# danielzgtg/TTS.cpp

Hardware: AMD Instinct MI355X
Metric: audio-sec/wall-sec (RTF^-1), Parler-TTS-mini v1 Q4_K AR decode + DAC decode (higher is better)
Workload: dtype q4_K weights x q8_K activations (int dot, f32 combine); DAC f16 im2col x f32 weights, f64 accumulate

## Files before the change

### include/tts_hip.h

```cpp
#ifndef TTS_HIP_H
#define TTS_HIP_H

#include <stddef.h>
#include <stdint.h>

#ifdef __cplusplus
extern "C" {
#endif

#define TTS_MAX_DIMS 4
#define TTS_MAX_SRC 4
#define TTS_MAX_OP_PARAMS 16
#define TTS_MAX_NAME 64

enum tts_type {
    TTS_TYPE_F32 = 0,
    TTS_TYPE_F16 = 1,
    TTS_TYPE_Q4_0 = 2,
    TTS_TYPE_Q4_1 = 3,
    TTS_TYPE_Q5_0 = 6,
    TTS_TYPE_Q5_1 = 7,
    TTS_TYPE_Q8_0 = 8,
    TTS_TYPE_Q8_1 = 9,
    TTS_TYPE_Q4_K = 12,
// ... 122 lines not shown
const char * tts_hip_backend_name(tts_hip_backend_t backend);

void * tts_hip_buffer_alloc(tts_hip_backend_t backend, size_t size);
void tts_hip_buffer_free(tts_hip_backend_t backend, void * ptr);
size_t tts_hip_buffer_alignment(void);

int tts_hip_tensor_set(tts_hip_backend_t backend, void * dst_dev, const void * src_host, size_t size);
int tts_hip_tensor_get(tts_hip_backend_t backend, void * dst_host, const void * src_dev, size_t size);
int tts_hip_tensor_copy(tts_hip_backend_t backend, void * dst_dev, const void * src_dev, size_t size);
int tts_hip_copy_stream(tts_hip_backend_t backend, void * dst_dev, const void * src_dev, size_t size);
int tts_hip_plan_stats(tts_tensor * const * nodes, int n_nodes, int mask, int32_t * counts);
int tts_hip_tensor_set_async(tts_hip_backend_t backend, void * dst_dev, const void * src_host, size_t size);
int tts_hip_memset(tts_hip_backend_t backend, void * dst_dev, int value, size_t size);
int tts_hip_synchronize(tts_hip_backend_t backend);

int tts_hip_weight_set(tts_hip_backend_t backend, tts_tensor * t, const void * src_host);
int tts_hip_weight_get(tts_hip_backend_t backend, const tts_tensor * t, void * dst_host);
int tts_hip_quantize(tts_hip_backend_t backend, int type, const float * x_dev, void * dst_dev, int64_t rows, int64_t K);
void tts_repack_q4_K(const void * src, void * dst, int64_t nblocks, int inverse);
void tts_repack_q4_K_tiled(const void * src, void * dst, int64_t nrows, int64_t nb, int inverse);

int tts_hip_supports_op(const tts_tensor * node);
int tts_hip_graph_compute(tts_hip_backend_t backend, tts_tensor * const * nodes, int n_nodes);
int tts_hip_graph_prepare(tts_hip_backend_t backend, tts_tensor * const * nodes, int n_nodes, int slot);
int tts_hip_graph_launch(tts_hip_backend_t backend, int slot);

enum tts_hip_option {
    TTS_HIP_OPT_FUSION = 0,
    TTS_HIP_OPT_PROFILE_GEMV = 1,
    TTS_HIP_OPT_GRAPHS = 2,
    TTS_HIP_OPT_CONV_F32ACC = 3,
    TTS_HIP_OPT_CONVT_LDS = 4,
    TTS_HIP_OPT_ATTN_SPLIT = 5,
    TTS_HIP_OPT_KV_PREFETCH = 6,
    TTS_HIP_OPT_KV_PREFETCH_BLOCKS = 7,
    TTS_HIP_OPT_Q4K_TILE_BYTES = 8,
    TTS_HIP_OPT_GEMV_DEBUG = 10,
    TTS_HIP_OPT_CONV_SPLIT = 12,
    TTS_HIP_OPT_GEMV_UNIQUE = 11,
    TTS_HIP_OPT_GEMV_KS = 13,
    TTS_HIP_OPT_ATTN_FUSED = 14,
    TTS_HIP_OPT_GEMM_Q8 = 18,
    TTS_HIP_OPT_BGEMM_F32 = 19,
    TTS_HIP_OPT_CU_PARTITION = 20,
    TTS_HIP_OPT_Q4K_DUAL_BYTES = 16,
    TTS_HIP_OPT_GEMV_RSPLIT = 17,
    TTS_HIP_OPT_ATTN_PV16 = 15,
    TTS_HIP_OPT_GEMV_PREQUANT = 21,
    TTS_HIP_OPT_GEMV_KRELAY = 22,
    TTS_HIP_OPT_ATTN_KS = 23,
    TTS_HIP_OPT_ATTN_PV8 = 24,
    TTS_HIP_OPT_GEMV_KRELAY_LOOP = 26,
    TTS_HIP_OPT_GEMV_Q80_PRO = 27,
    TTS_HIP_OPT_GEMV_Q80_SLAB = 28,
    TTS_HIP_OPT_GEMV_Q80_RW = 29,
    TTS_HIP_OPT_GEMM_Q8_STAGED = 30,
    TTS_HIP_OPT_GEMV_KR_INKERNEL = 31,
    TTS_HIP_OPT_GEMV_F32_WIDE = 32,
    TTS_HIP_OPT_ATTN_PV_MP = 33,
    TTS_HIP_OPT_GEMM_KR_INKERNEL = 35,
    TTS_HIP_OPT_GEMM_KR_CT2 = 36,
    TTS_HIP_OPT_GEMM_KR_NW = 34,
    TTS_HIP_OPT_GEMV_NW_MIN = 25,
    TTS_HIP_OPT_GEMM_KR_XCD = 38,
    TTS_HIP_OPT_GEMM_KR_CP = 39,
    TTS_HIP_OPT_GEMM_KR_WALK = 40,
    TTS_HIP_OPT_GEMM_PF = 41,
    TTS_HIP_OPT_GEMM_PF_NW = 42,
    TTS_HIP_OPT_ATTN_ONE = 43,
    TTS_HIP_OPT_GEMV_KR_TAIL = 44,
    TTS_HIP_OPT_GEMV_Q50_SLAB = 45,
    TTS_HIP_OPT_GEMV_Q50_RW = 46,
    TTS_HIP_OPT_GEMM_Q5 = 47,
    TTS_HIP_OPT_GEMM_Q5_STAGED = 48,
    TTS_HIP_OPT_GEMV_Q40_SLAB = 49,
    TTS_HIP_OPT_GEMV_Q40_RW = 50,
    TTS_HIP_OPT_GEMM_Q4_0 = 51,
    TTS_HIP_OPT_GEMM_Q4_0_STAGED = 52,
    TTS_HIP_OPT_CONV_VFMA = 53,
    TTS_HIP_OPT_CONV_TILE96 = 54,
    TTS_HIP_OPT_CONV_PACK = 55,
    TTS_HIP_OPT_CONVT_PACK = 56,
    TTS_HIP_OPT_CONV_XREG = 57,
    TTS_HIP_OPT_COALESCE = 37,
};
enum tts_fuse_bits {
    TTS_FUSE_LN = 1, TTS_FUSE_GROUP = 2, TTS_FUSE_KV = 4, TTS_FUSE_EPI = 8, TTS_FUSE_HEADS = 16, TTS_FUSE_ATTN = 32,
    TTS_FUSE_LSTM = 64,
    TTS_FUSE_SNAKE = 128,
    TTS_FUSE_EMBED = 256,
    TTS_FUSE_CONV = 512,
    TTS_FUSE_ADAIN = 1024,
    TTS_FUSE_XATTN = 2048,
    TTS_FUSE_MCPY = 4096,
    TTS_FUSE_CONTREAD = 8192
};
int tts_hip_set_option(tts_hip_backend_t backend, int option, int value);
int tts_hip_attn_decode(tts_hip_backend_t backend, const tts_tensor * q, const tts_tensor * k, const tts_tensor * v,
                        const float * mask, int64_t mbs, float scale, float * out, float * out2, const int64_t * koff,
                        const int64_t * voff, const int64_t * moff, const int32_t * pseq);
int tts_hip_coalesce_stats(int device, int64_t * out, int n);
void tts_hip_coalesce_set_wait(int us);
int tts_hip_coalesce_enable(int on);
#define TTS_HIP_HOOK_FAULT_WEIGHT_SET 1
int tts_hip_test_hook(int hook, int value);
int tts_hip_install_crash_handler(void);
int tts_hip_gemv_stats(tts_hip_backend_t backend, int type, double * ms, int64_t * launches, double * bytes, int reset);
int tts_hip_greedy_step(tts_hip_backend_t backend, const float * logits, int32_t B, int32_t NH, int32_t V, int32_t step,
                        int32_t bos, int32_t eos, int32_t * eos_seen, int32_t * hist, int32_t * next);
typedef struct tts_sampling {
    float temperature;
    float top_p;
    float repetition_penalty;
    int32_t top_k;
    int32_t do_sample;
    int32_t pad_;
    uint64_t seed;
} tts_sampling;
void tts_sampling_default(tts_sampling * cfg);
uint32_t tts_sampler_call_seed(uint64_t seed, int32_t stream, int64_t call);
int tts_sampler_sample(const tts_sampling * cfg, const float * logits, int32_t NH, int32_t V, uint32_t call_seed, int32_t * last,
                       int32_t * count, int32_t * out);
int tts_hip_sample_step(tts_hip_backend_t backend, const float * logits, int32_t B, int32_t NH, int32_t V, const tts_sampling * cfg,
                        int64_t call, int32_t * rep_state, int32_t step, int32_t bos, int32_t eos, int32_t * eos_seen, int32_t * hist,
                        int32_t * next);
int tts_sampling_device_ok(const tts_sampling * cfg, int32_t V);
int tts_hip_counters(tts_hip_backend_t backend, int64_t * out, int n);

int tts_hip_gemv(tts_hip_backend_t backend, int type, const void * w, const float * x, float * y,
                 int64_t K, int64_t N, int64_t M);
int tts_hip_gemv_ex(tts_hip_backend_t backend, int type, const void * w, const float * x, float * y,
                    int64_t K, int64_t N, int64_t M, int32_t wflags);
int tts_hip_gemv_res(tts_hip_backend_t backend, int type, const void * w, const float * x, float * y, const float * res,
                     int64_t K, int64_t N, int64_t M, int32_t wflags);

typedef struct tts_backend_iface {
    void * ctx;
    const char * name;
    void * (*alloc)(void * ctx, size_t size);
    void (*free)(void * ctx, void * ptr);
    int (*set)(void * ctx, void * dst, const void * src, size_t size);
    int (*set_tensor)(void * ctx, tts_tensor * t, const void * src);
    int (*get)(void * ctx, void * dst, const void * src, size_t size);
    int (*memset)(void * ctx, void * dst, int value, size_t size);
    int (*compute)(void * ctx, tts_tensor * const * nodes, int n_nodes);
    int (*synchronize)(void * ctx);
    int (*prepare)(void * ctx, tts_tensor * const * nodes, int n_nodes, int slot);
    int (*launch)(void * ctx, int slot);
    int (*set_async)(void * ctx, void * dst, const void * src, size_t size);
    int (*copy)(void * ctx, void * dst, const void * src, size_t size);
    int (*greedy_step)(void * ctx, const float * logits, int B, int NH, int V, int step, int bos, int eos, int32_t * eos_seen,
                       int32_t * hist, int32_t * next);
    int (*sample_step)(void * ctx, const float * logits, int B, int NH, int V, const tts_sampling * cfg, int64_t call, int32_t * rep_state,
                       int step, int bos, int eos, int32_t * eos_seen, int32_t * hist, int32_t * next);
} tts_backend_iface;

int tts_hip_backend_iface(tts_hip_backend_t backend, tts_backend_iface * out);

#ifdef __cplusplus
}
#endif

#endif
```

### tts.cpp_amd/csrc/backend.hip

```cpp
#include <cmath>
#include <atomic>
#include <cstring>
#include <map>
#include <mutex>
#include <thread>

#include "hip_internal.h"
#include <hip/hip_ext.h>

#include <dlfcn.h>
#include <execinfo.h>
#include <fcntl.h>
#include <signal.h>
#include <unistd.h>

using namespace tts;


static void build_gelu_table(uint16_t * t) {
    const float GELU_COEF_A = 0.044715f;
    const float SQRT_2_OVER_PI = 0.79788456080286535587989211986876f;
    for (int i = 0; i < 65536; ++i) {
        const float x = fp16_to_fp32_host((uint16_t)i);
        const float g = 0.5f * x * (1.0f + tanhf(SQRT_2_OVER_PI * x * (1.0f + GELU_COEF_A * x * x)));
// ... 326 lines not shown
        tts::conv_pack_freed(nullptr, ptr, r.size);
        tts::coalesce_written(ptr, r.size);
    }
    hipFree(ptr);
}

int tts_hip_tensor_set(tts_hip_backend_t be, void * dst, const void * src, size_t size) {
    if (!be) return TTS_STATUS_BAD_ARG;
    hipSetDevice(be->device);
    be->rb_clear();
    drop_tiled_copies(dst, size);
    tts::coalesce_written(dst, size);
    if (size > 0 && size <= be->pin_size / 4) {
        const int st = tts_hip_tensor_set_async(be, dst, src, size);
        if (st != 0) return st;
    } else if (hipMemcpyAsync(dst, src, size, hipMemcpyHostToDevice, be->stream) != hipSuccess) {
        return TTS_STATUS_FAILED;
    } else {
        tts::conv_pack_written(be, dst, size);
    }
    if (hipStreamSynchronize(be->stream) != hipSuccess) return TTS_STATUS_FAILED;
    return 0;
}

int tts_hip_tensor_set_async(tts_hip_backend_t be, void * dst, const void * src, size_t size) {
    if (!be) return TTS_STATUS_BAD_ARG;
    if (size == 0) return 0;
    hipSetDevice(be->device);
    be->rb_clear();
    if (size > be->pin_size / 2) return tts_hip_tensor_set(be, dst, src, size);
    tts::coalesce_written(dst, size);
    std::lock_guard<std::mutex> pl(be->pin_mu);
    while (!be->pin_pending.empty() && hipEventQuery(be->pin_pending.front().ev) == hipSuccess) {
        be->pin_events.push_back(be->pin_pending.front().ev);
        be->pin_pending.pop_front();
    }
    size_t off = (be->pin_head + 255) & ~(size_t)255;
    if (off + size > be->pin_size) off = 0;
    int last = -1;
    for (int i = 0; i < (int)be->pin_pending.size(); ++i) {
        const auto & r = be->pin_pending[i];
        if (r.off < off + size && off < r.off + r.size) last = i;
    }
    if (last >= 0) {
        if (hipEventSynchronize(be->pin_pending[last].ev) != hipSuccess) return TTS_STATUS_FAILED;
        for (int i = 0; i <= last; ++i) {
            be->pin_events.push_back(be->pin_pending.front().ev);
            be->pin_pending.pop_front();
        }
    }
    memcpy(be->pin + off, src, size);
    if (hipMemcpyAsync(dst, be->pin + off, size, hipMemcpyHostToDevice, be->stream) != hipSuccess) return TTS_STATUS_FAILED;
    tts::conv_pack_written(be, dst, size);
    hipEvent_t ev;
    if (be->pin_events.empty()) {
        if (hipEventCreateWithFlags(&ev, hipEventDisableTiming) != hipSuccess) return TTS_STATUS_FAILED;
    } else {
        ev = be->pin_events.back();
        be->pin_events.pop_back();
    }
    if (hipEventRecord(ev, be->stream) != hipSuccess) return TTS_STATUS_FAILED;
    be->pin_pending.push_back({off, size, ev});
    be->pin_head = off + size;
    return 0;
}

int tts_hip_greedy_step(tts_hip_backend_t be, const float * logits, int32_t B, int32_t NH, int32_t V, int32_t step, int32_t bos,
                        int32_t eos, int32_t * eos_seen, int32_t * hist, int32_t * next) {
    if (!be || !logits || B <= 0 || NH <= 0 || V <= 0) return TTS_STATUS_BAD_ARG;
    hipSetDevice(be->device);
    be->rb_clear();
    launch_greedy_step(be, logits, B, NH, V, step, bos, eos, eos_seen, hist, next);
    return 0;
}

int tts_hip_sample_step(tts_hip_backend_t be, const float * logits, int32_t B, int32_t NH, int32_t V, const tts_sampling * cfg, int64_t call,
                        int32_t * rep_state, int32_t step, int32_t bos, int32_t eos, int32_t * eos_seen, int32_t * hist, int32_t * next) {
    if (!be || !logits || !cfg || B <= 0 || NH <= 0 || V <= 0) return TTS_STATUS_BAD_ARG;
    hipSetDevice(be->device);
    be->rb_clear();
    return launch_sample_step(be, logits, B, NH, V, cfg, call, rep_state, step, bos, eos, eos_seen, hist, next);
}

int tts_hip_tensor_get(tts_hip_backend_t be, void * dst, const void * src, size_t size) {
    if (!be) return TTS_STATUS_BAD_ARG;
    hipSetDevice(be->device);
    if (be->rb_any.load(std::memory_order_acquire)) {
        std::lock_guard<std::mutex> l(be->rb_mu);
        for (const auto & r : be->rb) {
            const char * s = (const char *)src;
            if (s >= r.dev && s + size <= r.dev + r.bytes) {
                if (hipStreamSynchronize(be->stream) != hipSuccess) return TTS_STATUS_FAILED;
                memcpy(dst, be->rb_host + r.off + (s - r.dev), size);
                return 0;
            }
        }
    }
    if (hipMemcpyAsync(dst, src, size, hipMemcpyDeviceToHost, be->stream) != hipSuccess) return TTS_STATUS_FAILED;
    if (hipStreamSynchronize(be->stream) != hipSuccess) return TTS_STATUS_FAILED;
    return 0;
}

int tts_hip_copy_stream(tts_hip_backend_t be, void * dst, const void * src, size_t size) {
    if (!be || !dst || !src || size % 16 || ((uintptr_t)dst | (uintptr_t)src) % 16) return TTS_STATUS_BAD_ARG;
    if (size == 0) return 0;
    hipSetDevice(be->device);
    be->rb_clear();
    tts::launch_copy_stream(be, dst, src, (int64_t)(size / 16));
    tts::conv_pack_written(be, dst, size);
    return hipGetLastError() == hipSuccess ? 0 : TTS_STATUS_FAILED;
}

int tts_hip_tensor_copy(tts_hip_backend_t be, void * dst, const void * src, size_t size) {
    if (!be) return TTS_STATUS_BAD_ARG;
    hipSetDevice(be->device);
    be->rb_clear();
    tts::coalesce_written(dst, size);
    tts::launch_copy_bytes(be, dst, src, size);
    tts::conv_pack_written(be, dst, size);
    return hipGetLastError() == hipSuccess ? 0 : TTS_STATUS_FAILED;
}

int tts_hip_memset(tts_hip_backend_t be, void * dst, int value, size_t size) {
    if (!be) return TTS_STATUS_BAD_ARG;
    hipSetDevice(be->device);
    be->rb_clear();
    tts::coalesce_written(dst, size);
    if (hipMemsetAsync(dst, value, size, be->stream) != hipSuccess) return TTS_STATUS_FAILED;
    tts::conv_pack_written(be, dst, size);
    return 0;
}

int tts_hip_synchronize(tts_hip_backend_t be) {
    if (!be) return TTS_STATUS_BAD_ARG;
    hipSetDevice(be->device);
    return hipStreamSynchronize(be->stream) == hipSuccess ? 0 : TTS_STATUS_FAILED;
}

void tts_repack_q4_K(const void * src, void * dst, int64_t nblocks, int inverse) {
    const uint8_t * s = (const uint8_t *)src;
    uint8_t * d = (uint8_t *)dst;
    for (int64_t b = 0; b < nblocks; ++b) {
        const uint8_t * sb = s + b * 144;
        uint8_t * db = d + b * 144;
        memcpy(db, sb, 16);
        for (int i = 0; i < 128; ++i) {
            const int l = i >> 4, c = (i >> 2) & 3, k = i & 3;
            const int nat = 32 * c + 8 * k + l;
            if (!inverse) db[16 + i] = sb[16 + nat];
            else db[16 + nat] = sb[16 + i];
        }
    }
}

static void repack_tiled_rows(const uint8_t * s, uint8_t * d, int64_t r0, int64_t r1, int64_t nb, int inverse) {
    const int64_t rb = nb * 144;
    for (int64_t row = r0; row < r1; ++row) {
        const int64_t t = row >> 2, i = row & 3;
        for (int64_t b = 0; b < nb; ++b) {
            const int64_t nat = row * rb + b * 144;
            const int64_t til = (t * nb + b) * 576;
            const uint8_t * a = inverse ? s + til : s + nat;
            uint8_t * o = inverse ? d + nat : d + til;
            if (!inverse) memcpy(o + i * 16, a, 16);
            else memcpy(o, a + i * 16, 16);
            for (int c = 0; c < 4; ++c)
// ... 330 lines not shown
        }
        default:
            return 0;
    }
}

}

extern "C" int tts_hip_set_option(tts_hip_backend_t be, int option, int value) {
    if (!be) return TTS_STATUS_BAD_ARG;
    switch (option) {
        case TTS_HIP_OPT_FUSION: be->fusion = value; return 0;
        case TTS_HIP_OPT_CONVT_LDS: be->convt_lds = value != 0; return 0;
        case TTS_HIP_OPT_CONV_SPLIT: be->conv_split = value < 0 ? 1 : value; return 0;
        case TTS_HIP_OPT_CONV_VFMA: be->conv_vfma = value < 0 || value > 2 ? 1 : value; return 0;
        case TTS_HIP_OPT_CONV_TILE96: be->conv_tile96 = value != 0; return 0;
        case TTS_HIP_OPT_CONV_PACK: be->conv_pack = value != 0; return 0;
        case TTS_HIP_OPT_CONVT_PACK: be->convt_pack = value != 0; return 0;
        case TTS_HIP_OPT_CONV_XREG: be->conv_xreg = value != 0; return 0;
        case TTS_HIP_OPT_PROFILE_GEMV: be->profile_gemv = value != 0; return 0;
        case TTS_HIP_OPT_GRAPHS: be->use_graphs = value != 0; return 0;
        case TTS_HIP_OPT_CONV_F32ACC:
            be->conv_f32acc = value == 1;
            be->conv_acc_mode = value == 2 ? 2 : 0;
            return 0;
        case TTS_HIP_OPT_ATTN_SPLIT: be->attn_split_minp = value; return 0;
        case TTS_HIP_OPT_ATTN_FUSED: be->attn_fused_minp = value; return 0;
        case TTS_HIP_OPT_ATTN_PV16: be->attn_pv_uv16 = value != 0; return 0;
        case TTS_HIP_OPT_KV_PREFETCH: be->kv_prefetch_minp = value; return 0;
        case TTS_HIP_OPT_Q4K_TILE_BYTES: be->q4k_tile_bytes = value; return 0;
        case TTS_HIP_OPT_Q4K_DUAL_BYTES: be->q4k_dual_bytes = value; return 0;
        case TTS_HIP_OPT_GEMV_RSPLIT: be->gemv_mf_rsplit = value != 0; return 0;
        case TTS_HIP_OPT_GEMV_PREQUANT: be->gemv_mf_prequant = value != 0; return 0;
        case TTS_HIP_OPT_GEMV_KRELAY: be->gemv_kr = value != 0; return 0;
        case TTS_HIP_OPT_GEMV_KRELAY_LOOP: be->gemv_kr_loop = value != 0; return 0;
        case TTS_HIP_OPT_GEMV_Q80_PRO: be->gemv_q80_pro = value != 0; return 0;
        case TTS_HIP_OPT_GEMV_Q80_SLAB: be->gemv_q80_slab = value != 0; return 0;
        case TTS_HIP_OPT_GEMV_KR_INKERNEL:
            if (value < 0) return TTS_STATUS_BAD_ARG;
            be->gemv_kr_ink = value;
            return 0;
        case TTS_HIP_OPT_GEMM_Q8_STAGED:
            if (value < 0 || value > 2) return TTS_STATUS_BAD_ARG;
            be->gemm_q8_staged = value;
            return 0;
        case TTS_HIP_OPT_GEMV_Q80_RW:
            if (value < 0 || value > 32 || (value & (value - 1))) return TTS_STATUS_BAD_ARG;
            be->gemv_q80_rw = value;
            return 0;
        case TTS_HIP_OPT_GEMV_Q50_SLAB: be->gemv_q50_slab = value != 0; return 0;
        case TTS_HIP_OPT_GEMV_Q50_RW:
            if (value < 0 || value > 32 || (value & (value - 1))) return TTS_STATUS_BAD_ARG;
            be->gemv_q50_rw = value;
            return 0;
        case TTS_HIP_OPT_GEMM_Q5: be->gemm_q5 = value != 0; return 0;
        case TTS_HIP_OPT_GEMM_Q5_STAGED:
            if (value < 0 || value > 2) return TTS_STATUS_BAD_ARG;
            be->gemm_q5_staged = value;
            return 0;
        case TTS_HIP_OPT_GEMV_Q40_SLAB: be->gemv_q40_slab = value != 0; return 0;
        case TTS_HIP_OPT_GEMV_Q40_RW:
            if (value < 0 || value > 32 || (value & (value - 1))) return TTS_STATUS_BAD_ARG;
            be->gemv_q40_rw = value;
            return 0;
        case TTS_HIP_OPT_GEMM_Q4_0: be->gemm_q4_0 = value != 0; return 0;
        case TTS_HIP_OPT_GEMM_Q4_0_STAGED:
            if (value < 0 || value > 2) return TTS_STATUS_BAD_ARG;
            be->gemm_q4_0_staged = value;
            return 0;
        case TTS_HIP_OPT_ATTN_KS: be->attn_ks = value; return 0;
        case TTS_HIP_OPT_GEMV_NW_MIN: be->gemv_nw_min = value; return 0;
        case TTS_HIP_OPT_ATTN_PV8: be->attn_pv8 = value != 0; return 0;
        case TTS_HIP_OPT_GEMM_KR_CT2: be->gemm_kr_ct2 = value != 0; return 0;
        case TTS_HIP_OPT_GEMM_KR_INKERNEL: be->gemm_kr_ink = value < 0 ? 0 : value; return 0;
        case TTS_HIP_OPT_ATTN_PV_MP: be->attn_pv_mp = value == 2 ? 2 : value != 0; return 0;
        case TTS_HIP_OPT_ATTN_ONE:
            if (value < 0 || value > 2) return TTS_STATUS_BAD_ARG;
            be->attn_one = value;
            return 0;
        case TTS_HIP_OPT_GEMV_KR_TAIL:
            if (value < 0 || value > 4) return TTS_STATUS_BAD_ARG;
            be->gemv_kr_tail = value;
            return 0;
        case TTS_HIP_OPT_GEMM_KR_NW: be->gemm_kr_nw = value == 8 ? 8 : 4; return 0;
        case TTS_HIP_OPT_GEMM_Q8: be->gemm_q8 = value != 0; return 0;
        case TTS_HIP_OPT_CU_PARTITION: {
            const int count = value & 0xFF, index = (value >> 8) & 0xFF;
            const bool inter = (value >> 16) & 1;
            hipSetDevice(be->device);
            TTS_HIP_CHECK(hipStreamSynchronize(be->stream));
            hipStream_t ns = nullptr;
            if (count <= 1) {
                TTS_HIP_CHECK(hipStreamCreateWithFlags(&ns, hipStreamNonBlocking));
                be->cus = be->cu_total;
            } else {
                if (index >= count) return TTS_STATUS_BAD_ARG;
                std::vector<uint32_t> mask((be->cu_total + 31) / 32, 0u);
                const int per = be->cu_total / count;
                int n = 0;
                for (int c = 0; c < be->cu_total; ++c) {
                    const bool on = inter ? (c % count == index) : (c / per == index && c < per * count);
                    if (on) mask[c / 32] |= 1u << (c % 32), ++n;
                }
                if (hipExtStreamCreateWithCUMask(&ns, (uint32_t)mask.size(), mask.data()) != hipSuccess) return TTS_STATUS_FAILED;
                be->cus = n;
            }
            TTS_HIP_CHECK(hipStreamDestroy(be->stream));
            be->stream = ns;
            for (auto & ex : be->gsig_exec)
                if (ex) hipGraphExecDestroy(ex), ex = nullptr;
            for (auto & g : be->gsig) g = 0;
            return 0;
        }
        case TTS_HIP_OPT_BGEMM_F32: be->bgemm_f32 = value != 0; return 0;
        case TTS_HIP_OPT_GEMV_F32_WIDE: be->gemv_f32_wide = value != 0; return 0;
        case TTS_HIP_OPT_GEMV_DEBUG: be->gemv_dbg = value; return 0;
        case TTS_HIP_OPT_GEMV_UNIQUE: be->gemv_unique = value != 0; return 0;
        case TTS_HIP_OPT_GEMV_KS: be->gemv_ks_tiles = value > 0 ? value : 0; return 0;
        case TTS_HIP_OPT_COALESCE: be->co_member = value != 0; return 0;
        case TTS_HIP_OPT_GEMM_KR_XCD: be->gemm_kr_xcd = value != 0; return 0;
        case TTS_HIP_OPT_GEMM_KR_CP: be->gemm_kr_cp = value != 0; return 0;
        case TTS_HIP_OPT_GEMM_KR_WALK: be->gemm_kr_walk = value < 0 ? 0 : value; return 0;
        case TTS_HIP_OPT_GEMM_PF: be->gemm_pf = value < 0 ? 0 : value; return 0;
        case TTS_HIP_OPT_GEMM_PF_NW: be->gemm_pf_nw = value == 8 ? 8 : 4; return 0;
        case TTS_HIP_OPT_KV_PREFETCH_BLOCKS: be->kv_prefetch_blocks = value > 0 ? value : 1; return 0;
        default: return TTS_STATUS_BAD_ARG;
    }
}

extern "C" int tts_hip_counters(tts_hip_backend_t be, int64_t * out, int n) {
    if (!be || !out) return TTS_STATUS_BAD_ARG;
    const int64_t v[10] = {be->graph_updates, be->graph_instantiations, be->lstm_chains, be->lstm_steps, be->plan_wait_ns,
                           be->cap_plan_ns, be->cap_launch_ns, be->cap_update_ns, (int64_t)g_packs_n.load(), (int64_t)g_packs_bytes.load()};
    int k = 0;
    for (; k < n && k < 10; ++k) out[k] = v[k];
    return k;
}

extern "C" int tts_hip_gemv_stats(tts_hip_backend_t be, int type, double * ms, int64_t * launches, double * bytes, int reset) {
    if (!be) return TTS_STATUS_BAD_ARG;
    hipSetDevice(be->device);
    TTS_HIP_CHECK(hipStreamSynchronize(be->stream));
    for (size_t i = 0; i < be->ev_pending.size(); ++i) {
        float t = 0;
        TTS_HIP_CHECK(hipEventElapsedTime(&t, be->ev_pending[i].first, be->ev_pending[i].second));
        const int ty = be->ev_type[i];
        be->gemv_ms[ty] += t;
        be->gemv_launches[ty] += 1;
        be->gemv_bytes[ty] += be->ev_bytes[i];
        be->ev_free.push_back(be->ev_pending[i].first);
        be->ev_free.push_back(be->ev_pending[i].second);
    }
    be->ev_pending.clear();
    be->ev_bytes.clear();
    be->ev_type.clear();
    double a = 0, c = 0;
    int64_t b = 0;
    for (int ty = 0; ty < TTS_TYPE_COUNT; ++ty) {
        if (type >= 0 && ty != type) continue;
        a += be->gemv_ms[ty];
        b += be->gemv_launches[ty];
        c += be->gemv_bytes[ty];
    }
    if (ms) *ms = a;
    if (launches) *launches = b;
    if (bytes) *bytes = c;
    if (reset) {
        for (int ty = 0; ty < TTS_TYPE_COUNT; ++ty) {
            be->gemv_ms[ty] = 0;
            be->gemv_launches[ty] = 0;
            be->gemv_bytes[ty] = 0;
        }
    }
    return 0;
}

static void * hb_alloc(void * c, size_t n) { return tts_hip_buffer_alloc((tts_hip_backend_t)c, n); }
static void hb_free(void * c, void * p) { tts_hip_buffer_free((tts_hip_backend_t)c, p); }
static int hb_set(void * c, void * d, const void * s, size_t n) { return tts_hip_tensor_set((tts_hip_backend_t)c, d, s, n); }
static int hb_set_tensor(void * c, tts_tensor * t, const void * s) { return tts_hip_weight_set((tts_hip_backend_t)c, t, s); }
static int hb_get(void * c, void * d, const void * s, size_t n) { return tts_hip_tensor_get((tts_hip_backend_t)c, d, s, n); }
static int hb_memset(void * c, void * d, int v, size_t n) { return tts_hip_memset((tts_hip_backend_t)c, d, v, n); }
static int hb_compute(void * c, tts_tensor * const * nodes, int n) { return tts_hip_graph_compute((tts_hip_backend_t)c, nodes, n); }
static int hb_sync(void * c) { return tts_hip_synchronize((tts_hip_backend_t)c); }
static int hb_prepare(void * c, tts_tensor * const * nodes, int n, int slot) {
    return tts_hip_graph_prepare((tts_hip_backend_t)c, nodes, n, slot);
}
static int hb_launch(void * c, int slot) { return tts_hip_graph_launch((tts_hip_backend_t)c, slot); }
static int hb_set_async(void * c, void * d, const void * s, size_t n) { return tts_hip_tensor_set_async((tts_hip_backend_t)c, d, s, n); }
static int hb_copy(void * c, void * d, const void * s, size_t n) { return tts_hip_tensor_copy((tts_hip_backend_t)c, d, s, n); }
static int hb_greedy(void * c, const float * l, int B, int NH, int V, int step, int bos, int eos, int32_t * seen, int32_t * hist, int32_t * next) {
    return tts_hip_greedy_step((tts_hip_backend_t)c, l, B, NH, V, step, bos, eos, seen, hist, next);
}
static int hb_sample(void * c, const float * l, int B, int NH, int V, const tts_sampling * cfg, int64_t call, int32_t * rep, int step, int bos,
                     int eos, int32_t * seen, int32_t * hist, int32_t * next) {
    return tts_hip_sample_step((tts_hip_backend_t)c, l, B, NH, V, cfg, call, rep, step, bos, eos, seen, hist, next);
}

extern "C" int tts_hip_backend_iface(tts_hip_backend_t be, tts_backend_iface * out) {
    if (!be || !out) return TTS_STATUS_BAD_ARG;
    out->ctx = be;
    out->name = be->name;
    out->alloc = hb_alloc;
    out->free = hb_free;
    out->set = hb_set;
    out->set_tensor = hb_set_tensor;
    out->get = hb_get;
    out->memset = hb_memset;
    out->compute = hb_compute;
    out->synchronize = hb_sync;
    out->prepare = hb_prepare;
    out->launch = hb_launch;
    out->set_async = hb_set_async;
    out->copy = hb_copy;
    out->greedy_step = hb_greedy;
    out->sample_step = hb_sample;
    return 0;
}
```

### tts.cpp_amd/csrc/hip_internal.h

```cpp
#pragma once

#include <hip/hip_fp16.h>
#include <hip/hip_runtime.h>

#include <cstdio>
#include <cstdlib>
#include <atomic>
#include <deque>
#include <mutex>
#include <unordered_map>
#include <tuple>
#include <vector>

#include "common.h"

#define TTS_HIP_CHECK(expr)                                                                          \
    do {                                                                                             \
        hipError_t err_ = (expr);                                                                    \
        if (err_ != hipSuccess) {                                                                    \
            fprintf(stderr, "%s:%d: HIP error %s: %s\n", __FILE__, __LINE__, #expr, hipGetErrorString(err_)); \
            abort();                                                                                 \
        }                                                                                            \
    } while (0)

// ... 273 lines not shown
    const int64_t *koff = nullptr, *voff = nullptr;
    const int64_t * moff = nullptr;
    const int * pseq = nullptr;
    int pmax = 0;
    const int64_t * ioff[EMBED_MAX_TERMS] = {};
};
struct BatchCtx {
    int N = 0;
    uint64_t key = 0;
    std::vector<BatchCls> cls;
    std::vector<tts_tensor * const *> mnodes;
    std::vector<tts_hip_backend *> mbe;
    int n_nodes = 0;
    bool checked = false;
    int canon = 0;
    bool ragged = false;
    bool differs = false;
    std::vector<ItemTab> tabs;
    void * comap = nullptr;
    const BatchCls * find(const void * p) const {
        const char * c = (const char *)p;
        size_t lo = 0, hi = cls.size();
        while (lo < hi) {
            const size_t m = (lo + hi) / 2;
            if (cls[m].b0 <= c) lo = m + 1;
            else hi = m;
        }
        if (lo == 0) return nullptr;
        const BatchCls & b = cls[lo - 1];
        return c < b.b0 + b.size ? &b : nullptr;
    }
    template <typename T>
    T * win(T * p) const {
        const BatchCls * b = p ? find(p) : nullptr;
        return b ? (T *)(b->win + ((const char *)p - b->b0)) : p;
    }
    int64_t stride(const void * p) const {
        const BatchCls * b = p ? find(p) : nullptr;
        return b ? b->stride : 0;
    }
    template <typename T>
    T * reloc(T * p, int k) const {
        const BatchCls * b = p ? find(p) : nullptr;
        return b ? (T *)(b->win + k * b->stride + ((const char *)p - b->b0)) : p;
    }
};

}

struct tts_hip_backend {
    int device = 0;
    hipStream_t stream = nullptr;
    char name[64] = {0};
    char * scratch = nullptr;
    size_t scratch_size = 0;
    float * shadow = nullptr;
    size_t shadow_size = 0;
    void * hoist = nullptr;
    size_t hoist_size = 0;
    float * attn_buf = nullptr;
    size_t attn_floats = 0;
    int attn_split_minp = 128;
    int attn_ks = 2;
    int attn_pv_mp = 1;
    int attn_one = 1;
    int attn_pv8 = 0;
    int attn_pv_uv16 = 0;
    int attn_fused_minp = 0;
    unsigned long long * argmax_keys = nullptr;
    unsigned * argmax_counts = nullptr;
    int64_t q4k_tile_bytes = 4 << 20;
    int gemv_dbg = 0;
    int gemv_unique = 1;
    int gemm_q8 = 1;
    int64_t cus = 256;
    int cu_total = 256;
    int bgemm_f32 = 1;
    int gemv_f32_wide = 1;
    int gemm_kr_nw = 4;
    int64_t gemv_ks_tiles = 256;
    int gemv_mf_prequant = 1;
    int gemv_kr = 1;
    int gemv_kr_loop = 1;
    int gemv_kr_tail = 1;
    int gemv_q80_pro = 1;
    int gemv_q80_slab = 1;
    int gemv_q80_rw = 0;
    int gemm_q8_staged = 2;
    int gemv_q50_slab = 1;
    int gemv_q50_rw = 0;
    int gemm_q5 = 1;
    int gemm_q5_staged = 2;
    int gemv_q40_slab = 1;
    int gemv_q40_rw = 0;
    int gemm_q4_0 = 1;
    int gemm_q4_0_staged = 2;
    int64_t gemv_kr_ink = 0;
    int gemm_kr_walk = 0;
    int gemm_pf = 64;
    int gemm_pf_nw = 4;
    int gemm_kr_cp = 0;
    int gemm_kr_xcd = 0;
    int gemm_kr_ct2 = 0;
    int64_t gemm_kr_ink = 0;
    int gemv_nw_min = 0;
    int gemv_mf_rsplit = 1;
    int64_t q4k_dual_bytes = 1 << 20;
    void * sample_cand = nullptr;
    size_t sample_cand_size = 0;
    int kv_prefetch_minp = 0;
    int kv_prefetch_blocks = 128;
    hipStream_t pf_stream = nullptr;
    hipEvent_t pf_fork = nullptr, pf_join = nullptr;
    uint8_t * pin = nullptr;
    size_t pin_size = 0, pin_head = 0;
    struct PinRec {
        size_t off, size;
        hipEvent_t ev;
    };
    std::deque<PinRec> pin_pending;
    std::vector<hipEvent_t> pin_events;
    std::mutex pin_mu;
    hipEvent_t plan_ev[2] = {nullptr, nullptr};
    bool plan_ev_pending[2] = {false, false};
    float * lstm_buf = nullptr;
    float * conv_stage = nullptr;
    size_t conv_stage_floats = 0;
    float * vec_scratch = nullptr;
    size_t lstm_floats = 0;
    tts::ActQuant aq;
    int64_t graph_epoch = 0;
    uint16_t * gelu_table = nullptr;
    bool convt_lds = true;
    double * conv_part = nullptr;
    size_t conv_part_doubles = 0;
    int conv_vfma = 1;
    int conv_tile96 = 1;
    int conv_pack = 1;
    int convt_pack = 1;
    int conv_xreg = 1;
    bool capturing = false;
    int conv_split = 1;
    int fusion = 0x3FFF;
    bool profile_gemv = false;
    double gemv_ms[TTS_TYPE_COUNT] = {0};
    int64_t gemv_launches[TTS_TYPE_COUNT] = {0};
    double gemv_bytes[TTS_TYPE_COUNT] = {0};
    std::vector<std::pair<hipEvent_t, hipEvent_t>> ev_pending;
    std::vector<double> ev_bytes;
    std::vector<int> ev_type;
    std::vector<hipEvent_t> ev_free;
    char * repack_tmp = nullptr;
    size_t repack_tmp_size = 0;
    std::vector<char *> repack_retired;
    float * attn_stage = nullptr;
    size_t attn_stage_size = 0;
    bool use_graphs = false;
    static constexpr int N_GSIG = 4;
    uint64_t gsig[N_GSIG] = {};
    hipGraphExec_t gsig_exec[N_GSIG] = {};
    int gsig_next = 0;
    bool conv_f32acc = false;
    int conv_acc_mode = 0;
    hipStream_t cap_stream = nullptr;
    int64_t graph_updates = 0, graph_instantiations = 0;
    int64_t lstm_chains = 0, lstm_steps = 0;
    int64_t plan_wait_ns = 0;
    int64_t cap_plan_ns = 0, cap_launch_ns = 0, cap_update_ns = 0;
    hipGraphExec_t pexec[2] = {nullptr, nullptr};
    tts_tensor * const * plan_nodes[2] = {nullptr, nullptr};
    int plan_n[2] = {0, 0};
    bool plan_eager[2] = {true, true};
    bool plan_prepared[2] = {false, false};
    tts::BatchCtx * bat = nullptr;
    hipEvent_t co_ev = nullptr;
    int64_t * co_tab = nullptr;
    size_t co_tab_bytes = 0;
    int64_t co_prep_ns = 0;
    bool co_member = true;
    struct RbEnt {
        const char * dev;
        size_t bytes, off;
    };
    char * rb_host = nullptr;
    size_t rb_cap = 0;
    std::vector<RbEnt> rb;
    std::mutex rb_mu;
    std::atomic<bool> rb_any{false};
    void rb_clear() {
        if (!rb_any.load(std::memory_order_acquire)) return;
        std::lock_guard<std::mutex> l(rb_mu);
        rb.clear();
        rb_any.store(false, std::memory_order_release);
    }
};

namespace tts {

const uint8_t * tiled_copy_find(const void * weight);

void profile_pair(tts_hip_backend * be, hipEvent_t & e0, hipEvent_t & e1);
void profile_push(tts_hip_backend * be, hipEvent_t e0, hipEvent_t e1, double bytes, int type);

void launch_quantize_act(tts_hip_backend * be, int wtype, const float * x, int64_t xcs, int64_t K, int64_t M, ActQuant & aq);
void launch_gemv_job(tts_hip_backend * be, const GemvJob & job);
bool gemv_q6k_ok(const GemvJob & j);
bool launch_bgemm_f32(tts_hip_backend * be, const tts_tensor * node);
bool gemm_f32_ok(const GemvJob & j);
void launch_gemm_f32(tts_hip_backend * be, const GemvJob & j);
void launch_copy_cols(tts_hip_backend * be, float * dst, const float * src, int64_t K, int64_t scs, int64_t M);
void launch_profile_spin(tts_hip_backend * be, double us);
void launch_im2col(tts_hip_backend * be, const tts_tensor * node);
constexpr int kLstmQMaxK = 512;
struct LstmStepArgs {
    const float * pre[4];
    const void * w[4];
    int64_t w_rs[4];
    const float * bias[4];
    const float * hprev;
    const float * cprev;
    float * h;
    float * c;
    int Hd, K, wtype;
};
void launch_lstm_step(tts_hip_backend * be, const LstmStepArgs & a, const LstmStepArgs * b = nullptr);
void launch_repeat_interleave1(tts_hip_backend * be, const tts_tensor * dst, const tts_tensor * a, int r);
void launch_copy_bytes(tts_hip_backend * be, void * dst, const void * src, size_t bytes);
void launch_cpy_multi(tts_hip_backend * be, const tts_tensor * src, const tts_tensor * const * dsts, int nd);
void launch_rope_multi(tts_hip_backend * be, const tts_tensor * rope, const tts_tensor * src, const tts_tensor * const * dsts, int nd);
void launch_greedy_step(tts_hip_backend * be, const float * logits, int B, int NH, int V, int step, int bos, int eos, int32_t * eos_seen,
                        int32_t * hist, int32_t * next);
int launch_sample_step(tts_hip_backend * be, const float * logits, int B, int NH, int V, const tts_sampling * c, int64_t call,
                       int32_t * rep_state, int step, int bos, int eos, int32_t * eos_seen, int32_t * hist, int32_t * next);
struct BatchCtx;
void launch_embed_sum(tts_hip_backend * be, const tts_tensor * out, const tts_tensor * const * gr, int n, const BatchCtx * bat = nullptr,
                      const ItemTab * tab = nullptr);
void launch_snake(tts_hip_backend * be, const tts_tensor * dst, const tts_tensor * x, const tts_tensor * alpha, const tts_tensor * recip,
                  const tts_tensor * one = nullptr, const tts_tensor * mask = nullptr);
void launch_lstm_finish(tts_hip_backend * be, const tts_tensor * final_out, const float * hist, int64_t Hd, int64_t T);
bool audio_op_supported(const tts_tensor * n);
int launch_audio_op(tts_hip_backend * be, const tts_tensor * n);
void launch_conv_transpose_1d(tts_hip_backend * be, const tts_tensor * node, int w_stable = 0);
constexpr int CONV1D_MAX_R = 128;
struct Conv1dArgs {
    TD x;
    const void * w = nullptr;
    int w16 = 0;
    int64_t wk = 0, wic = 0, woc = 0;
    float * y = nullptr;
    int64_t ycs = 0;
    const float * bias = nullptr;
    int64_t bcs = 0;
    const float * res = nullptr;
    int64_t rcs = 0;
    int64_t L = 0, IC = 0, OL = 0, OC = 0;
    int K = 1, s = 1, p = 0, d = 1;
    int icc = 0, xw = 0, rs = 0;
    float * copy_dst = nullptr;
    uint32_t x_bytes = 0, w_bytes = 0;
    double * part = nullptr;
    int ic_per_split = 0;
    int w_stable = 0;
    const float * wimg = nullptr;
};
constexpr int CONV1D_XN = 16, CONV1D_WN = 16;
inline int conv1d_icc(int64_t IC, int K, int xw) {
    int best = 0;
    double best_eff = -1.0;
    const int top = (int)(IC < 64 ? IC : 64);
    for (int c = 1; c <= top; ++c) {
        const int r = c * K, rp = (r + 31) & ~31;
        if (rp > 64 || c * xw > 256 * CONV1D_XN) break;
        const double eff = (double)r / rp + 1e-4 * c;
        if (eff > best_eff) best_eff = eff, best = c;
    }
    return best;
}
bool conv1d_fused_ok(int64_t IC, int K, int s, int d, size_t * lds);
__host__ __device__ inline int64_t conv1d_pack_index(int nchunk, int oct, int rp, int ct, int chunk, int row, int r) {
    const int lane = (r & 3) * 16 + (row & 15);
    return (int64_t)(ct * nchunk + chunk) * oct * rp + ((((row >> 4) * (rp >> 4) + (r >> 4)) * 64 + lane) * 4 + ((r >> 2) & 3));
}
__host__ __device__ inline int convt_pack_index(int tap, int half, int icl, int c16) { return (((tap * 2 + half) * 16 + icl) * 16) + c16; }
struct ConvPackKey {
    const tts_hip_backend * be;
    const void * w;
    int kind = 0;
    int w16, K, oct, icc, rp;
    int64_t IC, OC, wk, wic, woc;
    bool operator<(const ConvPackKey & o) const {
        return std::tie(be, w, kind, w16, K, oct, icc, rp, IC, OC, wk, wic, woc) <
               std::tie(o.be, o.w, o.kind, o.w16, o.K, o.oct, o.icc, o.rp, o.IC, o.OC, o.wk, o.wic, o.woc);
    }
    int nchunk() const { return (int)((IC + icc - 1) / icc); }
    int ntile() const { return (int)((OC + oct - 1) / oct); }
    size_t floats() const { return (size_t)ntile() * nchunk() * oct * rp; }
};
void launch_conv1d_pack(hipStream_t stream, const ConvPackKey & k, float * img);
const float * conv_pack_get(tts_hip_backend * be, const ConvPackKey & k);
void conv_pack_written(tts_hip_backend * be, const void * p, size_t n);
void conv_pack_freed(const tts_hip_backend * be, const void * p, size_t n);
bool conv1d_pack_key(const tts_hip_backend * be, const Conv1dArgs & a, ConvPackKey * k);
bool convt_pack_key(const tts_hip_backend * be, const tts_tensor * node, int w_stable, ConvPackKey * k);
struct AdainArgs {
    const float * x = nullptr;
    int64_t xcs = 0;
    float * y = nullptr;
    int64_t ycs = 0;
    const float *gamma = nullptr, *beta = nullptr, *alpha = nullptr, *recip = nullptr;
    const float * one = nullptr;
    int stage = 0;
    const float *gw = nullptr, *gb = nullptr, *bw = nullptr, *bb = nullptr, *style = nullptr;
    int64_t S = 0;
    int64_t gcs = 1, bcs = 1, acs = 1, rcs = 1;
    int64_t T = 0, C = 0;
    float eps = 0.f;
// ... 25 lines not shown
```

### tts.cpp_amd/csrc/k_fused.hip

```cpp
#include "hip_internal.h"

namespace tts {

template <bool RMS>
__global__ __launch_bounds__(256) void k_layernorm(TD dst, TD x, const float * __restrict__ w, const float * __restrict__ bias,
                                                   float eps) {
    __shared__ double shd[2][4];
    const int64_t r = blockIdx.x;
    const int64_t i1 = r % x.ne[1], i2 = (r / x.ne[1]) % x.ne[2], i3 = r / (x.ne[1] * x.ne[2]);
    const float * xr = (const float *)(x.data + i1 * x.nb[1] + i2 * x.nb[2] + i3 * x.nb[3]);
    float * yr = (float *)(dst.data + i1 * dst.nb[1] + i2 * dst.nb[2] + i3 * dst.nb[3]);
    const int n = (int)x.ne[0];
    const int tid = threadIdx.x, lane = tid & 63, wave = tid >> 6;
    auto bsum = [&](double v, int slot) {
        v = wave_sum_f64(v);
        if (lane == 0) shd[slot][wave] = v;
        __syncthreads();
        return ((shd[slot][0] + shd[slot][1]) + shd[slot][2]) + shd[slot][3];
    };
    float mean = 0.f;
    if (!RMS) {
        double s = 0.0;
        for (int i = tid; i < n; i += 256) s += (double)xr[i];
        mean = (float)(bsum(s, 0) / (double)n);
// ... 259 lines not shown
        const float d = __fsub_rn(v[u], mean);
        if (t < T) s2 += (double)__fmul_rn(d, d);
    }
    s2 = block_sum1024(s2, sh);
    const float variance = (float)(s2 / (double)T);
    const float scale = cr_divf(1.0f, cr_sqrtf(__fadd_rn(variance, a.eps)));
    float g, b;
    if (a.gw) {
        __shared__ float gbv[2];
        const int w = threadIdx.x >> 6, l = threadIdx.x & 63;
        if (w < 2) {
            const float * wr = (w == 0 ? a.gw : a.bw) + c * a.S;
            double acc = 0.0;
            for (int64_t k = l * 4; k < a.S; k += 256) {
                const float4 wv = *(const float4 *)(wr + k);
                const float4 xv = *(const float4 *)(a.style + k);
                acc += (double)__fmul_rn(wv.x, xv.x);
                acc += (double)__fmul_rn(wv.y, xv.y);
                acc += (double)__fmul_rn(wv.z, xv.z);
                acc += (double)__fmul_rn(wv.w, xv.w);
            }
            for (int off = 32; off >= 1; off >>= 1) acc += __shfl_xor(acc, off);
            if (l == 0) gbv[w] = __fadd_rn((float)acc, (w == 0 ? a.gb : a.bb)[c]);
        }
        __syncthreads();
        g = gbv[0], b = gbv[1];
    } else {
        g = a.gamma[c * a.gcs], b = a.beta[c * a.bcs];
    }
    const float al = SNAKE ? a.alpha[c * a.acs] : 0.f;
    const float rc = SNAKE ? (a.recip ? a.recip[c * a.rcs] : cr_divf(a.one[0], al)) : 0.f;
#pragma unroll
    for (int u = 0; u < NPT; ++u) {
        const int64_t t = threadIdx.x + 1024 * u;
        if (t >= T) continue;
        const float n = __fmul_rn(__fsub_rn(v[u], mean), scale);
        float o = __fadd_rn(__fadd_rn(n, __fmul_rn(n, g)), b);
        if (SNAKE) {
            const float sn = cr_sinf(__fmul_rn(o, al));
            o = __fadd_rn(o, __fmul_rn(__fmul_rn(sn, sn), rc));
        }
        y[t] = o;
    }
}

bool adain_supported(int64_t T) { return T >= 1 && T <= 1024 * 64; }

__global__ void k_stage_vecs(float * __restrict__ dst, AdainArgs a) {
    const int64_t c = (int64_t)blockIdx.x * blockDim.x + threadIdx.x;
    if (c >= a.C) return;
    if (!a.gw) {
        dst[c] = a.gamma[c * a.gcs];
        dst[a.C + c] = a.beta[c * a.bcs];
    }
    if (a.alpha) dst[2 * a.C + c] = a.alpha[c * a.acs];
    if (a.alpha && a.recip) dst[3 * a.C + c] = a.recip[c * a.rcs];
    if (c == 0 && a.one) dst[4 * a.C] = a.one[0];
}

void launch_adain_snake(tts_hip_backend * be, const AdainArgs & args) {
    AdainArgs a = args;
    if (a.stage) {
        float * v = be->vec_scratch;
        hipLaunchKernelGGL(k_stage_vecs, dim3((unsigned)((a.C + 255) / 256)), dim3(256), 0, be->stream, v, args);
        if (!a.gw) a.gamma = v, a.gcs = 1, a.beta = v + a.C, a.bcs = 1;
        if (a.alpha) a.alpha = v + 2 * a.C, a.acs = 1;
        if (a.alpha && a.recip) a.recip = v + 3 * a.C, a.rcs = 1;
        if (a.one) a.one = v + 4 * a.C;
    }
    const bool sn = a.alpha != nullptr;
    const int npt = a.T <= 8192 ? 8 : a.T <= 16384 ? 16 : a.T <= 32768 ? 32 : 64;
    const dim3 grid((unsigned)a.C), block(1024);
#define TTS_ADAIN(N)                                                                                       \
    if (npt == N) {                                                                                        \
        if (sn) hipLaunchKernelGGL((k_adain_snake<N, true>), grid, block, 0, be->stream, a);               \
        else hipLaunchKernelGGL((k_adain_snake<N, false>), grid, block, 0, be->stream, a);                 \
    }
    TTS_ADAIN(8) TTS_ADAIN(16) TTS_ADAIN(32) TTS_ADAIN(64)
#undef TTS_ADAIN
    TTS_HIP_CHECK(hipGetLastError());
}

__global__ __launch_bounds__(256) void k_greedy_step(const float * __restrict__ logits, int B, int NH, int V, int step, int bos, int eos,
                                                     int32_t * eos_seen, int32_t * hist, int32_t * next) {
    const int row = blockIdx.x * 4 + (threadIdx.x >> 6);
    const int lane = threadIdx.x & 63;
    if (row >= B * NH) return;
    const float * l = logits + (int64_t)row * V;
    float best = -INFINITY;
    int bi = 0x7FFFFFFF;
    for (int i = lane; i < V; i += 64) {
        const float v = l[i];
        if (v > best) {
            best = v;
            bi = i;
        }
    }
    for (int off = 32; off >= 1; off >>= 1) {
        const float ov = __shfl_xor(best, off);
        const int oi = __shfl_xor(bi, off);
        if (ov > best || (ov == best && oi < bi)) {
            best = ov;
            bi = oi;
        }
    }
    if (lane != 0) return;
    const int tok = bi == 0x7FFFFFFF ? 0 : bi;
    const int b = row / NH, h = row % NH;
    hist[row] = tok;
    const int seen = eos_seen[row] | (tok == eos);
    eos_seen[row] = seen;
    next[h * B + b] = step + 1 > h ? (seen ? eos : tok) : bos;
}

__device__ __forceinline__ unsigned long long argmax_key(float v, int i) {
    unsigned u = __float_as_uint(v);
    u = (u & 0x80000000u) ? ~u : (u | 0x80000000u);
    return ((unsigned long long)u << 32) | (unsigned)(0xFFFFFFFFu - (unsigned)i);
}

__global__ __launch_bounds__(256) void k_greedy_step_wide(const float * __restrict__ logits, int B, int NH, int V, int step, int bos,
                                                          int eos, int32_t * eos_seen, int32_t * hist, int32_t * next,
                                                          unsigned long long * keys, unsigned * counts) {
    __shared__ unsigned long long s_k[4];
    const int row = blockIdx.y, nseg = gridDim.x;
    const int64_t seg = ((int64_t)V + nseg - 1) / nseg;
    const int64_t i0 = (int64_t)blockIdx.x * seg, i1 = min((int64_t)V, i0 + seg);
    const float * l = logits + (int64_t)row * V;
    unsigned long long best = 0;
    for (int64_t i = i0 + threadIdx.x; i < i1; i += 256) {
        const unsigned long long k = argmax_key(l[i], (int)i);
        best = k > best ? k : best;
    }
    for (int off = 32; off >= 1; off >>= 1) {
        const unsigned long long o = __shfl_xor(best, off);
        best = o > best ? o : best;
    }
    if ((threadIdx.x & 63) == 0) s_k[threadIdx.x >> 6] = best;
    __syncthreads();
    if (threadIdx.x != 0) return;
    for (int w = 1; w < 4; ++w) best = s_k[w] > best ? s_k[w] : best;
    atomicMax(keys + row, best);
    __threadfence();
    if (atomicAdd(counts + row, 1u) != (unsigned)nseg - 1) return;
    const unsigned long long k = atomicExch(keys + row, 0ull);
    atomicExch(counts + row, 0u);
    const int tok = k ? (int)(0xFFFFFFFFu - (unsigned)(k & 0xFFFFFFFFull)) : 0;
    const int b = row / NH, h = row % NH;
    hist[row] = tok;
    const int seen = eos_seen[row] | (tok == eos);
    eos_seen[row] = seen;
    next[h * B + b] = step + 1 > h ? (seen ? eos : tok) : bos;
}

void launch_greedy_step(tts_hip_backend * be, const float * logits, int B, int NH, int V, int step, int bos, int eos, int32_t * eos_seen,
                        int32_t * hist, int32_t * next) {
    if (V >= 16384 && B * NH <= kArgmaxRows) {
        const unsigned nseg = (unsigned)((V + 4095) / 4096 < 64 ? (V + 4095) / 4096 : 64);
        hipLaunchKernelGGL(k_greedy_step_wide, dim3(nseg, (unsigned)(B * NH)), dim3(256), 0, be->stream, logits, B, NH, V, step, bos, eos,
                           eos_seen, hist, next, be->argmax_keys, be->argmax_counts);
        TTS_HIP_CHECK(hipGetLastError());
        return;
    }
    hipLaunchKernelGGL(k_greedy_step, dim3((unsigned)((B * NH + 3) / 4)), dim3(256), 0, be->stream, logits, B, NH, V, step, bos, eos, eos_seen,
                       hist, next);
    TTS_HIP_CHECK(hipGetLastError());
}

}
```

### tts.cpp_amd/csrc/k_ops.hip

```cpp
#include "hip_internal.h"

namespace tts {

__global__ void k_cpy(TD dst, TD src, int64_t n) {
    for (int64_t k = (int64_t)blockIdx.x * blockDim.x + threadIdx.x; k < n; k += (int64_t)gridDim.x * blockDim.x) {
        int64_t a0, a1, a2, a3, b0, b1, b2, b3;
        unravel(k, src.ne, a0, a1, a2, a3);
        unravel(k, dst.ne, b0, b1, b2, b3);
        if (src.type == TTS_TYPE_I32 && dst.type == TTS_TYPE_I32) {
            *(int32_t *)td_ptr(dst, b0, b1, b2, b3) = *(const int32_t *)td_ptr(src, a0, a1, a2, a3);
        } else {
            td_store(dst, b0, b1, b2, b3, td_load(src, a0, a1, a2, a3));
        }
    }
}

__global__ void k_copy_bytes(char * __restrict__ dst, const char * __restrict__ src, int64_t n) {
    const int64_t n16 = (((uintptr_t)dst | (uintptr_t)src) & 15) == 0 ? n >> 4 : 0;
    const int64_t stride = (int64_t)gridDim.x * blockDim.x;
    const int64_t t = (int64_t)blockIdx.x * blockDim.x + threadIdx.x;
    for (int64_t k = t; k < n16; k += stride) ((uint4 *)dst)[k] = ((const uint4 *)src)[k];
    for (int64_t k = (n16 << 4) + t; k < n; k += stride) dst[k] = src[k];
}

// ... 207 lines not shown
    }
}

__global__ __launch_bounds__(256) void k_soft_max(TD dst, TD a, TD m, int mask_f16, float scale) {
    __shared__ double shd[8];
    __shared__ float shf[8];
    const int64_t r = blockIdx.x;
    const int64_t nc = a.ne[0];
    const float * sp = (const float *)(a.data + r * a.nb[1]);
    float * dp = (float *)(dst.data + r * dst.nb[1]);
    const int64_t i01 = r % a.ne[1], i02 = (r / a.ne[1]) % a.ne[2], i03 = r / (a.ne[1] * a.ne[2]);
    const char * mask = m.data ? m.data + (i01 % m.ne[1]) * m.nb[1] + (i02 % m.ne[2]) * m.nb[2] + (i03 % m.ne[3]) * m.nb[3] : nullptr;
    float mx = -INFINITY;
    for (int64_t i = threadIdx.x; i < nc; i += blockDim.x) {
        float w = __fmul_rn(sp[i], scale);
        if (mask) {
            const float mv = mask_f16 ? __half2float(((const __half *)mask)[i]) : ((const float *)mask)[i];
            w = __fadd_rn(w, __fmul_rn(1.0f, mv));
        }
        dp[i] = w;
        mx = fmaxf(mx, w);
    }
    mx = block_max(mx, shf);
    double s = 0.0;
    for (int64_t i = threadIdx.x; i < nc; i += blockDim.x) {
        const float v = cr_expf(__fsub_rn(dp[i], mx));
        dp[i] = v;
        s += (double)v;
    }
    s = block_sum<double>(s, shd);
    const float inv = (float)(1.0 / s);
    for (int64_t i = threadIdx.x; i < nc; i += blockDim.x) dp[i] = __fmul_rn(dp[i], inv);
}

__device__ __forceinline__ float table_elem(const TD & s0, const char * src, int64_t k) {
    if (s0.type == TTS_TYPE_F32) return ((const float *)src)[k];
    if (s0.type == TTS_TYPE_F16) return __half2float(((const __half *)src)[k]);
    if (s0.type == TTS_TYPE_Q8_0) {
        const block_q8_0 * b = (const block_q8_0 *)src + k / QK8_0;
        return __fmul_rn((float)b->qs[k % QK8_0], __half2float(__ushort_as_half(b->d)));
    }
    if (s0.type == TTS_TYPE_Q5_0) {
        const block_q5_0 * b = (const block_q5_0 *)src + k / QK5_0;
        const int e = (int)(k % QK5_0), jq = e & 15;
        const int nib = e < 16 ? (b->qs[jq] & 0x0F) : (b->qs[jq] >> 4);
        const int hb = (b->qh[e >> 3] >> (e & 7)) & 1;
        return __fmul_rn((float)((nib | (hb << 4)) - 16), __half2float(__ushort_as_half(b->d)));
    }
    if (s0.type == TTS_TYPE_Q4_0) {
        const block_q4_0 * b = (const block_q4_0 *)src + k / QK4_0;
        const int e = (int)(k % QK4_0), jq = e & 15;
        const int nib = e < 16 ? (b->qs[jq] & 0x0F) : (b->qs[jq] >> 4);
        return __fmul_rn((float)(nib - 8), __half2float(__ushort_as_half(b->d)));
    }
    if (s0.type == TTS_TYPE_Q6_K) {
        const uint8_t * b = (const uint8_t *)src + (k / QK_K) * (int64_t)sizeof(block_q6_K);
        const int e = (int)(k % QK_K), h = e >> 7, gq = (e >> 5) & 3, l = e & 31;
        const int qb = b[64 * h + 32 * (gq & 1) + l];
        const int v = ((gq & 2 ? qb >> 4 : qb & 15) | (((b[128 + 32 * h + l] >> (2 * gq)) & 3) << 4)) - 32;
        const float d = __half2float(__ushort_as_half((uint16_t)(b[208] | (b[209] << 8))));
        return __fmul_rn(__fmul_rn(d, (float)(int8_t)b[192 + (e >> 4)]), (float)v);
    }
    const block_q4_K * b = (const block_q4_K *)src + k / QK_K;
    const int e = (int)(k % QK_K);
    const int j64 = e / 64, w = e % 64, hi = w >= 32, l = w % 32;
    const int qbyte = (s0.pad & TTS_FLAG_REPACKED) ? ((l & 7) * 16 + j64 * 4 + (l >> 3)) : (32 * j64 + l);
    const int sb = 2 * j64 + hi;
    const uint8_t * q = b->scales;
    int sc, mn;
    if (sb < 4) {
        sc = q[sb] & 63;
        mn = q[sb + 4] & 63;
    } else {
        sc = (q[sb + 4] & 0xF) | ((q[sb - 4] >> 6) << 4);
        mn = (q[sb + 4] >> 4) | ((q[sb] >> 6) << 4);
    }
    const float d = __half2float(__ushort_as_half(b->d));
    const float dm = __half2float(__ushort_as_half(b->dmin));
    const uint8_t qb = b->qs[qbyte];
    const int qv = hi ? (qb >> 4) : (qb & 0xF);
    return __fsub_rn(__fmul_rn(__fmul_rn(d, (float)sc), (float)qv), __fmul_rn(dm, (float)mn));
}

__device__ __forceinline__ float table_elem_q4K_tiled(const char * base, int64_t row, int64_t nb, int64_t k) {
    const uint8_t * g = (const uint8_t *)base + ((row >> 2) * nb + k / QK_K) * 576;
    const int i = (int)(row & 3);
    const uint8_t * hdr = g + i * 16;
    const int e = (int)(k % QK_K);
    const int c = e / 64, w = e % 64, hi = w >= 32, l = w % 32 % 8, kk = w % 32 / 8;
    const int sb = 2 * c + hi;
    const uint8_t * q = hdr + 4;
    int sc, mn;
    if (sb < 4) {
        sc = q[sb] & 63;
        mn = q[sb + 4] & 63;
    } else {
        sc = (q[sb + 4] & 0xF) | ((q[sb - 4] >> 6) << 4);
        mn = (q[sb + 4] >> 4) | ((q[sb] >> 6) << 4);
    }
    const float d = __half2float(__ushort_as_half(*(const uint16_t *)hdr));
    const float dm = __half2float(__ushort_as_half(*(const uint16_t *)(hdr + 2)));
    const uint8_t qb = g[64 + ((c * 2 + (l >> 2)) * 4 + i) * 16 + (l & 3) * 4 + kk];
    const int qv = hi ? (qb >> 4) : (qb & 0xF);
    return __fsub_rn(__fmul_rn(__fmul_rn(d, (float)sc), (float)qv), __fmul_rn(dm, (float)mn));
}

__global__ void k_get_rows(TD dst, TD s0, TD s1) {
    const int64_t i = blockIdx.x;
    const int64_t i10 = i % s1.ne[0], i11 = (i / s1.ne[0]) % s1.ne[1], i12 = i / (s1.ne[0] * s1.ne[1]);
    const int64_t i01 = *(const int32_t *)(s1.data + i10 * s1.nb[0] + i11 * s1.nb[1] + i12 * s1.nb[2]);
    const char * src = s0.data + i01 * s0.nb[1] + i11 * s0.nb[2] + i12 * s0.nb[3];
    float * out = (float *)(dst.data + i10 * dst.nb[1] + i11 * dst.nb[2] + i12 * dst.nb[3]);
    const int64_t nc = s0.ne[0];
    if (s0.type == TTS_TYPE_Q4_K && (s0.pad & TTS_FLAG_TILED)) {
        for (int64_t k = threadIdx.x; k < nc; k += blockDim.x) out[k] = table_elem_q4K_tiled(s0.data, i01, nc / QK_K, k);
        return;
    }
    for (int64_t k = threadIdx.x; k < nc; k += blockDim.x) out[k] = table_elem(s0, src, k);
}

struct EmbedTerm {
    TD table;
    const int32_t * idx;
    int64_t idx_stride;
    int64_t rows;
    const int64_t * moff;
};
struct EmbedArgs {
    EmbedTerm t[EMBED_MAX_TERMS];
    int n;
    float * out;
    int64_t H, M;
    int64_t ocs;
};

__global__ void k_embed_sum(EmbedArgs a) {
    const int64_t m = blockIdx.y;
    const int64_t h = (int64_t)blockIdx.x * blockDim.x + threadIdx.x;
    if (h >= a.H) return;
    float acc = 0.f;
    for (int t = 0; t < a.n; ++t) {
        const EmbedTerm & T = a.t[t];
        const int64_t r = T.moff ? T.idx[T.moff[m]] : T.idx[(T.rows == 1 ? 0 : m) * T.idx_stride];
        const float v = (T.table.type == TTS_TYPE_Q4_K && (T.table.pad & TTS_FLAG_TILED))
                            ? table_elem_q4K_tiled(T.table.data, r, T.table.ne[0] / QK_K, h)
                            : table_elem(T.table, T.table.data + r * T.table.nb[1], h);
        acc = t == 0 ? v : __fadd_rn(acc, v);
    }
    a.out[m * a.ocs + h] = acc;
}

void launch_embed_sum(tts_hip_backend * be, const tts_tensor * out, const tts_tensor * const * gr, int n, const BatchCtx * bat,
                      const ItemTab * tab) {
    EmbedArgs a{};
    a.n = n;
    a.out = (float *)out->data;
    a.H = out->ne[0];
    a.M = out->ne[1] * out->ne[2] * out->ne[3];
    a.ocs = a.H;
    for (int i = 0; i < n; ++i) {
        a.t[i].table = make_td(gr[i]->src[0]);
        a.t[i].idx = (const int32_t *)gr[i]->src[1]->data;
        a.t[i].idx_stride = (int64_t)(gr[i]->src[1]->nb[0] / 4);
        a.t[i].rows = gr[i]->ne[1] * gr[i]->ne[2] * gr[i]->ne[3];
    }
    if (bat) {
        a.M = bat->N;
        a.ocs = bat->stride(a.out) / 4;
        a.out = bat->win(a.out);
        for (int i = 0; i < n; ++i) {
            if (tab && tab->ioff[i]) {
                a.t[i].moff = tab->ioff[i];
                a.t[i].rows = bat->N;
                continue;
            }
            const int64_t s = bat->stride(a.t[i].idx);
            a.t[i].idx_stride = s / 4;
            a.t[i].rows = s ? bat->N : 1;
            a.t[i].idx = bat->win(a.t[i].idx);
        }
    }
    hipLaunchKernelGGL(k_embed_sum, dim3((unsigned)((a.H + 255) / 256), (unsigned)a.M), dim3(256), 0, be->stream, a);
    TTS_HIP_CHECK(hipGetLastError());
}

__global__ void k_concat(TD dst, TD a, TD b, int dim, int64_t n) {
    const bool i32 = dst.type == TTS_TYPE_I32 && a.type == TTS_TYPE_I32 && b.type == TTS_TYPE_I32;
    for (int64_t k = (int64_t)blockIdx.x * blockDim.x + threadIdx.x; k < n; k += (int64_t)gridDim.x * blockDim.x) {
        int64_t i[4];
        unravel(k, dst.ne, i[0], i[1], i[2], i[3]);
        const bool first = i[0] < a.ne[0] && i[1] < a.ne[1] && i[2] < a.ne[2] && i[3] < a.ne[3];
        const char * sp;
        if (first) sp = td_ptr(a, i[0], i[1], i[2], i[3]);
        else {
            i[dim] -= a.ne[dim];
            sp = td_ptr(b, i[0], i[1], i[2], i[3]);
            i[dim] += a.ne[dim];
        }
        if (i32) *(int32_t *)td_ptr(dst, i[0], i[1], i[2], i[3]) = *(const int32_t *)sp;
        else td_store(dst, i[0], i[1], i[2], i[3], first ? td_load_at(a, sp) : td_load_at(b, sp));
    }
}

__global__ void k_repeat(TD dst, TD a, int64_t n) {
    const bool i32 = dst.type == TTS_TYPE_I32 && a.type == TTS_TYPE_I32;
    for (int64_t k = (int64_t)blockIdx.x * blockDim.x + threadIdx.x; k < n; k += (int64_t)gridDim.x * blockDim.x) {
        int64_t i0, i1, i2, i3;
        unravel(k, dst.ne, i0, i1, i2, i3);
        const char * sp = td_ptr(a, i0 % a.ne[0], i1 % a.ne[1], i2 % a.ne[2], i3 % a.ne[3]);
        if (i32) *(int32_t *)td_ptr(dst, i0, i1, i2, i3) = *(const int32_t *)sp;
        else td_store(dst, i0, i1, i2, i3, td_load_at(a, sp));
    }
}

__global__ __launch_bounds__(256) void k_sum_rows(TD dst, TD a) {
    __shared__ double shd[8];
    const int64_t r = blockIdx.x;
    const int64_t i1 = r % a.ne[1], i2 = (r / a.ne[1]) % a.ne[2], i3 = r / (a.ne[1] * a.ne[2]);
    double s = 0.0;
    for (int64_t i = threadIdx.x; i < a.ne[0]; i += blockDim.x) s += (double)td_load(a, i, i1, i2, i3);
    s = block_sum<double>(s, shd);
    if (threadIdx.x == 0) td_store(dst, 0, i1, i2, i3, (float)s);
}

__global__ void k_rope(CpyMulti m, TD a, const int32_t * pos, const float * ff, int n_dims, int neox, float theta_scale,
                       float freq_scale, float attn_factor) {
    auto td_store_all = [&](int64_t j0, int64_t i1, int64_t i2, int64_t i3, float v) {
        for (int d = 0; d < m.nd; ++d) td_store(m.dst[d], j0, i1, i2, i3, v);
    };
    const int64_t i1 = blockIdx.x, i2 = blockIdx.y, i3 = blockIdx.z;
    const int64_t p = pos[i2];
    for (int64_t i0 = 2 * threadIdx.x; i0 < a.ne[0]; i0 += 2 * blockDim.x) {
        if (i0 < n_dims) {
            float theta = (float)p;
            for (int64_t k = 0; k < i0 / 2; ++k) theta = __fmul_rn(theta, theta_scale);
            const float f = ff ? ff[i0 / 2] : 1.0f;
            const float th = __fmul_rn(freq_scale, cr_divf(theta, f));
            const float c = __fmul_rn(cr_cosf(th), attn_factor), s = __fmul_rn(cr_sinf(th), attn_factor);
            int64_t j0, j1;
            if (neox) {
                j0 = i0 / 2;
                j1 = i0 / 2 + n_dims / 2;
            } else {
                j0 = i0;
                j1 = i0 + 1;
            }
            const float x0 = td_load(a, j0, i1, i2, i3), x1 = td_load(a, j1, i1, i2, i3);
            td_store_all(j0, i1, i2, i3, __fsub_rn(__fmul_rn(x0, c), __fmul_rn(x1, s)));
            td_store_all(j1, i1, i2, i3, __fadd_rn(__fmul_rn(x0, s), __fmul_rn(x1, c)));
        } else {
            const float x0 = td_load(a, i0, i1, i2, i3);
            const float x1 = i0 + 1 < a.ne[0] ? td_load(a, i0 + 1, i1, i2, i3) : 0.f;
            td_store_all(i0, i1, i2, i3, x0);
            if (i0 + 1 < a.ne[0]) td_store_all(i0 + 1, i1, i2, i3, x1);
        }
    }
}

__global__ __launch_bounds__(256) void k_mul_mat_f32(TD dst, TD s0, TD s1, int64_t nout) {
    const int lane = threadIdx.x & 63;
    const int64_t o = (int64_t)blockIdx.x * 4 + (threadIdx.x >> 6);
    if (o >= nout) return;
    const int64_t i01 = o % dst.ne[0];
    int64_t rest = o / dst.ne[0];
    const int64_t i11 = rest % dst.ne[1];
// ... 259 lines not shown
```

### tts.cpp_amd/csrc/k_sample.hip

```cpp
#include "hip_internal.h"

namespace tts {

namespace {

constexpr int SMAX = 4096;
constexpr int KC = 64;

struct SampleArgs {
    const float * logits;
    int B, NH, V;
    float temperature, top_p, rep;
    int top_k, do_sample;
    uint64_t seed;
    int64_t call;
    int32_t * rep_state;
    int step, bos, eos;
    int32_t *eos_seen, *hist, *next;
    unsigned long long * cand;
    int nseg;
};

__device__ __forceinline__ uint32_t ord_f32(float f) {
    const uint32_t u = __float_as_uint(__fadd_rn(f, 0.0f));
    return (u & 0x80000000u) ? ~u : (u | 0x80000000u);
}
__device__ __forceinline__ unsigned long long sort_key(float v, int i) {
    return ((unsigned long long)(~ord_f32(v)) << 32) | (unsigned)i;
}

__device__ void bitonic(unsigned long long * k, int n) {
    for (int size = 2; size <= n; size <<= 1) {
        for (int stride = size >> 1; stride > 0; stride >>= 1) {
            __syncthreads();
            for (int t = threadIdx.x; t < n / 2; t += blockDim.x) {
                const int lo = 2 * t - (t & (stride - 1));
                const int hi = lo + stride;
                const bool up = (lo & size) == 0;
                const unsigned long long a = k[lo], b = k[hi];
                if ((a > b) == up) {
                    k[lo] = b;
                    k[hi] = a;
                }
            }
        }
    }
    __syncthreads();
}

__device__ __forceinline__ uint32_t minstd_at(uint32_t s, int n) {
    uint64_t x = s;
    for (int i = 0; i < n; ++i) x = (x * 48271ull) % 2147483647ull;
    return (uint32_t)x;
}
__device__ __forceinline__ float canonical_f32(uint32_t g) {
    const float r = __fmul_rn((float)(g - 1u), 4.656612873077392578125e-10f);
    return r >= 1.0f ? __uint_as_float(0x3F7FFFFFu) : r;
}

__device__ __forceinline__ uint32_t call_seed_dev(uint64_t seed, int stream, int64_t call) {
    uint64_t z = seed ^ ((uint64_t)(uint32_t)stream << 40) ^ ((uint64_t)call * 0x9E3779B97F4A7C15ull);
    z += 0x9E3779B97F4A7C15ull;
    z = (z ^ (z >> 30)) * 0xBF58476D1CE4E5B9ull;
    z = (z ^ (z >> 27)) * 0x94D049BB133111EBull;
    z ^= z >> 31;
    return (uint32_t)(1 + z % 2147483646ull);
}

struct RowState {
    int last, count;
    double pw;
    bool rep, temp;
};

__device__ __forceinline__ float penal(const RowState & r, int i, float v) {
    return (r.rep && r.last == i) ? (float)((double)v / r.pw) : v;
}
__device__ __forceinline__ float temper(const SampleArgs & a, const RowState & r, float v) {
    return r.temp ? __fdiv_rn(v, a.temperature) : v;
}

__device__ void finish_row(const SampleArgs & a, RowState & r, int row, int tok) {
    const int b = row / a.NH, h = row % a.NH;
    if (r.rep && a.do_sample) {
        if (r.last != tok) r.count = 0;
        r.last = tok;
        r.count += 1;
        a.rep_state[2 * row] = r.last;
        a.rep_state[2 * row + 1] = r.count;
    }
    a.hist[row] = tok;
    const int seen = a.eos_seen[row] | (tok == a.eos);
    a.eos_seen[row] = seen;
    a.next[h * a.B + b] = a.step + 1 > h ? (seen ? a.eos : tok) : a.bos;
}

__device__ int draw_pick(const SampleArgs & a, int row, const float * p, const int * pick, int n, float mhp, bool topp) {
    const int b = row / a.NH, h = row % a.NH;
    float u = canonical_f32(minstd_at(call_seed_dev(a.seed, b, a.call), h + 1));
    if (topp) u = __fmul_rn(u, mhp);
    float cum = 0.0f;
    for (int j = 0; j < n; ++j) {
        cum = __fadd_rn(cum, p[j]);
        if (u <= cum || j >= n - 1) return pick ? pick[j] : j;
    }
    return 0;
}

__device__ void load_state(const SampleArgs & a, int row, RowState & r) {
    r.rep = a.rep != 1.0f;
    r.temp = a.temperature != 1.0f;
    r.last = r.rep ? a.rep_state[2 * row] : -1;
    r.count = r.rep ? a.rep_state[2 * row + 1] : 0;
    r.pw = r.rep ? pow((double)a.rep, (double)(uint32_t)r.count) : 1.0;
}

}

__global__ __launch_bounds__(256) void k_sample_rows(SampleArgs a) {
    __shared__ unsigned long long keys[SMAX];
    __shared__ float pv[SMAX];
    __shared__ int pk[SMAX];
    __shared__ int s_n;
    __shared__ float s_max, s_cum, s_mhp;
    const int row = blockIdx.x;
    const int V = a.V;
    const float * l = a.logits + (int64_t)row * V;
    RowState r;
    load_state(a, row, r);
    int n2 = 1;
    while (n2 < V) n2 <<= 1;
    for (int i = threadIdx.x; i < n2; i += 256) keys[i] = i < V ? sort_key(penal(r, i, l[i]), i) : ~0ull;
    __syncthreads();
    unsigned long long best = ~0ull;
    for (int i = threadIdx.x; i < V; i += 256) best = keys[i] < best ? keys[i] : best;
    for (int off = 32; off >= 1; off >>= 1) {
        const unsigned long long o = __shfl_xor(best, off);
        best = o < best ? o : best;
    }
    __shared__ unsigned long long s_best[4];
    if ((threadIdx.x & 63) == 0) s_best[threadIdx.x >> 6] = best;
    __syncthreads();
    for (int w = 0; w < 4; ++w) best = s_best[w] < best ? s_best[w] : best;
    const int maxi = (int)(best & 0xFFFFFFFFu);
    if (!a.do_sample) {
        if (threadIdx.x == 0) finish_row(a, r, row, maxi);
        return;
    }
    const bool topp = a.top_p < 1.0f;
    const bool usek = a.top_k > 0 && a.top_k < V;
    const float max_val = temper(a, r, penal(r, maxi, l[maxi]));
    if (topp) {
        for (int i = threadIdx.x; i < V; i += 256) pv[i] = cr_expf(__fsub_rn(temper(a, r, penal(r, i, l[i])), max_val));
        __syncthreads();
        if (threadIdx.x == 0) {
            float c = 0.0f;
            for (int i = 0; i < V; ++i) c = __fadd_rn(c, pv[i]);
            s_cum = c;
        }
        __syncthreads();
        const float cum = s_cum;
        for (int i = threadIdx.x; i < V; i += 256) pv[i] = __fdiv_rn(pv[i], cum);
        __syncthreads();
        for (int i = threadIdx.x; i < n2; i += 256) keys[i] = i < V ? sort_key(pv[i], i) : ~0ull;
        bitonic(keys, n2);
        const int n = usek ? a.top_k : V;
        for (int j = threadIdx.x; j < n; j += 256) pk[j] = (int)(keys[j] & 0xFFFFFFFFu);
        __syncthreads();
        if (threadIdx.x == 0) {
            float ps = 0.0f;
            int trim = -1;
            for (int j = 0; j < n; ++j) {
                ps = __fadd_rn(ps, pv[pk[j]]);
                if (ps >= a.top_p) {
                    trim = j + 1;
                    break;
                }
            }
            s_mhp = ps < a.top_p ? ps : a.top_p;
            s_n = trim > 0 ? trim : n;
        }
        __syncthreads();
        float * pp = (float *)keys;
        const int n_ = s_n;
        for (int j = threadIdx.x; j < n_; j += 256) pp[j] = pv[pk[j]];
        __syncthreads();
        if (threadIdx.x == 0) finish_row(a, r, row, draw_pick(a, row, pp, pk, n_, s_mhp, true));
        return;
    }
    if (usek) {
        bitonic(keys, n2);
        const int k = a.top_k;
        for (int j = threadIdx.x; j < k; j += 256) {
            const int i = (int)(keys[j] & 0xFFFFFFFFu);
            pk[j] = i;
            pv[j] = cr_expf(__fsub_rn(temper(a, r, penal(r, i, l[i])), max_val));
        }
        __syncthreads();
        if (threadIdx.x == 0) {
            float c = 0.0f;
            for (int j = 0; j < k; ++j) c = __fadd_rn(c, pv[j]);
            s_cum = c;
        }
        __syncthreads();
        for (int j = threadIdx.x; j < k; j += 256) pv[j] = __fdiv_rn(pv[j], s_cum);
        __syncthreads();
        if (threadIdx.x == 0) finish_row(a, r, row, draw_pick(a, row, pv, pk, k, 1.0f, false));
        return;
    }
    for (int i = threadIdx.x; i < V; i += 256) pv[i] = cr_expf(__fsub_rn(temper(a, r, penal(r, i, l[i])), max_val));
    __syncthreads();
    if (threadIdx.x == 0) {
        float c = 0.0f;
        for (int i = 0; i < V; ++i) c = __fadd_rn(c, pv[i]);
        s_cum = c;
    }
    __syncthreads();
    for (int i = threadIdx.x; i < V; i += 256) pv[i] = __fdiv_rn(pv[i], s_cum);
    __syncthreads();
    if (threadIdx.x == 0) finish_row(a, r, row, draw_pick(a, row, pv, nullptr, V, 1.0f, false));
}

__global__ __launch_bounds__(256) void k_topk_segments(SampleArgs a) {
    __shared__ unsigned long long keys[SMAX];
    const int row = blockIdx.y, seg = blockIdx.x;
    const float * l = a.logits + (int64_t)row * a.V;
    RowState r;
    load_state(a, row, r);
    const int i0 = seg * SMAX;
    for (int t = threadIdx.x; t < SMAX; t += 256) {
        const int i = i0 + t;
        keys[t] = i < a.V ? sort_key(penal(r, i, l[i]), i) : ~0ull;
    }
    bitonic(keys, SMAX);
    for (int t = threadIdx.x; t < KC; t += 256) a.cand[((int64_t)row * a.nseg + seg) * KC + t] = keys[t];
}

__global__ __launch_bounds__(256) void k_sample_wide(SampleArgs a) {
    __shared__ unsigned long long keys[SMAX];
    __shared__ float pv[KC];
    __shared__ int pk[KC];
    __shared__ float s_cum;
    const int row = blockIdx.x;
    const float * l = a.logits + (int64_t)row * a.V;
    RowState r;
    load_state(a, row, r);
    const int nc = a.nseg * KC;
    int n2 = 1;
    while (n2 < nc) n2 <<= 1;
    for (int t = threadIdx.x; t < n2; t += 256) keys[t] = t < nc ? a.cand[(int64_t)row * nc + t] : ~0ull;
    bitonic(keys, n2);
    const int maxi = (int)(keys[0] & 0xFFFFFFFFu);
    if (!a.do_sample) {
        if (threadIdx.x == 0) finish_row(a, r, row, maxi);
        return;
    }
    const float max_val = temper(a, r, penal(r, maxi, l[maxi]));
    const int k = a.top_k;
    for (int j = threadIdx.x; j < k; j += 256) {
        const int i = (int)(keys[j] & 0xFFFFFFFFu);
        pk[j] = i;
        pv[j] = cr_expf(__fsub_rn(temper(a, r, penal(r, i, l[i])), max_val));
    }
    __syncthreads();
    if (threadIdx.x == 0) {
        float c = 0.0f;
        for (int j = 0; j < k; ++j) c = __fadd_rn(c, pv[j]);
        s_cum = c;
    }
    __syncthreads();
    for (int j = threadIdx.x; j < k; j += 256) pv[j] = __fdiv_rn(pv[j], s_cum);
    __syncthreads();
    if (threadIdx.x == 0) finish_row(a, r, row, draw_pick(a, row, pv, pk, k, 1.0f, false));
}

int launch_sample_step(tts_hip_backend * be, const float * logits, int B, int NH, int V, const tts_sampling * c, int64_t call,
                       int32_t * rep_state, int step, int bos, int eos, int32_t * eos_seen, int32_t * hist, int32_t * next) {
    SampleArgs a;
    a.logits = logits;
    a.B = B, a.NH = NH, a.V = V;
    a.temperature = c->temperature, a.top_p = c->top_p, a.rep = c->repetition_penalty;
    a.top_k = c->top_k, a.do_sample = c->do_sample;
    a.seed = c->seed, a.call = call;
    a.rep_state = rep_state;
    a.step = step, a.bos = bos, a.eos = eos;
    a.eos_seen = eos_seen, a.hist = hist, a.next = next;
    a.cand = nullptr, a.nseg = 0;
    if (a.rep != 1.0f && !rep_state) return TTS_STATUS_BAD_ARG;
    const int rows = B * NH;
    if (V <= SMAX) {
        hipLaunchKernelGGL(k_sample_rows, dim3((unsigned)rows), dim3(256), 0, be->stream, a);
        TTS_HIP_CHECK(hipGetLastError());
        return 0;
    }
    const int nseg = (V + SMAX - 1) / SMAX;
    const bool ok = nseg * KC <= SMAX && (!c->do_sample || (c->top_k > 0 && c->top_k <= KC && c->top_p >= 1.0f));
    if (!ok) return TTS_STATUS_UNSUPPORTED;
    const size_t need = (size_t)rows * nseg * KC * sizeof(unsigned long long);
    if (need > be->sample_cand_size) {
        if (be->sample_cand) {
            TTS_HIP_CHECK(hipStreamSynchronize(be->stream));
            TTS_HIP_CHECK(hipFree(be->sample_cand));
        }
        TTS_HIP_CHECK(hipMalloc(&be->sample_cand, need));
        be->sample_cand_size = need;
    }
    a.cand = (unsigned long long *)be->sample_cand;
    a.nseg = nseg;
    hipLaunchKernelGGL(k_topk_segments, dim3((unsigned)nseg, (unsigned)rows), dim3(256), 0, be->stream, a);
    hipLaunchKernelGGL(k_sample_wide, dim3((unsigned)rows), dim3(256), 0, be->stream, a);
    TTS_HIP_CHECK(hipGetLastError());
    return 0;
}

}
```

### tts.cpp_amd/csrc/parler.cpp

```cpp
#include <chrono>
#include <cmath>
#include <cstdio>
#include <cstring>
#include <string>
#include <vector>

#include "../../include/tts_gguf.h"
#include "../../include/tts_runners.h"
#include "graph.h"
#include "weights.h"

using namespace tts;

struct parler_layer {
    tts_tensor *q, *k, *v, *o, *sa_norm, *sa_norm_b;
    tts_tensor *aq, *ak, *av, *ao, *a_norm, *a_norm_b;
    tts_tensor *cross_k, *cross_v;
    tts_tensor *fc1, *fc2, *f_norm, *f_norm_b;
};

struct tts_parler {
    tts_parler_config cfg;
    tts_backend_iface be;
    weight_store w;
    void * kvbuf = nullptr;
    size_t kvbytes = 0;
    std::vector<tts_tensor *> embds, heads;
    std::vector<parler_layer> layers;
    tts_tensor *pos_embd = nullptr, *prompt_embd = nullptr, *text_encoding = nullptr, *norm = nullptr, *norm_b = nullptr;
    std::vector<tts_tensor *> k_l, v_l;
    char * arena = nullptr;
    size_t arena_size = 0;
    tg::context gctx;
    tts_tensor * res = nullptr;
    tts_tensor *in_tokens = nullptr, *in_positions = nullptr, *in_mask = nullptr, *in_mask_cross = nullptr;
    int32_t position = 0;
    int32_t current_step = 0;
    bool ragged = false;
    std::vector<int32_t> seq_len;
    int32_t hole_end = 0;
    int32_t last_nodes = 0;
    double host_us[5] = {0, 0, 0, 0, 0};
    bool prepared = false;
    bool device_sampling = true;
    int prep_slot = 0, prep_n = 0;
    bool prep_audio = true;
    void * launched_out = nullptr;
    int launched_n = 0;
    int64_t host_steps = 0;
    std::vector<std::vector<int32_t>> output_tokens;
    std::vector<std::vector<char>> eos_seen;
    bool sampling = false;
    tts_sampling samp{};
    int64_t sample_calls = 0;
    std::vector<int32_t> rep_last, rep_count;
};

extern "C" void tts_parler_default_config(tts_parler_config * c) {
    c->n_layers = 24;
    c->hidden_size = 1024;
    c->n_attn_heads = 16;
    c->ffn_size = 4096;
    c->n_output_heads = 9;
    c->output_vocab = 1088;
    c->audio_vocab = 1024;
    c->max_ctx = 4096;
    c->n_encode = 3;
    c->prompt_vocab = 32128;
    c->max_positions = 4102;
    c->weight_type = TTS_TYPE_Q4_K;
    c->head_type = TTS_TYPE_F32;
    c->use_cross_attn = 1;
    c->batch = 1;
    c->eos_token = 1024;
    c->bos_token = 1025;
    c->seed = 0x5EED;
    c->arena_bytes = 0;
    c->debug_no_reuse = 0;
    c->pad_ = 0;
}

static tts_tensor * wnew(tts_parler * p, int type, int64_t ne0, int64_t ne1, int kind, const std::string & name) {
    type = p->w.file_type(name, type);
    const weight_fill fill = type != TTS_TYPE_F32 || kind == 0 ? weight_fill::matrix(kind == 3 ? 0.25f : 0.02f)
                             : kind == 1                       ? weight_fill::uniform(0.1f, 1.0f)
                             : kind == 2                       ? weight_fill::uniform(0.02f, 0.0f)
                                                               : weight_fill::uniform(0.5f, 0.0f);
    return p->w.add(type, ne0, ne1, 1, name, fill, p->cfg.seed ^ p->w.index());
}

static tts_tensor * layer_norm(tg::context & c, tts_tensor * x, tts_tensor * w, tts_tensor * b) {
    x = tg::norm(c, x, 0.00001f);
    x = tg::mul(c, x, w);
    return tg::add(c, x, b);
}

static bool run_graph(tts_parler * p, tg::context & c) {
    if (!tg::alloc_graph(c, p->arena, p->arena_size, !p->cfg.debug_no_reuse)) {
        fprintf(stderr, "parler: compute arena too small (%zu needed)\n", c.arena_used);
        return false;
    }
    return true;
}

static bool prep_cross_key_values(tts_parler * p) {
    const auto & cf = p->cfg;
    const int hd = cf.hidden_size / cf.n_attn_heads;
    tg::context & c = p->gctx;
    c.reset();
    for (int l = 0; l < cf.n_layers; ++l) {
        parler_layer & L = p->layers[l];
        tts_tensor * Kc = tg::mul_mat(c, L.ak, p->text_encoding);
        tts_tensor * Vc = tg::mul_mat(c, L.av, p->text_encoding);
        Kc = tg::reshape_3d(c, Kc, hd, cf.n_attn_heads, cf.n_encode);
        Vc = tg::transpose(c, Vc);
// ... 23 lines not shown
    for (int i = 0; i < cf.n_output_heads; ++i)
        p->heads.push_back(wnew(p, cf.head_type, H, cf.output_vocab, 0, "lm_heads." + std::to_string(i) + ".weight.head"));
    p->pos_embd = wnew(p, TTS_TYPE_F32, H, cf.max_positions, 3, "positional_embed");
    p->prompt_embd = wnew(p, TTS_TYPE_F32, H, cf.prompt_vocab, 3, "embed_prompts");
    p->text_encoding = wnew(p, TTS_TYPE_F32, H, cf.n_encode, 3, "text_encoding");
    p->norm = wnew(p, TTS_TYPE_F32, H, 1, 1, "layer_norm.weight");
    p->norm_b = wnew(p, TTS_TYPE_F32, H, 1, 2, "layer_norm.bias");
    p->layers.resize(cf.n_layers);
    for (int l = 0; l < cf.n_layers; ++l) {
        parler_layer & L = p->layers[l];
        const std::string pre = "layers." + std::to_string(l);
        L.q = wnew(p, cf.weight_type, H, H, 0, pre + ".self_attn.q_proj.weight");
        L.k = wnew(p, cf.weight_type, H, H, 0, pre + ".self_attn.k_proj.weight");
        L.v = wnew(p, cf.weight_type, H, H, 0, pre + ".self_attn.v_proj.weight");
        L.o = wnew(p, cf.weight_type, H, H, 0, pre + ".self_attn.out_proj.weight");
        L.sa_norm = wnew(p, TTS_TYPE_F32, H, 1, 1, pre + ".self_attn_layer_norm.weight");
        L.sa_norm_b = wnew(p, TTS_TYPE_F32, H, 1, 2, pre + ".self_attn_layer_norm.bias");
        L.aq = wnew(p, cf.weight_type, H, H, 0, pre + ".encoder_attn.q_proj.weight");
        L.ak = wnew(p, TTS_TYPE_F32, H, H, 0, pre + ".encoder_attn.k_proj.weight");
        L.av = wnew(p, TTS_TYPE_F32, H, H, 0, pre + ".encoder_attn.v_proj.weight");
        L.ao = wnew(p, cf.weight_type, H, H, 0, pre + ".encoder_attn.out_proj.weight");
        L.a_norm = wnew(p, TTS_TYPE_F32, H, 1, 1, pre + ".encoder_attn_layer_norm.weight");
        L.a_norm_b = wnew(p, TTS_TYPE_F32, H, 1, 2, pre + ".encoder_attn_layer_norm.bias");
        L.fc1 = wnew(p, cf.weight_type, H, cf.ffn_size, 0, pre + ".fc1.weight");
        L.fc2 = wnew(p, cf.weight_type, cf.ffn_size, H, 0, pre + ".fc2.weight");
        L.f_norm = wnew(p, TTS_TYPE_F32, H, 1, 1, pre + ".final_layer_norm.weight");
        L.f_norm_b = wnew(p, TTS_TYPE_F32, H, 1, 2, pre + ".final_layer_norm.bias");
    }
}

static tts_parler * parler_create(const tts_backend_iface * be, const tts_parler_config * cfg, const tts_gguf * g) {
    auto * p = new tts_parler();
    p->cfg = *cfg;
    p->be = *be;
    p->w.attach(g);
    const auto & cf = p->cfg;
    const int64_t H = cf.hidden_size;
    const int hd = cf.hidden_size / cf.n_attn_heads;
    const int B = cf.batch < 1 ? 1 : cf.batch;
    p->cfg.batch = B;
    declare_weights(p);
    if (!p->w.upload(p->be)) {
        fprintf(stderr, "parler: weight allocation/upload failed\n");
        tts_parler_free(p);
        return nullptr;
    }
    const size_t ck = (size_t)hd * cf.n_encode * cf.n_attn_heads * 4;
    const size_t cv = ck * (size_t)B;
    const size_t kvl = (size_t)H * cf.max_ctx * 4 * (size_t)B;
    p->kvbytes = (size_t)cf.n_layers * (((ck + 255) & ~(size_t)255) + ((cv + 255) & ~(size_t)255) + 2 * kvl);
    p->kvbuf = p->be.alloc(p->be.ctx, p->kvbytes);
    if (!p->kvbuf) {
        tts_parler_free(p);
        return nullptr;
    }
    p->be.memset(p->be.ctx, p->kvbuf, 0, p->kvbytes);
    char * kp = (char *)p->kvbuf;
    for (int l = 0; l < cf.n_layers; ++l) {
        parler_layer & L = p->layers[l];
        L.cross_k = tg::new_tensor_3d(p->w.wctx, TTS_TYPE_F32, hd, cf.n_encode, cf.n_attn_heads);
        L.cross_k->data = kp;
        kp += (ck + 255) & ~(size_t)255;
        if (B > 1) L.cross_v = tg::new_tensor_4d(p->w.wctx, TTS_TYPE_F32, cf.n_encode, hd, cf.n_attn_heads, B);
        else L.cross_v = tg::new_tensor_3d(p->w.wctx, TTS_TYPE_F32, cf.n_encode, hd, cf.n_attn_heads);
        L.cross_v->data = kp;
        kp += (cv + 255) & ~(size_t)255;
        tts_tensor * k = tg::new_tensor_1d(p->w.wctx, TTS_TYPE_F32, H * cf.max_ctx * B);
        k->data = kp;
        kp += kvl;
        tts_tensor * v = tg::new_tensor_1d(p->w.wctx, TTS_TYPE_F32, H * cf.max_ctx * B);
        v->data = kp;
        kp += kvl;
        tg::set_name(k, "cache_k_l" + std::to_string(l));
        tg::set_name(v, "cache_v_l" + std::to_string(l));
        p->k_l.push_back(k);
        p->v_l.push_back(v);
    }
    p->arena_size = cf.arena_bytes ? cf.arena_bytes : (256ull << 20);
    p->arena = (char *)p->be.alloc(p->be.ctx, p->arena_size);
    if (!p->arena) {
        tts_parler_free(p);
        return nullptr;
    }
    if (cf.use_cross_attn && !prep_cross_key_values(p)) {
        fprintf(stderr, "parler: cross K/V precompute failed\n");
        tts_parler_free(p);
        return nullptr;
    }
    tts_parler_reset(p);
    return p;
}

extern "C" tts_parler * tts_parler_create(const tts_backend_iface * be, const tts_parler_config * cfg) { return parler_create(be, cfg, nullptr); }

extern "C" void tts_parler_free(tts_parler * p) {
    if (!p) return;
    if (p->arena) p->be.free(p->be.ctx, p->arena);
    if (p->kvbuf) p->be.free(p->be.ctx, p->kvbuf);
    p->w.release(p->be);
    delete p;
}

extern "C" void tts_parler_reset(tts_parler * p) {
    p->position = 0;
    p->ragged = false;
    p->seq_len.clear();
    p->hole_end = 0;
    p->current_step = 0;
    p->prepared = false;
    p->output_tokens.assign(p->cfg.batch, {});
    p->eos_seen.assign(p->cfg.batch, std::vector<char>(p->cfg.n_output_heads, 0));
    p->sample_calls = 0;
    p->rep_last.assign((size_t)p->cfg.batch * p->cfg.n_output_heads, -1);
    p->rep_count.assign((size_t)p->cfg.batch * p->cfg.n_output_heads, 0);
}

extern "C" int tts_parler_set_conditional_prompt(tts_parler * p, const float * encoding, int32_t n) {
    if (!p || !encoding || !p->cfg.use_cross_attn || n != p->cfg.n_encode) return TTS_STATUS_BAD_ARG;
    if (p->be.synchronize(p->be.ctx) != 0) return TTS_STATUS_FAILED;
    if (p->be.set_tensor(p->be.ctx, p->text_encoding, encoding) != 0) return TTS_STATUS_FAILED;
    if (!prep_cross_key_values(p)) return TTS_STATUS_FAILED;
    tts_parler_reset(p);
    return TTS_STATUS_SUCCESS;
}

extern "C" void tts_parler_set_sampling(tts_parler * p, const tts_sampling * cfg) {
    p->sampling = cfg != nullptr;
    if (cfg) p->samp = *cfg;
}

static tts_tensor * build_graph(tts_parler * p, bool audio, int n) {
    const auto & cf = p->cfg;
    const int B = cf.batch;
    const int64_t H = cf.hidden_size;
    const int hd = cf.hidden_size / cf.n_attn_heads;
    const int nh = cf.n_attn_heads;
    const int64_t full = p->position + n;
    const size_t S = (size_t)H * cf.max_ctx * 4;
    tg::context & c = p->gctx;
    c.reset();

    const bool rg = p->ragged && B > 1;
    p->in_positions = tg::new_tensor_1d(c, TTS_TYPE_I32, rg ? (int64_t)n * B : n);
    tg::set_input(p->in_positions);
    tts_tensor * inp = nullptr;
    if (audio) {
        if (B == 1) {
            tts_tensor * tok = tg::reshape_2d(c, tg::new_tensor_1d(c, TTS_TYPE_I32, (int64_t)n * cf.n_output_heads), n, cf.n_output_heads);
            p->in_tokens = tok->view_src;
            tg::set_input(p->in_tokens);
            for (int i = 0; i < cf.n_output_heads; ++i) {
                tts_tensor * e = tg::get_rows(c, p->embds[i], tg::view_2d(c, tok, 1, n, tok->nb[1], i * sizeof(int32_t)));
                inp = i == 0 ? e : tg::add(c, e, inp);
            }
        } else {
            p->in_tokens = tg::new_tensor_1d(c, TTS_TYPE_I32, (int64_t)B * cf.n_output_heads);
            tg::set_input(p->in_tokens);
            for (int i = 0; i < cf.n_output_heads; ++i) {
                tts_tensor * idx = tg::view_1d(c, p->in_tokens, B, (size_t)i * B * sizeof(int32_t));
                tts_tensor * e = tg::get_rows(c, p->embds[i], idx);
                inp = i == 0 ? e : tg::add(c, e, inp);
            }
        }
    } else {
        if (B == 1) {
            p->in_tokens = tg::new_tensor_1d(c, TTS_TYPE_I32, n);
            tg::set_input(p->in_tokens);
            inp = tg::get_rows(c, p->prompt_embd, p->in_tokens);
        } else {
            p->in_tokens = tg::new_tensor_1d(c, TTS_TYPE_I32, (int64_t)n * B);
            tg::set_input(p->in_tokens);
            inp = tg::reshape_3d(c, tg::get_rows(c, p->prompt_embd, p->in_tokens), H, n, B);
        }
    }
    tts_tensor * pe = tg::get_rows(c, p->pos_embd, p->in_positions);
    if (rg && !audio) pe = tg::reshape_3d(c, pe, H, n, B);
    tts_tensor * inpL = tg::add(c, inp, pe);
    if (B > 1 && audio) inpL = tg::reshape_3d(c, inpL, H, 1, B);

    p->in_mask = rg ? tg::new_tensor_4d(c, TTS_TYPE_F32, full, n, 1, B) : tg::new_tensor_2d(c, TTS_TYPE_F32, full, full);
    tg::set_input(p->in_mask);
    p->in_mask_cross = tg::new_tensor_2d(c, TTS_TYPE_F32, cf.n_encode, n);
    tg::set_input(p->in_mask_cross);

    const float kq_scale = 1.0f / sqrtf((float)hd);
    tts_tensor * cur = nullptr;
    for (int l = 0; l < cf.n_layers; ++l) {
        parler_layer & L = p->layers[l];
        tts_tensor * residual = inpL;
        cur = layer_norm(c, inpL, L.sa_norm, L.sa_norm_b);
        tts_tensor * attn_out;
        {
            tts_tensor * Qcur = tg::mul_mat(c, L.q, cur);
            tts_tensor * Kcur = tg::mul_mat(c, L.k, cur);
            tts_tensor * Vcur = tg::mul_mat(c, L.v, cur);
            if (B == 1) {
                tts_tensor * kv = tg::view_1d(c, p->k_l[l], (int64_t)n * H, tts_row_size(TTS_TYPE_F32, H) * p->position);
                tg::build_forward_expand(c, tg::cpy(c, Kcur, kv));
                tts_tensor * vv = tg::view_2d(c, p->v_l[l], n, H, (size_t)cf.max_ctx * 4, (size_t)p->position * 4);
                tts_tensor * vt = tg::cont(c, tg::transpose(c, Vcur));
                tg::build_forward_expand(c, tg::cpy(c, vt, vv));
            } else {
                tts_tensor * kv = tg::view_2d(c, p->k_l[l], (int64_t)n * H, B, S, tts_row_size(TTS_TYPE_F32, H) * p->position);
                tg::build_forward_expand(c, tg::cpy(c, Kcur, kv));
                tts_tensor * vv = tg::view_3d(c, p->v_l[l], n, H, B, (size_t)cf.max_ctx * 4, S, (size_t)p->position * 4);
                tts_tensor * V3 = tg::reshape_3d(c, Vcur, H, n, B);
                tts_tensor * vt = tg::cont(c, tg::transpose(c, V3));
                tg::build_forward_expand(c, tg::cpy(c, vt, vv));
            }
            tts_tensor *k, *v, *q;
            if (B == 1) {
                k = tg::view_3d(c, p->k_l[l], hd, full, nh, tts_row_size(TTS_TYPE_F32, H), tts_row_size(TTS_TYPE_F32, hd), 0);
                v = tg::view_3d(c, p->v_l[l], full, hd, nh, 4 * (size_t)cf.max_ctx, 4 * (size_t)cf.max_ctx * hd, 0);
                Qcur = tg::reshape_3d(c, Qcur, hd, nh, n);
            } else {
                k = tg::view_4d(c, p->k_l[l], hd, full, nh, B, tts_row_size(TTS_TYPE_F32, H), tts_row_size(TTS_TYPE_F32, hd), S, 0);
                v = tg::view_4d(c, p->v_l[l], full, hd, nh, B, 4 * (size_t)cf.max_ctx, 4 * (size_t)cf.max_ctx * hd, S, 0);
                Qcur = tg::reshape_4d(c, Qcur, hd, nh, n, B);
            }
            q = tg::cont(c, tg::permute(c, Qcur, 0, 2, 1, 3));
            tts_tensor * kq = tg::mul_mat(c, tg::cont(c, k), q);
            kq = tg::soft_max_ext(c, kq, p->in_mask, kq_scale, 0.0f);
            tts_tensor * kqv = tg::mul_mat(c, kq, v);
            tts_tensor * merged = tg::permute(c, kqv, 2, 0, 1, 3);
            attn_out = B == 1 ? tg::cont_2d(c, merged, H, n) : tg::cont_3d(c, merged, H, n, B);
            attn_out = tg::mul_mat(c, L.o, attn_out);
        }
        cur = tg::add(c, attn_out, residual);
        if (cf.use_cross_attn) {
            tts_tensor * residuala = cur;
            cur = layer_norm(c, cur, L.a_norm, L.a_norm_b);
            tts_tensor * Qcur = tg::mul_mat(c, L.aq, cur);
            Qcur = B == 1 ? tg::reshape_3d(c, Qcur, hd, nh, n) : tg::reshape_4d(c, Qcur, hd, nh, n, B);
            tts_tensor * q = tg::cont(c, tg::permute(c, Qcur, 0, 2, 1, 3));
            tts_tensor * kq = tg::mul_mat(c, L.cross_k, q);
            kq = tg::soft_max_ext(c, kq, p->in_mask_cross, kq_scale, 0.0f);
            tts_tensor * kqv = tg::mul_mat(c, kq, L.cross_v);
            tts_tensor * merged = tg::permute(c, kqv, 2, 0, 1, 3);
            cur = B == 1 ? tg::cont_2d(c, merged, H, n) : tg::cont_3d(c, merged, H, n, B);
            cur = tg::mul_mat(c, L.ao, cur);
            cur = tg::add(c, cur, residuala);
        }
        tts_tensor * residualffn = cur;
        cur = layer_norm(c, cur, L.f_norm, L.f_norm_b);
        cur = tg::mul_mat(c, L.fc1, cur);
        cur = tg::gelu(c, cur);
        cur = tg::mul_mat(c, L.fc2, cur);
        cur = tg::add(c, cur, residualffn);
        inpL = cur;
    }
    if (!audio && B > 1) {
        tg::set_output(cur);
        tg::build_forward_expand(c, cur);
        return cur;
    }
    cur = layer_norm(c, cur, p->norm, p->norm_b);
    tts_tensor * out = nullptr;
    for (int i = 0; i < cf.n_output_heads; ++i) {
        tts_tensor * h = tg::mul_mat(c, p->heads[i], cur);
        out = i == 0 ? h : tg::concat(c, out, h, 1);
    }
    tg::set_name(out, "final_out");
    if (B == 1) {
        const int64_t sql = tg::nelements(out) / ((int64_t)cf.output_vocab * cf.n_output_heads);
        out = tg::cont_3d(c, out, cf.output_vocab, sql, cf.n_output_heads);
    }
    tg::set_output(out);
    tg::build_forward_expand(c, out);
    return out;
}

static int set_inputs(tts_parler * p, const int32_t * tokens, bool audio, int n, bool async = false) {
    const auto & cf = p->cfg;
    const int B = cf.batch;
    auto & be0 = p->be;
    struct {
        tts_backend_iface & b;
        bool a;
        void * ctx;
        int set(void *, void * d, const void * s, size_t n) { return a ? b.set_async(b.ctx, d, s, n) : b.set(b.ctx, d, s, n); }
    } be{be0, async && be0.set_async, be0.ctx};
    int st = 0;
    if (audio && !tokens) {
    } else if (audio) {
        if (B == 1) {
            st |= be.set(be.ctx, p->in_tokens->data, tokens, sizeof(int32_t) * n * cf.n_output_heads);
        } else {
            std::vector<int32_t> hm((size_t)B * cf.n_output_heads);
            for (int b = 0; b < B; ++b)
                for (int h = 0; h < cf.n_output_heads; ++h) hm[(size_t)h * B + b] = tokens[(size_t)b * cf.n_output_heads + h];
            st |= be.set(be.ctx, p->in_tokens->data, hm.data(), sizeof(int32_t) * hm.size());
        }
    } else {
        st |= be.set(be.ctx, p->in_tokens->data, tokens, sizeof(int32_t) * n * B);
    }
    const int64_t full = p->position + n;
    if (p->ragged && B > 1) {
        std::vector<int32_t> pos((size_t)n * B);
        std::vector<float> mask((size_t)B * n * full);
        for (int b = 0; b < B; ++b) {
            const int32_t L = p->seq_len[b];
            for (int i = 0; i < n; ++i) {
                const int32_t s = p->position + i;
                pos[(size_t)b * n + i] = s < p->hole_end ? s : L + (s - p->hole_end);
                for (int64_t j = 0; j < full; ++j)
                    mask[((size_t)b * n + i) * full + j] = j > s || (j >= L && j < p->hole_end) ? -INFINITY : 0.0f;
            }
        }
        st |= be.set(be.ctx, p->in_positions->data, pos.data(), sizeof(int32_t) * pos.size());
        st |= be.set(be.ctx, p->in_mask->data, mask.data(), mask.size() * sizeof(float));
    } else {
        std::vector<int32_t> pos(n);
        for (int i = 0; i < n; ++i) pos[i] = p->position + i;
        st |= be.set(be.ctx, p->in_positions->data, pos.data(), sizeof(int32_t) * n);
        std::vector<float> mask((size_t)n * full);
        for (int i = 0; i < n; ++i)
            for (int64_t j = 0; j < full; ++j) mask[(size_t)i * full + j] = j > pos[i] ? -INFINITY : 0.0f;
        st |= be.set(be.ctx, p->in_mask->data, mask.data(), mask.size() * sizeof(float));
    }
    std::vector<float> mc((size_t)cf.n_encode * n, 0.0f);
    st |= be.set(be.ctx, p->in_mask_cross->data, mc.data(), mc.size() * sizeof(float));
    return st;
}

static int prepare_step(tts_parler * p, bool audio, int n) {
    const auto & cf = p->cfg;
    if (p->position + n > cf.max_ctx) return TTS_STATUS_BAD_ARG;
    auto t0 = std::chrono::steady_clock::now();
    p->res = build_graph(p, audio, n);
    auto t1 = std::chrono::steady_clock::now();
    if (!run_graph(p, p->gctx)) return TTS_STATUS_ALLOC_FAILED;
    auto t2 = std::chrono::steady_clock::now();
    p->last_nodes = (int32_t)p->gctx.nodes.size();
    p->prep_slot = (int)(p->host_steps & 1);
    p->prep_audio = audio;
    p->prep_n = n;
    if (p->be.prepare) {
        const int st = p->be.prepare(p->be.ctx, p->gctx.nodes.data(), (int)p->gctx.nodes.size(), p->prep_slot);
        if (st != 0) return st;
    }
    auto t3 = std::chrono::steady_clock::now();
    p->prepared = true;
    auto us = [](auto a, auto b) { return std::chrono::duration<double, std::micro>(b - a).count(); };
    p->host_us[0] += us(t0, t1);
    p->host_us[1] += us(t1, t2);
    p->host_us[3] += us(t2, t3);
    return 0;
}

static int launch_step(tts_parler * p, const int32_t * tokens, bool async = false) {
    if (!p->prepared) return TTS_STATUS_FAILED;
    auto t0 = std::chrono::steady_clock::now();
    if (set_inputs(p, tokens, p->prep_audio, p->prep_n, async) != 0) return TTS_STATUS_FAILED;
    auto t1 = std::chrono::steady_clock::now();
    const int st = p->be.launch ? p->be.launch(p->be.ctx, p->prep_slot)
                                : p->be.compute(p->be.ctx, p->gctx.nodes.data(), (int)p->gctx.nodes.size());
    if (st != 0) return st;
    auto t2 = std::chrono::steady_clock::now();
    p->prepared = false;
    p->launched_out = p->res->data;
    p->launched_n = p->prep_n;
    p->position += p->prep_n;
    p->host_steps += 1;
    auto us = [](auto a, auto b) { return std::chrono::duration<double, std::micro>(b - a).count(); };
    p->host_us[2] += us(t0, t1);
    p->host_us[3] += us(t1, t2);
    return 0;
}

static int finish_step(tts_parler * p, float * logits) {
    const auto & cf = p->cfg;
    auto t0 = std::chrono::steady_clock::now();
    int st = 0;
    if (logits) {
        const size_t bytes = (size_t)cf.batch * p->launched_n * cf.n_output_heads * cf.output_vocab * sizeof(float);
        st = p->be.get(p->be.ctx, logits, p->launched_out, bytes);
    }
    auto t1 = std::chrono::steady_clock::now();
    p->host_us[4] += std::chrono::duration<double, std::micro>(t1 - t0).count();
    return st;
}

static int decode(tts_parler * p, const int32_t * tokens, bool audio, int n, float * logits) {
    int st = prepare_step(p, audio, n);
    if (st == 0) st = launch_step(p, tokens);
    if (st == 0) st = finish_step(p, logits);
    return st;
}

extern "C" int tts_parler_prefill(tts_parler * p, const int32_t * tokens, int32_t n) {
    int st = decode(p, tokens, false, n, nullptr);
    if (st == 0) p->be.synchronize(p->be.ctx);
    return st;
}

extern "C" int tts_parler_prefill_ragged(tts_parler * p, const int32_t * tokens, const int32_t * lens, int32_t n_max) {
    if (!p || !tokens || !lens || n_max < 1 || p->position != 0 || p->current_step != 0) return TTS_STATUS_BAD_ARG;
    const int B = p->cfg.batch;
    for (int b = 0; b < B; ++b)
        if (lens[b] < 1 || lens[b] > n_max) return TTS_STATUS_BAD_ARG;
    p->seq_len.assign(lens, lens + B);
    p->hole_end = n_max;
    p->ragged = B > 1;
    std::vector<int32_t> tok((size_t)B * n_max);
    for (int b = 0; b < B; ++b)
        for (int i = 0; i < n_max; ++i) tok[(size_t)b * n_max + i] = i < lens[b] ? tokens[(size_t)b * n_max + i] : 0;
    int st = decode(p, tok.data(), false, n_max, nullptr);
    if (st == 0) p->be.synchronize(p->be.ctx);
    return st;
}

extern "C" int tts_parler_decode(tts_parler * p, const int32_t * audio_tokens, float * logits) {
    return decode(p, audio_tokens, true, 1, logits);
}

static int32_t argmax_head(const float * l, int vocab) {
    float mx = -INFINITY;
    int32_t id = 0;
    for (int i = 0; i < vocab; ++i) {
        if (l[i] > mx) {
            mx = l[i];
            id = i;
        }
    }
    return id;
}

static int generate_device(tts_parler * p, int32_t n_steps, int32_t * tokens_out) {
    const auto & cf = p->cfg;
    const int B = cf.batch, NH = cf.n_output_heads, V = cf.output_vocab;
    auto & be = p->be;
    const size_t rowi = (size_t)B * NH * sizeof(int32_t);
    int32_t * d_seen = (int32_t *)be.alloc(be.ctx, rowi);
    int32_t * d_next = (int32_t *)be.alloc(be.ctx, rowi);
    int32_t * d_hist = (int32_t *)be.alloc(be.ctx, rowi * (size_t)n_steps);
    int32_t * d_rep = p->sampling ? (int32_t *)be.alloc(be.ctx, 2 * rowi) : nullptr;
    auto release = [&] {
        for (int32_t * q : {d_rep, d_seen, d_next, d_hist})
            if (q) be.free(be.ctx, q);
    };
    if (!d_seen || !d_next || !d_hist || (p->sampling && !d_rep)) {
        release();
        return TTS_STATUS_ALLOC_FAILED;
    }
    std::vector<int32_t> rep(2 * (size_t)B * NH);
    if (p->sampling) {
        for (size_t r = 0; r < (size_t)B * NH; ++r) rep[2 * r] = p->rep_last[r], rep[2 * r + 1] = p->rep_count[r];
        if (be.set(be.ctx, d_rep, rep.data(), 2 * rowi) != 0) {
            release();
            return TTS_STATUS_FAILED;
        }
    }
    std::vector<int32_t> seen((size_t)B * NH), next((size_t)B * NH);
    for (int b = 0; b < B; ++b)
        for (int h = 0; h < NH; ++h) {
            seen[(size_t)b * NH + h] = p->eos_seen[b][h] ? 1 : 0;
            const auto & ot = p->output_tokens[b];
            next[(size_t)b * NH + h] = p->current_step > h ? (p->eos_seen[b][h] ? cf.eos_token : ot[ot.size() - NH + h]) : cf.bos_token;
        }
    int st = be.set(be.ctx, d_seen, seen.data(), rowi);
    if (st == 0 && !p->prepared) st = prepare_step(p, true, 1);
    if (st == 0) st = launch_step(p, next.data(), true);
    for (int s = 0; st == 0 && s < n_steps; ++s) {
        const float * logits = (const float *)p->launched_out;
        if (s + 1 < n_steps) st = prepare_step(p, true, 1);
        if (st == 0 && p->sampling)
            st = be.sample_step(be.ctx, logits, B, NH, V, &p->samp, p->sample_calls + s, d_rep, p->current_step + s, cf.bos_token, cf.eos_token,
                                d_seen, d_hist + (size_t)s * B * NH, d_next);
        else if (st == 0)
            st = be.greedy_step(be.ctx, logits, B, NH, V, p->current_step + s, cf.bos_token, cf.eos_token, d_seen,
                                d_hist + (size_t)s * B * NH, d_next);
        if (st == 0 && s + 1 < n_steps) {
            st = be.copy(be.ctx, p->in_tokens->data, d_next, rowi);
            if (st == 0) st = launch_step(p, nullptr, true);
        }
    }
    std::vector<int32_t> hist((size_t)n_steps * B * NH);
    if (st == 0) st = be.get(be.ctx, hist.data(), d_hist, hist.size() * sizeof(int32_t));
    if (st == 0) st = be.get(be.ctx, seen.data(), d_seen, rowi);
    if (st == 0 && d_rep) {
        st = be.get(be.ctx, rep.data(), d_rep, 2 * rowi);
        for (size_t r = 0; r < (size_t)B * NH; ++r) p->rep_last[r] = rep[2 * r], p->rep_count[r] = rep[2 * r + 1];
    }
    release();
    if (st != 0) return st;
    for (int s = 0; s < n_steps; ++s)
        for (int b = 0; b < B; ++b)
            for (int h = 0; h < NH; ++h) {
                const int32_t t = hist[((size_t)s * B + b) * NH + h];
                p->output_tokens[b].push_back(t);
                if (tokens_out) tokens_out[((size_t)b * n_steps + s) * NH + h] = t;
            }
    for (int b = 0; b < B; ++b)
        for (int h = 0; h < NH; ++h) p->eos_seen[b][h] = seen[(size_t)b * NH + h] != 0;
    p->current_step += n_steps;
    p->sample_calls += n_steps;
    return 0;
}

extern "C" int tts_parler_generate(tts_parler * p, int32_t n_steps, int32_t * tokens_out) {
    const auto & cf = p->cfg;
    if (n_steps <= 0) return 0;
    const bool dev_sample = !p->sampling || (p->be.sample_step && tts_sampling_device_ok(&p->samp, cf.output_vocab));
    if (p->be.greedy_step && p->be.set_async && p->be.copy && p->be.prepare && p->device_sampling && dev_sample)
        return generate_device(p, n_steps, tokens_out);
    const int B = cf.batch, NH = cf.n_output_heads;
    std::vector<float> logits((size_t)B * NH * cf.output_vocab);
    std::vector<int32_t> next((size_t)B * NH);
    for (int s = 0; s < n_steps; ++s) {
        for (int b = 0; b < B; ++b) {
            const auto & ot = p->output_tokens[b];
            for (int h = 0; h < NH; ++h) {
                int32_t t;
                if (p->current_step > h) {
                    t = p->eos_seen[b][h] ? cf.eos_token : ot[ot.size() - NH + h];
                } else {
                    t = cf.bos_token;
                }
                next[(size_t)b * NH + h] = t;
            }
        }
        int st = p->prepared ? 0 : prepare_step(p, true, 1);
        if (st == 0) st = launch_step(p, next.data());
        if (st == 0 && s + 1 < n_steps) st = prepare_step(p, true, 1);
        if (st == 0) st = finish_step(p, logits.data());
        if (st != 0) return st;
        std::vector<int32_t> drawn((size_t)B * NH);
        if (p->sampling) {
            for (int b = 0; b < B; ++b) {
                const int st2 = tts_sampler_sample(&p->samp, logits.data() + (size_t)b * NH * cf.output_vocab, NH, cf.output_vocab,
                                                   tts_sampler_call_seed(p->samp.seed, b, p->sample_calls), &p->rep_last[(size_t)b * NH],
                                                   &p->rep_count[(size_t)b * NH], &drawn[(size_t)b * NH]);
                if (st2 != 0) return st2;
            }
            p->sample_calls += 1;
        }
        for (int b = 0; b < B; ++b) {
            for (int h = 0; h < NH; ++h) {
                const int32_t t = p->sampling ? drawn[(size_t)b * NH + h]
                                              : argmax_head(logits.data() + ((size_t)b * NH + h) * cf.output_vocab, cf.output_vocab);
                p->output_tokens[b].push_back(t);
                if (tokens_out) tokens_out[((size_t)b * n_steps + s) * NH + h] = t;
                p->eos_seen[b][h] = p->eos_seen[b][h] || t == cf.eos_token;
            }
        }
        p->current_step += 1;
    }
    return 0;
}

extern "C" int32_t tts_parler_position(const tts_parler * p) { return p->position; }

extern "C" int tts_parler_set_position(tts_parler * p, int32_t position) {
    if (position < p->position || position >= p->cfg.max_ctx) return TTS_STATUS_BAD_ARG;
    p->position = position;
    p->prepared = false;
    return 0;
// ... 111 lines not shown
```

### tts.cpp_amd/ttship/__init__.py

```python
import ctypes
import os
import pathlib

_HERE = pathlib.Path(__file__).resolve().parent
PKG_ROOT = _HERE.parent
REPO_ROOT = PKG_ROOT.parent
LIB_PATH = PKG_ROOT / "lib" / "libtts_hip.so"

F32, F16, Q4_0, Q5_0, Q8_0, Q4_K, Q6_K, Q8_K, I32 = 0, 1, 2, 6, 8, 12, 14, 15, 26
QUANT_MIX_Q4_K_M = 1
PROF_ATTN = 39

OPS = ["NONE", "DUP", "ADD", "SUB", "MUL", "DIV", "SQR", "SQRT", "SIN", "COS", "SUM_ROWS", "REPEAT",
       "CONCAT", "NORM", "RMS_NORM", "MUL_MAT", "SCALE", "CPY", "CONT", "RESHAPE", "VIEW", "PERMUTE",
       "TRANSPOSE", "GET_ROWS", "SOFT_MAX", "ROPE", "CLAMP", "CONV_TRANSPOSE_1D", "IM2COL", "UPSCALE",
       "PAD", "LEAKY_RELU", "UNARY", "CUMSUM", "MOD", "ROUND", "STFT", "ISTFT", "MAP_CUSTOM3", "MAP_CUSTOM2"]
OP = {n: i for i, n in enumerate(OPS)}
FUSE = {"LN": 1, "GROUP": 2, "KV": 4, "EPI": 8, "HEADS": 16, "ATTN": 32, "LSTM": 64, "SNAKE": 128, "EMBED": 256, "CONV": 512, "ADAIN": 1024, "XATTN": 2048, "MCPY": 4096, "CONTREAD": 8192}
FUSE_ALL = sum(FUSE.values())
UNARY = {"ABS": 0, "NEG": 1, "TANH": 2, "RELU": 3, "SIGMOID": 4, "GELU": 5, "SILU": 6, "EXP": 7}

OPT = {"FUSION": 0, "PROFILE_GEMV": 1, "GRAPHS": 2, "CONV_F32ACC": 3, "CONVT_LDS": 4, "ATTN_SPLIT": 5, "KV_PREFETCH": 6, "KV_PREFETCH_BLOCKS": 7, "Q4K_TILE_BYTES": 8, "GEMV_DEBUG": 10, "GEMV_UNIQUE": 11, "CONV_SPLIT": 12, "GEMV_KS": 13, "ATTN_FUSED": 14, "ATTN_PV16": 15, "Q4K_DUAL_BYTES": 16, "GEMV_RSPLIT": 17, "GEMM_Q8": 18, "BGEMM_F32": 19, "CU_PARTITION": 20, "GEMV_PREQUANT": 21, "GEMV_KRELAY": 22, "ATTN_KS": 23, "ATTN_PV8": 24, "GEMV_NW_MIN": 25, "GEMV_KRELAY_LOOP": 26, "GEMV_Q80_PRO": 27, "GEMV_Q80_SLAB": 28, "GEMV_Q80_RW": 29, "GEMM_Q8_STAGED": 30, "GEMV_KR_INKERNEL": 31, "GEMV_F32_WIDE": 32, "ATTN_PV_MP": 33, "GEMM_KR_NW": 34, "GEMM_KR_INKERNEL": 35, "GEMM_KR_CT2": 36, "COALESCE": 37, "GEMM_KR_XCD": 38, "GEMM_KR_CP": 39, "GEMM_KR_WALK": 40, "GEMM_PF": 41, "GEMM_PF_NW": 42, "ATTN_ONE": 43, "GEMV_KR_TAIL": 44, "GEMV_Q50_SLAB": 45, "GEMV_Q50_RW": 46, "GEMM_Q5": 47, "GEMM_Q5_STAGED": 48, "GEMV_Q40_SLAB": 49, "GEMV_Q40_RW": 50, "GEMM_Q4_0": 51, "GEMM_Q4_0_STAGED": 52, "CONV_VFMA": 53, "CONV_TILE96": 54, "CONV_PACK": 55, "CONVT_PACK": 56, "CONV_XREG": 57}
ATTN_SPLIT_DEFAULT = 128
ATTN_ONE_DEFAULT = 1
GEMV_KR_TAIL_DEFAULT = 1
ATTN_FUSED_ON = 128

TYPE_SIZE = {F32: 4, F16: 2, Q4_K: 144, Q6_K: 210, Q8_0: 34, Q5_0: 22, Q4_0: 18, I32: 4}
BLCK_SIZE = {F32: 1, F16: 1, Q4_K: 256, Q6_K: 256, Q8_0: 32, Q5_0: 32, Q4_0: 32, I32: 1}


class TtsTensor(ctypes.Structure):
    pass


TtsTensor._fields_ = [
    ("type", ctypes.c_int32),
    ("op", ctypes.c_int32),
    ("ne", ctypes.c_int64 * 4),
    ("nb", ctypes.c_uint64 * 4),
    ("op_params", ctypes.c_int32 * 16),
    ("src", ctypes.POINTER(TtsTensor) * 4),
    ("view_src", ctypes.POINTER(TtsTensor)),
    ("view_offs", ctypes.c_uint64),
    ("data", ctypes.c_void_p),
    ("flags", ctypes.c_int32),
    ("pad_", ctypes.c_int32),
    ("name", ctypes.c_char * 64),
]


class BackendIface(ctypes.Structure):
    _fields_ = [
        ("ctx", ctypes.c_void_p),
        ("name", ctypes.c_char_p),
        ("alloc", ctypes.c_void_p),
        ("free", ctypes.c_void_p),
        ("set", ctypes.c_void_p),
        ("set_tensor", ctypes.c_void_p),
        ("get", ctypes.c_void_p),
        ("memset", ctypes.c_void_p),
        ("compute", ctypes.c_void_p),
        ("synchronize", ctypes.c_void_p),
        ("prepare", ctypes.c_void_p),
        ("launch", ctypes.c_void_p),
        ("set_async", ctypes.c_void_p),
        ("copy", ctypes.c_void_p),
        ("greedy_step", ctypes.c_void_p),
        ("sample_step", ctypes.c_void_p),
    ]


class Sampling(ctypes.Structure):
    _fields_ = [
        ("temperature", ctypes.c_float),
        ("top_p", ctypes.c_float),
        ("repetition_penalty", ctypes.c_float),
        ("top_k", ctypes.c_int32),
        ("do_sample", ctypes.c_int32),
        ("pad_", ctypes.c_int32),
        ("seed", ctypes.c_uint64),
    ]


def sampling(**kw):
    c = Sampling()
    lib().tts_sampling_default(ctypes.byref(c))
    for k, v in kw.items():
        setattr(c, k, v)
    return c


def call_seed(seed, stream, call):
    return int(lib().tts_sampler_call_seed(seed, stream, call))


def host_sample(cfg, logits, call_seed_, last=None, count=None):
    import numpy as np
    lg = np.ascontiguousarray(logits, dtype=np.float32)
    NH, V = lg.shape
    out = np.zeros(NH, dtype=np.int32)
    if last is None:
        last = np.full(NH, -1, dtype=np.int32)
    if count is None:
        count = np.zeros(NH, dtype=np.int32)
    st = lib().tts_sampler_sample(ctypes.byref(cfg), lg.ctypes.data, NH, V, call_seed_, last.ctypes.data, count.ctypes.data, out.ctypes.data)
    if st != 0:
        raise RuntimeError(f"tts_sampler_sample failed {st}")
    return out


class ParlerConfig(ctypes.Structure):
    _fields_ = [
        ("n_layers", ctypes.c_int32),
        ("hidden_size", ctypes.c_int32),
        ("n_attn_heads", ctypes.c_int32),
        ("ffn_size", ctypes.c_int32),
        ("n_output_heads", ctypes.c_int32),
        ("output_vocab", ctypes.c_int32),
        ("audio_vocab", ctypes.c_int32),
        ("max_ctx", ctypes.c_int32),
        ("n_encode", ctypes.c_int32),
        ("prompt_vocab", ctypes.c_int32),
        ("max_positions", ctypes.c_int32),
        ("weight_type", ctypes.c_int32),
        ("head_type", ctypes.c_int32),
        ("use_cross_attn", ctypes.c_int32),
        ("batch", ctypes.c_int32),
        ("eos_token", ctypes.c_int32),
        ("bos_token", ctypes.c_int32),
        ("seed", ctypes.c_uint64),
        ("arena_bytes", ctypes.c_uint64),
        ("debug_no_reuse", ctypes.c_int32),
        ("pad_", ctypes.c_int32),
    ]


class T5Config(ctypes.Structure):
    _fields_ = [
        ("n_layers", ctypes.c_int32),
        ("hidden_size", ctypes.c_int32),
        ("n_attn_heads", ctypes.c_int32),
        ("head_size", ctypes.c_int32),
        ("ffn_size", ctypes.c_int32),
        ("relative_attn_buckets", ctypes.c_int32),
        ("vocab_size", ctypes.c_int32),
        ("max_context_length", ctypes.c_int32),
        ("output_size", ctypes.c_int32),
        ("has_down_proj", ctypes.c_int32),
        ("weight_type", ctypes.c_int32),
        ("eos_token_id", ctypes.c_int32),
        ("seed", ctypes.c_uint64),
        ("arena_bytes", ctypes.c_uint64),
        ("debug_no_reuse", ctypes.c_int32),
        ("pad_", ctypes.c_int32),
    ]


class OrpheusConfig(ctypes.Structure):
    _fields_ = [
        ("n_layers", ctypes.c_int32),
        ("hidden_size", ctypes.c_int32),
        ("n_attn_heads", ctypes.c_int32),
        ("n_kv_attn_heads", ctypes.c_int32),
# ... 117 lines not shown

_lib = None


class QuantizeParams(ctypes.Structure):
    _fields_ = [("quantize_type", ctypes.c_int32), ("quantize_output_heads", ctypes.c_int32),
                ("quantize_text_embeddings", ctypes.c_int32), ("quantize_cross_attn_kv", ctypes.c_int32),
                ("convert_dac_to_f16", ctypes.c_int32), ("convert_non_quantizable_to_f16", ctypes.c_int32),
                ("mix", ctypes.c_int32)]


QUANTIZE_ROWS_FN = ctypes.CFUNCTYPE(ctypes.c_int, ctypes.c_void_p, ctypes.c_int32, ctypes.c_void_p, ctypes.c_void_p,
                                    ctypes.c_int64, ctypes.c_int64)


def row_size(t, ne0):
    return TYPE_SIZE[t] * (ne0 // BLCK_SIZE[t])


def lib():
    global _lib
    if _lib is not None:
        return _lib
    path = LIB_PATH
    variant = os.environ.get("TTS_HIP_LIB_VARIANT")
    if variant:
        path = PKG_ROOT / "lib" / variant / "libtts_hip.so"
    if not path.exists():
        raise RuntimeError(f"{path} missing: run `make -j8` (or __graft_entry__.build())")
    L = ctypes.CDLL(str(path))
    vp, i32, i64, u64, sz = ctypes.c_void_p, ctypes.c_int32, ctypes.c_int64, ctypes.c_uint64, ctypes.c_size_t
    sig = {
        "tts_type_size": (sz, [ctypes.c_int]),
        "tts_blck_size": (i64, [ctypes.c_int]),
        "tts_row_size": (sz, [ctypes.c_int, i64]),
        "tts_type_name": (ctypes.c_char_p, [ctypes.c_int]),
        "tts_op_name": (ctypes.c_char_p, [ctypes.c_int]),
        "tts_hip_device_count": (ctypes.c_int, []),
        "tts_hip_backend_init": (vp, [ctypes.c_int]),
        "tts_hip_backend_free": (None, [vp]),
        "tts_hip_backend_name": (ctypes.c_char_p, [vp]),
        "tts_hip_buffer_alloc": (vp, [vp, sz]),
        "tts_hip_buffer_free": (None, [vp, vp]),
        "tts_hip_buffer_alignment": (sz, []),
        "tts_hip_tensor_set": (ctypes.c_int, [vp, vp, vp, sz]),
        "tts_hip_tensor_get": (ctypes.c_int, [vp, vp, vp, sz]),
        "tts_hip_tensor_copy": (ctypes.c_int, [vp, vp, vp, sz]),
        "tts_hip_copy_stream": (ctypes.c_int, [vp, vp, vp, sz]),
        "tts_hip_memset": (ctypes.c_int, [vp, vp, ctypes.c_int, sz]),
        "tts_hip_synchronize": (ctypes.c_int, [vp]),
        "tts_hip_supports_op": (ctypes.c_int, [ctypes.POINTER(TtsTensor)]),
        "tts_hip_graph_compute": (ctypes.c_int, [vp, ctypes.POINTER(ctypes.POINTER(TtsTensor)), ctypes.c_int]),
        "tts_hip_set_option": (ctypes.c_int, [vp, ctypes.c_int, ctypes.c_int]),
        "tts_hip_attn_decode": (ctypes.c_int, [vp, ctypes.POINTER(TtsTensor), ctypes.POINTER(TtsTensor), ctypes.POINTER(TtsTensor), vp,
                                               i64, ctypes.c_float, vp, vp, vp, vp, vp, vp]),
        "tts_hip_gemv_stats": (ctypes.c_int, [vp, ctypes.c_int, ctypes.POINTER(ctypes.c_double), ctypes.POINTER(i64),
                                              ctypes.POINTER(ctypes.c_double), ctypes.c_int]),
        "tts_hip_gemv": (ctypes.c_int, [vp, ctypes.c_int, vp, vp, vp, i64, i64, i64]),
        "tts_hip_gemv_ex": (ctypes.c_int, [vp, ctypes.c_int, vp, vp, vp, i64, i64, i64, i32]),
        "tts_hip_gemv_res": (ctypes.c_int, [vp, ctypes.c_int, vp, vp, vp, vp, i64, i64, i64, i32]),
        "tts_hip_counters": (ctypes.c_int, [vp, ctypes.POINTER(i64), ctypes.c_int]),
        "tts_hip_coalesce_stats": (ctypes.c_int, [ctypes.c_int, ctypes.POINTER(i64), ctypes.c_int]),
        "tts_hip_coalesce_set_wait": (None, [ctypes.c_int]),
        "tts_hip_coalesce_enable": (ctypes.c_int, [ctypes.c_int]),
        "tts_hip_test_hook": (ctypes.c_int, [ctypes.c_int, ctypes.c_int]),
        "tts_hip_install_crash_handler": (ctypes.c_int, []),
        "tts_parler_n_weights": (i32, [vp]),
        "tts_dia_n_weights": (i32, [vp]),
        "tts_dia_weight": (u64, [vp, i32, ctypes.c_char_p, u64, ctypes.POINTER(i64), ctypes.POINTER(i32), vp, u64]),
        "tts_parler_weight": (u64, [vp, i32, ctypes.c_char_p, u64, ctypes.POINTER(i64), ctypes.POINTER(i32), vp, u64]),
        "tts_orpheus_n_weights": (i32, [vp]),
        "tts_orpheus_weight": (u64, [vp, i32, ctypes.c_char_p, u64, ctypes.POINTER(i64), ctypes.POINTER(i32), vp, u64]),
        "tts_dac_n_weights": (i32, [vp]),
        "tts_dac_weight": (u64, [vp, i32, ctypes.c_char_p, u64, ctypes.POINTER(i64), ctypes.POINTER(i32), vp, u64]),
        "tts_sampling_default": (None, [ctypes.POINTER(Sampling)]),
        "tts_parler_set_sampling": (None, [vp, ctypes.POINTER(Sampling)]),
        "tts_parler_set_position": (ctypes.c_int, [vp, i32]),
        "tts_dia_set_sampling": (None, [vp, ctypes.POINTER(Sampling)]),
        "tts_orpheus_set_sampling": (None, [vp, ctypes.POINTER(Sampling)]),
        "tts_sampler_call_seed": (ctypes.c_uint32, [ctypes.c_uint64, i32, i64]),
        "tts_sampler_sample": (ctypes.c_int, [ctypes.POINTER(Sampling), vp, i32, i32, ctypes.c_uint32, vp, vp, vp]),
        "tts_hip_sample_step": (ctypes.c_int, [vp, vp, i32, i32, i32, ctypes.POINTER(Sampling), i64, vp, i32, i32, i32, vp, vp, vp]),
        "tts_hip_greedy_step": (ctypes.c_int, [vp, vp, i32, i32, i32, i32, i32, i32, vp, vp, vp]),
        "tts_hip_backend_iface": (ctypes.c_int, [vp, ctypes.POINTER(BackendIface)]),
        "tts_hip_weight_set": (ctypes.c_int, [vp, ctypes.POINTER(TtsTensor), vp]),
        "tts_hip_quantize": (ctypes.c_int, [vp, ctypes.c_int, vp, vp, i64, i64]),
        "tts_hip_weight_get": (ctypes.c_int, [vp, ctypes.POINTER(TtsTensor), vp]),
        "tts_repack_q4_K": (None, [vp, vp, i64, ctypes.c_int]),
        "tts_repack_q4_K_tiled": (None, [vp, vp, i64, i64, ctypes.c_int]),
        "tts_dia_default_config": (None, [ctypes.POINTER(DiaConfig)]),
        "tts_dia_create": (vp, [ctypes.POINTER(BackendIface), ctypes.POINTER(DiaConfig)]),
        "tts_dia_free": (None, [vp]),
        "tts_dia_prefill": (ctypes.c_int, [vp, vp, i32, vp, vp]),
        "tts_dia_decode": (ctypes.c_int, [vp, vp, vp]),
        "tts_dia_generate": (ctypes.c_int, [vp, vp, i32, vp]),
        "tts_dia_position": (i32, [vp]),
        "tts_dia_last_graph_nodes": (i32, [vp]),
        "tts_dia_weight_bytes": (u64, [vp]),
        "tts_dia_graph": (vp, [vp, ctypes.POINTER(i32)]),
        "tts_orpheus_default_config": (None, [ctypes.POINTER(OrpheusConfig)]),
        "tts_orpheus_create": (vp, [ctypes.POINTER(BackendIface), ctypes.POINTER(OrpheusConfig)]),
        "tts_orpheus_free": (None, [vp]),
        "tts_orpheus_reset": (None, [vp]),
        "tts_orpheus_prefill": (ctypes.c_int, [vp, vp, i32, vp]),
        "tts_orpheus_decode": (ctypes.c_int, [vp, vp, vp]),
        "tts_orpheus_generate": (ctypes.c_int, [vp, vp, i32, vp]),
        "tts_orpheus_position": (i32, [vp]),
        "tts_orpheus_last_graph_nodes": (i32, [vp]),
        "tts_orpheus_weight_bytes": (u64, [vp]),
        "tts_orpheus_graph": (vp, [vp, ctypes.POINTER(i32)]),
        "tts_t5_default_config": (None, [ctypes.POINTER(T5Config)]),
        "tts_t5_create": (vp, [ctypes.POINTER(BackendIface), ctypes.POINTER(T5Config)]),
        "tts_t5_free": (None, [vp]),
        "tts_t5_encode": (ctypes.c_int, [vp, vp, i32, vp]),
        "tts_t5_output_size": (i32, [vp]),
        "tts_t5_last_graph_nodes": (i32, [vp]),
        "tts_t5_weight_bytes": (u64, [vp]),
        "tts_t5_n_weights": (i32, [vp]),
        "tts_t5_weight": (u64, [vp, i32, ctypes.c_char_p, u64, ctypes.POINTER(ctypes.c_int64), ctypes.POINTER(i32), vp, u64]),
        "tts_t5_graph": (vp, [vp, ctypes.POINTER(i32)]),
        "tts_t5_get_node": (u64, [vp, ctypes.c_char_p, vp, u64]),
        "tts_t5_node": (u64, [vp, i32, ctypes.POINTER(i32), ctypes.POINTER(i32), ctypes.POINTER(i64), vp, u64]),
        "tts_t5_config_from_gguf": (ctypes.c_int, [vp, ctypes.POINTER(T5Config)]),
        "tts_t5_create_from_gguf": (vp, [ctypes.POINTER(BackendIface), ctypes.POINTER(T5Config), vp]),
        "tts_t5_write_synthetic_gguf": (ctypes.c_int, [ctypes.POINTER(T5Config), ctypes.c_char_p]),
        "tts_parler_set_conditional_prompt": (ctypes.c_int, [vp, vp, i32]),
        "tts_parler_default_config": (None, [ctypes.POINTER(ParlerConfig)]),
        "tts_parler_create": (vp, [ctypes.POINTER(BackendIface), ctypes.POINTER(ParlerConfig)]),
        "tts_parler_free": (None, [vp]),
        "tts_parler_set_device_sampling": (None, [vp, ctypes.c_int32]),
        "tts_parler_reset": (None, [vp]),
        "tts_parler_prefill": (ctypes.c_int, [vp, vp, i32]),
        "tts_parler_prefill_ragged": (ctypes.c_int, [vp, vp, vp, i32]),
        "tts_parler_decode": (ctypes.c_int, [vp, vp, vp]),
        "tts_parler_generate": (ctypes.c_int, [vp, i32, vp]),
        "tts_parler_position": (i32, [vp]),
        "tts_parler_host_stats": (i64, [vp, ctypes.POINTER(ctypes.c_double), ctypes.c_int]),
        "tts_parler_last_graph_nodes": (i32, [vp]),
        "tts_parler_graph": (vp, [vp, ctypes.POINTER(i32)]),
        "tts_parler_weight_bytes": (u64, [vp]),
        "tts_parler_get_node": (u64, [vp, ctypes.c_char_p, vp, u64]),
        "tts_parler_node": (u64, [vp, i32, ctypes.POINTER(i32), ctypes.POINTER(i32), ctypes.POINTER(i64), vp, u64]),
        "tts_dac_default_config": (None, [ctypes.POINTER(DacConfig)]),
        "tts_dac_create": (vp, [ctypes.POINTER(BackendIface), ctypes.POINTER(DacConfig)]),
        "tts_dac_free": (None, [vp]),
        "tts_dac_decode": (ctypes.c_int, [vp, vp, i32, vp]),
        "tts_dac_hop": (i64, [vp]),
        "tts_dac_last_graph_nodes": (i32, [vp]),
        "tts_dac_decode_batch": (ctypes.c_int, [vp, vp, i32, i32, i32, vp]),
        "tts_dac_min_gap": (i64, [vp]),
        "tts_dac_graph": (vp, [vp, ctypes.POINTER(i32)]),
        "tts_snac_default_config": (None, [ctypes.POINTER(SnacConfig)]),
        "tts_snac_create": (vp, [ctypes.POINTER(BackendIface), ctypes.POINTER(SnacConfig)]),
        "tts_snac_free": (None, [vp]),
        "tts_snac_decode": (ctypes.c_int, [vp, vp, i32, vp, vp]),
        "tts_snac_hop": (i64, [vp]),
        "tts_snac_noise_per_frame": (i64, [vp]),
        "tts_snac_last_graph_nodes": (i32, [vp]),
        "tts_snac_n_weights": (i32, [vp]),
        "tts_snac_get_node": (u64, [vp, ctypes.c_char_p, vp, u64]),
        "tts_snac_weight": (u64, [vp, i32, ctypes.c_char_p, u64, ctypes.POINTER(ctypes.c_int64), vp, u64]),
        "tts_kokoro_default_config": (None, [ctypes.POINTER(KokoroConfig)]),
        "tts_kokoro_create": (vp, [ctypes.POINTER(BackendIface), ctypes.POINTER(KokoroConfig)]),
        "tts_kokoro_free": (None, [vp]),
        "tts_kokoro_durations": (ctypes.c_int, [vp, vp, i32, vp, vp]),
        "tts_kokoro_decode": (ctypes.c_int, [vp, vp, i32, vp, vp, vp, vp, u64]),
# ... 27 lines not shown
        "tts_gguf_data_offset": (u64, [vp]),
        "tts_gguf_n_kv": (i64, [vp]),
        "tts_gguf_find_key": (i64, [vp, ctypes.c_char_p]),
        "tts_gguf_key": (ctypes.c_char_p, [vp, i64]),
        "tts_gguf_kv_type": (i32, [vp, i64]),
        "tts_gguf_get_u32": (ctypes.c_int, [vp, i64, ctypes.POINTER(ctypes.c_uint32)]),
        "tts_gguf_get_i64": (ctypes.c_int, [vp, i64, ctypes.POINTER(i64)]),
        "tts_gguf_get_f64": (ctypes.c_int, [vp, i64, ctypes.POINTER(ctypes.c_double)]),
        "tts_gguf_get_str": (ctypes.c_char_p, [vp, i64]),
        "tts_gguf_arr_type": (i32, [vp, i64]),
        "tts_gguf_arr_n": (i64, [vp, i64]),
        "tts_gguf_arr_data": (vp, [vp, i64]),
        "tts_gguf_arr_str": (ctypes.c_char_p, [vp, i64, i64]),
        "tts_gguf_n_tensors": (i64, [vp]),
        "tts_gguf_find_tensor": (i64, [vp, ctypes.c_char_p]),
        "tts_gguf_tensor_name": (ctypes.c_char_p, [vp, i64]),
        "tts_gguf_tensor_type": (i32, [vp, i64]),
        "tts_gguf_tensor_ndims": (i32, [vp, i64, ctypes.POINTER(i64)]),
        "tts_gguf_tensor_offset": (u64, [vp, i64]),
        "tts_gguf_tensor_size": (u64, [vp, i64]),
        "tts_gguf_tensor_data": (vp, [vp, i64]),
        "tts_gguf_type_size": (sz, [i32]),
        "tts_gguf_blck_size": (i64, [i32]),
        "tts_gguf_writer_new": (vp, []),
        "tts_gguf_writer_free": (None, [vp]),
        "tts_gguf_set_u32": (None, [vp, ctypes.c_char_p, ctypes.c_uint32]),
        "tts_gguf_set_i32": (None, [vp, ctypes.c_char_p, i32]),
        "tts_gguf_set_f32": (None, [vp, ctypes.c_char_p, ctypes.c_float]),
        "tts_gguf_set_u64": (None, [vp, ctypes.c_char_p, u64]),
        "tts_gguf_set_bool": (None, [vp, ctypes.c_char_p, ctypes.c_int]),
        "tts_gguf_set_str": (None, [vp, ctypes.c_char_p, ctypes.c_char_p]),
        "tts_gguf_set_arr": (None, [vp, ctypes.c_char_p, i32, vp, i64]),
        "tts_gguf_set_arr_str": (None, [vp, ctypes.c_char_p, ctypes.POINTER(ctypes.c_char_p), i64]),
        "tts_gguf_copy_kv": (None, [vp, vp]),
        "tts_gguf_add_tensor": (ctypes.c_int, [vp, ctypes.c_char_p, i32, i32, ctypes.POINTER(i64), vp, u64]),
        "tts_gguf_writer_write": (ctypes.c_int, [vp, ctypes.c_char_p]),
        "tts_gguf_tensor_rule": (ctypes.c_int, [ctypes.c_char_p, ctypes.c_char_p, ctypes.POINTER(QuantizeParams)]),
        "tts_gguf_tensor_out_type": (ctypes.c_int32, [ctypes.c_char_p, ctypes.c_char_p, ctypes.c_int32, ctypes.POINTER(QuantizeParams)]),
        "tts_gguf_quantize": (ctypes.c_int, [ctypes.c_char_p, ctypes.c_char_p, ctypes.POINTER(QuantizeParams), vp, vp]),
        "tts_hip_gguf_quantize": (ctypes.c_int, [vp, ctypes.c_char_p, ctypes.c_char_p, ctypes.POINTER(QuantizeParams)]),
        "tts_parler_config_from_gguf": (ctypes.c_int, [vp, ctypes.POINTER(ParlerConfig)]),
        "tts_parler_create_from_gguf": (vp, [ctypes.POINTER(BackendIface), ctypes.POINTER(ParlerConfig), vp]),
        "tts_parler_write_synthetic_gguf": (ctypes.c_int, [ctypes.POINTER(ParlerConfig), ctypes.POINTER(DacConfig), ctypes.c_char_p]),
        "tts_dac_config_from_gguf": (ctypes.c_int, [vp, ctypes.POINTER(DacConfig)]),
        "tts_dac_create_from_gguf": (vp, [ctypes.POINTER(BackendIface), ctypes.POINTER(DacConfig), vp]),
        "tts_dia_config_from_gguf": (ctypes.c_int, [vp, ctypes.POINTER(DiaConfig)]),
        "tts_dia_create_from_gguf": (vp, [ctypes.POINTER(BackendIface), ctypes.POINTER(DiaConfig), vp]),
        "tts_dia_write_synthetic_gguf": (ctypes.c_int, [ctypes.POINTER(DiaConfig), ctypes.POINTER(DacConfig), ctypes.c_char_p]),
        "tts_dia_set_weight": (ctypes.c_int, [vp, i32, vp, u64]),
        "tts_orpheus_config_from_gguf": (ctypes.c_int, [vp, ctypes.POINTER(OrpheusConfig)]),
        "tts_orpheus_create_from_gguf": (vp, [ctypes.POINTER(BackendIface), ctypes.POINTER(OrpheusConfig), vp]),
        "tts_orpheus_write_synthetic_gguf": (ctypes.c_int, [ctypes.POINTER(OrpheusConfig), ctypes.POINTER(SnacConfig), ctypes.c_char_p]),
        "tts_orpheus_set_weight": (ctypes.c_int, [vp, i32, vp, u64]),
        "tts_snac_config_from_gguf": (ctypes.c_int, [vp, ctypes.POINTER(SnacConfig)]),
        "tts_snac_create_from_gguf": (vp, [ctypes.POINTER(BackendIface), ctypes.POINTER(SnacConfig), vp]),
    }
    for name, (res, args) in sig.items():
        fn = getattr(L, name)
        fn.restype = res
        fn.argtypes = args
    _lib = L
    if os.environ.get("TTS_HIP_CRASH_HANDLER") == "1":
        L.tts_hip_install_crash_handler()
    return L


class HipBackend:

    def __init__(self, device=0):
        L = lib()
        n = L.tts_hip_device_count()
        if n <= device:
            raise RuntimeError(f"no HIP device {device} (device count {n})")
        self.ptr = L.tts_hip_backend_init(device)
        if not self.ptr:
            raise RuntimeError("tts_hip_backend_init failed")
        self.L = L

    def iface(self, reference_flow=False):
        it = BackendIface()
        if self.L.tts_hip_backend_iface(self.ptr, ctypes.byref(it)) != 0:
            raise RuntimeError("tts_hip_backend_iface failed")
        if reference_flow:
            for f in ("prepare", "launch", "set_async", "copy", "greedy_step", "sample_step"):
                setattr(it, f, None)
        return it

    def alloc(self, nbytes):
        p = self.L.tts_hip_buffer_alloc(self.ptr, nbytes)
        if not p:
            raise MemoryError(f"tts_hip_buffer_alloc({nbytes}) failed")
        return p

    def free(self, p):
        self.L.tts_hip_buffer_free(self.ptr, p)

    def set(self, dev, host_arr):
        st = self.L.tts_hip_tensor_set(self.ptr, dev, host_arr.ctypes.data, host_arr.nbytes)
        if st != 0:
            raise RuntimeError(f"tensor_set failed {st}")

    def get(self, host_arr, dev):
        st = self.L.tts_hip_tensor_get(self.ptr, host_arr.ctypes.data, dev, host_arr.nbytes)
        if st != 0:
            raise RuntimeError(f"tensor_get failed {st}")

    def sample_step(self, logits, cfg, call, rep_state=None, step=100, bos=-2, eos=-3, eos_seen=None):
        import numpy as np
        lg = np.ascontiguousarray(logits, dtype=np.float32)
        B, NH, V = lg.shape
        rs = np.ascontiguousarray(rep_state if rep_state is not None else np.tile(np.array([-1, 0], np.int32), B * NH), dtype=np.int32)
        es = np.ascontiguousarray(eos_seen if eos_seen is not None else np.zeros(B * NH, np.int32), dtype=np.int32)
        bufs = [self.alloc(n) for n in (lg.nbytes, rs.nbytes, es.nbytes, B * NH * 4, B * NH * 4)]
        try:
            self.set(bufs[0], lg)
            self.set(bufs[1], rs)
            self.set(bufs[2], es)
            st = self.L.tts_hip_sample_step(self.ptr, bufs[0], B, NH, V, ctypes.byref(cfg), call, bufs[1], step, bos, eos, bufs[2], bufs[3], bufs[4])
            if st != 0:
                raise RuntimeError(f"tts_hip_sample_step failed {st}")
            hist = np.zeros((B, NH), np.int32)
            nxt = np.zeros((NH, B), np.int32)
            self.get(hist, bufs[3])
            self.get(nxt, bufs[4])
            self.get(rs, bufs[1])
            self.get(es, bufs[2])
            return hist, nxt, es, rs
        finally:
            for b in bufs:
                self.free(b)

    def quantize(self, wtype, x):
        import numpy as np
        x = np.ascontiguousarray(x, dtype=np.float32)
        N, K = x.shape
        rs = K // BLCK_SIZE[wtype] * TYPE_SIZE[wtype]
        dx, dq = self.alloc(x.nbytes), self.alloc(N * rs)
        try:
            self.set(dx, x)
            st = self.L.tts_hip_quantize(self.ptr, wtype, dx, dq, N, K)
            if st != 0:
                raise RuntimeError(f"tts_hip_quantize failed {st}")
            out = np.empty(N * rs, dtype=np.uint8)
            self.get(out, dq)
            return out
        finally:
            self.free(dx)
            self.free(dq)

    def sync(self):
        if self.L.tts_hip_synchronize(self.ptr) != 0:
            raise RuntimeError("synchronize failed")

    def set_option(self, opt, value):
        self.L.tts_hip_set_option(self.ptr, opt, value)

    def gemv_stats(self, wtype=-1, reset=True):
        ms = ctypes.c_double()
        n = ctypes.c_int64()
        b = ctypes.c_double()
        self.L.tts_hip_gemv_stats(self.ptr, wtype, ctypes.byref(ms), ctypes.byref(n), ctypes.byref(b), 1 if reset else 0)
        return ms.value, n.value, b.value

    def counters(self):
        out = (ctypes.c_int64 * 10)()
        n = self.L.tts_hip_counters(self.ptr, out, 10)
        keys = ("graph_updates", "graph_instantiations", "lstm_chains", "lstm_steps", "plan_wait_ns",
                "cap_plan_ns", "cap_launch_ns", "cap_update_ns", "conv_pack_images", "conv_pack_bytes")
        return {keys[i]: int(out[i]) for i in range(n)}

    def close(self):
        if self.ptr:
            self.L.tts_hip_backend_free(self.ptr)
            self.ptr = None


def runner_weights(n_fn, w_fn, ptr):
    import numpy as np
    out = {}
    for i in range(n_fn(ptr)):
        name = ctypes.create_string_buffer(128)
        ne = (ctypes.c_int64 * 4)()
        ty = ctypes.c_int32()
        n = w_fn(ptr, i, name, 128, ne, ctypes.byref(ty), None, 0)
        if ty.value not in (F32, F16):
            continue
        a = np.empty(n, dtype=np.uint8)
        w_fn(ptr, i, name, 128, ne, ctypes.byref(ty), a.ctypes.data, n)
        a = a.view(np.float32 if ty.value == F32 else np.float16).astype(np.float32)
        shape = [int(v) for v in reversed(list(ne))]
        while len(shape) > 1 and shape[0] == 1:
            shape.pop(0)
        out[name.value.decode()] = a.reshape(shape)
    return out


class _Runner:
    PREFIX = None
    TYPED_WEIGHTS = True

    def _fn(self, name):
        return getattr(self.L, f"{self.PREFIX}_{name}")

    def weight_bytes(self):
        return self._fn("weight_bytes")(self.ptr)

    def weights(self):
        n_fn, w_fn = self._fn("n_weights"), self._fn("weight")
        if self.TYPED_WEIGHTS:
            return runner_weights(n_fn, w_fn, self.ptr)
        return runner_weights(n_fn, lambda ptr, i, name, cap, ne, ty, dst, n: w_fn(ptr, i, name, cap, ne, dst, n), self.ptr)

    def weights_raw(self):
        import numpy as np
        w_fn = self._fn("weight" if self.TYPED_WEIGHTS else "weight_raw")
        out = {}
        for i in range(self._fn("n_weights")(self.ptr)):
            name = ctypes.create_string_buffer(128)
            ne = (ctypes.c_int64 * 4)()
            ty = ctypes.c_int32()
            n = w_fn(self.ptr, i, name, 128, ne, ctypes.byref(ty), None, 0)
            a = np.empty(n, dtype=np.uint8)
            if w_fn(self.ptr, i, name, 128, ne, ctypes.byref(ty), a.ctypes.data, n) != n:
                raise RuntimeError(f"reading weight {name.value.decode()} failed")
            out[name.value.decode()] = (ty.value, tuple(ne), a)
        return out

    def set_weight(self, i, data):
        import numpy as np
        d = np.ascontiguousarray(data).view(np.uint8).reshape(-1)
        if self._fn("set_weight")(self.ptr, i, d.ctypes.data, d.nbytes) != 0:
            raise RuntimeError(f"setting weight {i} failed ({d.nbytes} bytes)")

    def plan_stats(self, mask=None):
        n = ctypes.c_int32()
        p = self._fn("graph")(self.ptr, ctypes.byref(n))
        return plan_stats(p, n.value, FUSE_ALL if mask is None else mask)

    def node(self, i, cap=1 << 26):
        import numpy as np
        op, ty = ctypes.c_int32(), ctypes.c_int32()
        ne = (ctypes.c_int64 * 4)()
        buf = np.empty(cap // 4, dtype=np.float32)
        n = self._fn("node")(self.ptr, i, ctypes.byref(op), ctypes.byref(ty), ne, buf.ctypes.data, cap)
        data = buf[: n // 4].copy() if n else None
        return OPS[op.value], ty.value, tuple(ne), data

    def named(self, name, dtype="float32", lead=()):
        import numpy as np
        get = self._fn("get_node")
        n = get(self.ptr, *lead, name.encode(), None, 0)
# ... 845 lines not shown
```

Before: 125.1.

## Fuse next-step input feed (tokens, positions, masks) into greedy/sample step kernels

Adds a step_feed path in which the greedy and sampling kernels also write the next decode step's token ids, positions, self-attention mask and cross-attention mask directly into the graph input tensors. This replaces the separate device copy of next tokens and the host-side upload of positions and masks each AR step, cutting per-step launches and host-to-device transfers. It also rewrites the Q4_K embedding-sum kernel into a templated version that loads the header as vectors. The cost is extra work inside the sampling kernel and more complex invalidation bookkeeping for the coalesce and conv-pack caches.

```diff
diff --git a/include/tts_hip.h b/include/tts_hip.h
--- a/include/tts_hip.h
+++ b/include/tts_hip.h
@@ -228,6 +228,7 @@
     TTS_HIP_OPT_CONV_PACK = 55,
     TTS_HIP_OPT_CONVT_PACK = 56,
     TTS_HIP_OPT_CONV_XREG = 57,
+    TTS_HIP_OPT_STEP_FEED = 58,
     TTS_HIP_OPT_COALESCE = 37,
 };
 enum tts_fuse_bits {
@@ -271,6 +272,20 @@
                         int64_t call, int32_t * rep_state, int32_t step, int32_t bos, int32_t eos, int32_t * eos_seen, int32_t * hist,
                         int32_t * next);
 int tts_sampling_device_ok(const tts_sampling * cfg, int32_t V);
+typedef struct tts_step_feed {
+    int32_t * tokens;
+    int32_t * positions;
+    float * mask;
+    float * mask_cross;
+    const int32_t * seq_len;
+    int32_t position;
+    int32_t rows;
+    int32_t n_cross;
+    int32_t hole_end;
+} tts_step_feed;
+int tts_hip_step_feed(tts_hip_backend_t backend, const float * logits, int32_t B, int32_t NH, int32_t V, const tts_sampling * cfg,
+                      int64_t call, int32_t * rep_state, int32_t step, int32_t bos, int32_t eos, int32_t * eos_seen, int32_t * hist,
+                      int32_t * next, const tts_step_feed * feed);
 int tts_hip_counters(tts_hip_backend_t backend, int64_t * out, int n);
 
 int tts_hip_gemv(tts_hip_backend_t backend, int type, const void * w, const float * x, float * y,
@@ -299,6 +314,8 @@
                        int32_t * hist, int32_t * next);
     int (*sample_step)(void * ctx, const float * logits, int B, int NH, int V, const tts_sampling * cfg, int64_t call, int32_t * rep_state,
                        int step, int bos, int eos, int32_t * eos_seen, int32_t * hist, int32_t * next);
+    int (*step_feed)(void * ctx, const float * logits, int B, int NH, int V, const tts_sampling * cfg, int64_t call, int32_t * rep_state,
+                     int step, int bos, int eos, int32_t * eos_seen, int32_t * hist, int32_t * next, const tts_step_feed * feed);
 } tts_backend_iface;
 
 int tts_hip_backend_iface(tts_hip_backend_t backend, tts_backend_iface * out);
diff --git a/tts.cpp_amd/csrc/backend.hip b/tts.cpp_amd/csrc/backend.hip
--- a/tts.cpp_amd/csrc/backend.hip
+++ b/tts.cpp_amd/csrc/backend.hip
@@ -432,6 +432,36 @@
     return launch_sample_step(be, logits, B, NH, V, cfg, call, rep_state, step, bos, eos, eos_seen, hist, next);
 }
 
+int tts_hip_step_feed(tts_hip_backend_t be, const float * logits, int32_t B, int32_t NH, int32_t V, const tts_sampling * cfg, int64_t call,
+                      int32_t * rep_state, int32_t step, int32_t bos, int32_t eos, int32_t * eos_seen, int32_t * hist, int32_t * next,
+                      const tts_step_feed * f) {
+    if (!be || !logits || B <= 0 || NH <= 0 || V <= 0 || !f || !f->tokens || !f->positions || !f->mask || !f->mask_cross || f->position < 0 ||
+        f->rows <= 0 || f->n_cross < 0 || (f->seq_len && f->rows != B))
+        return TTS_STATUS_BAD_ARG;
+    if (!be->step_feed) return TTS_STATUS_UNSUPPORTED;
+    hipSetDevice(be->device);
+    be->rb_clear();
+    const struct {
+        void * p;
+        size_t n;
+    } wr[4] = {{f->tokens, sizeof(int32_t) * B * NH},
+               {f->positions, sizeof(int32_t) * f->rows},
+               {f->mask, sizeof(float) * f->rows * ((size_t)f->position + 1)},
+               {f->mask_cross, sizeof(float) * f->n_cross}};
+    const char *l0 = (const char *)logits, *l1 = l0 + sizeof(float) * B * NH * (size_t)V;
+    for (const auto & w : wr)
+        if ((const char *)w.p < l1 && l0 < (const char *)w.p + w.n) return TTS_STATUS_UNSUPPORTED;
+    for (const auto & w : wr) tts::coalesce_written(w.p, w.n);
+    int st = 0;
+    if (cfg) st = launch_sample_step(be, logits, B, NH, V, cfg, call, rep_state, step, bos, eos, eos_seen, hist, next, f);
+    else launch_greedy_step(be, logits, B, NH, V, step, bos, eos, eos_seen, hist, next, f);
+    if (st == 0) {
+        for (const auto & w : wr) tts::conv_pack_written(be, w.p, w.n);
+        be->step_feeds += 1;
+    }
+    return st;
+}
+
 int tts_hip_tensor_get(tts_hip_backend_t be, void * dst, const void * src, size_t size) {
     if (!be) return TTS_STATUS_BAD_ARG;
     hipSetDevice(be->device);
@@ -928,6 +958,7 @@
             if (value < 0 || value > 4) return TTS_STATUS_BAD_ARG;
             be->gemv_kr_tail = value;
             return 0;
+        case TTS_HIP_OPT_STEP_FEED: be->step_feed = value != 0; return 0;
         case TTS_HIP_OPT_GEMM_KR_NW: be->gemm_kr_nw = value == 8 ? 8 : 4; return 0;
         case TTS_HIP_OPT_GEMM_Q8: be->gemm_q8 = value != 0; return 0;
         case TTS_HIP_OPT_CU_PARTITION: {
@@ -976,10 +1007,11 @@
 
 extern "C" int tts_hip_counters(tts_hip_backend_t be, int64_t * out, int n) {
     if (!be || !out) return TTS_STATUS_BAD_ARG;
-    const int64_t v[10] = {be->graph_updates, be->graph_instantiations, be->lstm_chains, be->lstm_steps, be->plan_wait_ns,
-                           be->cap_plan_ns, be->cap_launch_ns, be->cap_update_ns, (int64_t)g_packs_n.load(), (int64_t)g_packs_bytes.load()};
+    const int64_t v[11] = {be->graph_updates, be->graph_instantiations, be->lstm_chains, be->lstm_steps, be->plan_wait_ns,
+                           be->cap_plan_ns, be->cap_launch_ns, be->cap_update_ns, (int64_t)g_packs_n.load(), (int64_t)g_packs_bytes.load(),
+                           be->step_feeds};
     int k = 0;
-    for (; k < n && k < 10; ++k) out[k] = v[k];
+    for (; k < n && k < 11; ++k) out[k] = v[k];
     return k;
 }
 
@@ -1041,6 +1073,10 @@
 static int hb_sample(void * c, const float * l, int B, int NH, int V, const tts_sampling * cfg, int64_t call, int32_t * rep, int step, int bos,
                      int eos, int32_t * seen, int32_t * hist, int32_t * next) {
     return tts_hip_sample_step((tts_hip_backend_t)c, l, B, NH, V, cfg, call, rep, step, bos, eos, seen, hist, next);
+}
+static int hb_step_feed(void * c, const float * l, int B, int NH, int V, const tts_sampling * cfg, int64_t call, int32_t * rep, int step,
+                        int bos, int eos, int32_t * seen, int32_t * hist, int32_t * next, const tts_step_feed * feed) {
+    return tts_hip_step_feed((tts_hip_backend_t)c, l, B, NH, V, cfg, call, rep, step, bos, eos, seen, hist, next, feed);
 }
 
 extern "C" int tts_hip_backend_iface(tts_hip_backend_t be, tts_backend_iface * out) {
@@ -1061,5 +1097,6 @@
     out->copy = hb_copy;
     out->greedy_step = hb_greedy;
     out->sample_step = hb_sample;
+    out->step_feed = hb_step_feed;
     return 0;
 }
diff --git a/tts.cpp_amd/csrc/hip_internal.h b/tts.cpp_amd/csrc/hip_internal.h
--- a/tts.cpp_amd/csrc/hip_internal.h
+++ b/tts.cpp_amd/csrc/hip_internal.h
@@ -379,6 +379,8 @@
     int gemv_mf_prequant = 1;
     int gemv_kr = 1;
     int gemv_kr_loop = 1;
+    bool step_feed = true;
+    int64_t step_feeds = 0;
     int gemv_kr_tail = 1;
     int gemv_q80_pro = 1;
     int gemv_q80_slab = 1;
@@ -526,9 +528,23 @@
 void launch_cpy_multi(tts_hip_backend * be, const tts_tensor * src, const tts_tensor * const * dsts, int nd);
 void launch_rope_multi(tts_hip_backend * be, const tts_tensor * rope, const tts_tensor * src, const tts_tensor * const * dsts, int nd);
 void launch_greedy_step(tts_hip_backend * be, const float * logits, int B, int NH, int V, int step, int bos, int eos, int32_t * eos_seen,
-                        int32_t * hist, int32_t * next);
+                        int32_t * hist, int32_t * next, const tts_step_feed * feed = nullptr);
 int launch_sample_step(tts_hip_backend * be, const float * logits, int B, int NH, int V, const tts_sampling * c, int64_t call,
-                       int32_t * rep_state, int step, int bos, int eos, int32_t * eos_seen, int32_t * hist, int32_t * next);
+                       int32_t * rep_state, int step, int bos, int eos, int32_t * eos_seen, int32_t * hist, int32_t * next,
+                       const tts_step_feed * feed = nullptr);
+#ifdef __HIPCC__
+__device__ __forceinline__ void step_feed_write(const tts_step_feed & f, int64_t tid, int64_t nt) {
+    if (!f.mask) return;
+    const int32_t s = f.position;
+    const int64_t full = (int64_t)s + 1;
+    for (int64_t b = tid; b < f.rows; b += nt) f.positions[b] = f.seq_len && s >= f.hole_end ? f.seq_len[b] + (s - f.hole_end) : s;
+    for (int64_t k = tid; k < f.rows * full; k += nt) {
+        const int64_t b = k / full, j = k % full;
+        f.mask[k] = j > s || (f.seq_len && j >= f.seq_len[b] && j < f.hole_end) ? -INFINITY : 0.0f;
+    }
+    for (int64_t k = tid; k < f.n_cross; k += nt) f.mask_cross[k] = 0.0f;
+}
+#endif
 struct BatchCtx;
 void launch_embed_sum(tts_hip_backend * be, const tts_tensor * out, const tts_tensor * const * gr, int n, const BatchCtx * bat = nullptr,
                       const ItemTab * tab = nullptr);
diff --git a/tts.cpp_amd/csrc/k_fused.hip b/tts.cpp_amd/csrc/k_fused.hip
--- a/tts.cpp_amd/csrc/k_fused.hip
+++ b/tts.cpp_amd/csrc/k_fused.hip
@@ -365,9 +365,10 @@
 }
 
 __global__ __launch_bounds__(256) void k_greedy_step(const float * __restrict__ logits, int B, int NH, int V, int step, int bos, int eos,
-                                                     int32_t * eos_seen, int32_t * hist, int32_t * next) {
+                                                     int32_t * eos_seen, int32_t * hist, int32_t * next, tts_step_feed feed) {
     const int row = blockIdx.x * 4 + (threadIdx.x >> 6);
     const int lane = threadIdx.x & 63;
+    step_feed_write(feed, (int64_t)blockIdx.x * 256 + threadIdx.x, (int64_t)gridDim.x * 256);
     if (row >= B * NH) return;
     const float * l = logits + (int64_t)row * V;
     float best = -INFINITY;
@@ -393,7 +394,9 @@
     hist[row] = tok;
     const int seen = eos_seen[row] | (tok == eos);
     eos_seen[row] = seen;
-    next[h * B + b] = step + 1 > h ? (seen ? eos : tok) : bos;
+    const int nx = step + 1 > h ? (seen ? eos : tok) : bos;
+    next[h * B + b] = nx;
+    if (feed.tokens) feed.tokens[h * B + b] = nx;
 }
 
 __device__ __forceinline__ unsigned long long argmax_key(float v, int i) {
@@ -404,9 +407,10 @@
 
 __global__ __launch_bounds__(256) void k_greedy_step_wide(const float * __restrict__ logits, int B, int NH, int V, int step, int bos,
                                                           int eos, int32_t * eos_seen, int32_t * hist, int32_t * next,
-                                                          unsigned long long * keys, unsigned * counts) {
+                                                          unsigned long long * keys, unsigned * counts, tts_step_feed feed) {
     __shared__ unsigned long long s_k[4];
     const int row = blockIdx.y, nseg = gridDim.x;
+    step_feed_write(feed, ((int64_t)blockIdx.y * gridDim.x + blockIdx.x) * 256 + threadIdx.x, (int64_t)gridDim.x * gridDim.y * 256);
     const int64_t seg = ((int64_t)V + nseg - 1) / nseg;
     const int64_t i0 = (int64_t)blockIdx.x * seg, i1 = min((int64_t)V, i0 + seg);
     const float * l = logits + (int64_t)row * V;
@@ -433,21 +437,24 @@
     hist[row] = tok;
     const int seen = eos_seen[row] | (tok == eos);
     eos_seen[row] = seen;
-    next[h * B + b] = step + 1 > h ? (seen ? eos : tok) : bos;
+    const int nx = step + 1 > h ? (seen ? eos : tok) : bos;
+    next[h * B + b] = nx;
+    if (feed.tokens) feed.tokens[h * B + b] = nx;
 }
 
 void launch_greedy_step(tts_hip_backend * be, const float * logits, int B, int NH, int V, int step, int bos, int eos, int32_t * eos_seen,
-                        int32_t * hist, int32_t * next) {
+                        int32_t * hist, int32_t * next, const tts_step_feed * feed) {
+    const tts_step_feed f = feed ? *feed : tts_step_feed{};
     if (V >= 16384 && B * NH <= kArgmaxRows) {
         const unsigned nseg = (unsigned)((V + 4095) / 4096 < 64 ? (V + 4095) / 4096 : 64);
         hipLaunchKernelGGL(k_greedy_step_wide, dim3(nseg, (unsigned)(B * NH)), dim3(256), 0, be->stream, logits, B, NH, V, step, bos, eos,
-                           eos_seen, hist, next, be->argmax_keys, be->argmax_counts);
+                           eos_seen, hist, next, be->argmax_keys, be->argmax_counts, f);
         TTS_HIP_CHECK(hipGetLastError());
         return;
     }
     hipLaunchKernelGGL(k_greedy_step, dim3((unsigned)((B * NH + 3) / 4)), dim3(256), 0, be->stream, logits, B, NH, V, step, bos, eos, eos_seen,
-                       hist, next);
-    TTS_HIP_CHECK(hipGetLastError());
-}
-
-}
+                       hist, next, f);
+    TTS_HIP_CHECK(hipGetLastError());
+}
+
+}
diff --git a/tts.cpp_amd/csrc/k_ops.hip b/tts.cpp_amd/csrc/k_ops.hip
--- a/tts.cpp_amd/csrc/k_ops.hip
+++ b/tts.cpp_amd/csrc/k_ops.hip
@@ -313,27 +313,46 @@
     return __fsub_rn(__fmul_rn(__fmul_rn(d, (float)sc), (float)qv), __fmul_rn(dm, (float)mn));
 }
 
-__device__ __forceinline__ float table_elem_q4K_tiled(const char * base, int64_t row, int64_t nb, int64_t k) {
+__device__ __forceinline__ void q4K_tiled_addr(const char * base, int64_t row, int64_t nb, int64_t k, const u32x4 *& hdr,
+                                               const uint8_t *& qb) {
     const uint8_t * g = (const uint8_t *)base + ((row >> 2) * nb + k / QK_K) * 576;
     const int i = (int)(row & 3);
-    const uint8_t * hdr = g + i * 16;
     const int e = (int)(k % QK_K);
-    const int c = e / 64, w = e % 64, hi = w >= 32, l = w % 32 % 8, kk = w % 32 / 8;
-    const int sb = 2 * c + hi;
-    const uint8_t * q = hdr + 4;
+    const int c = e / 64, w = e % 64, l = w % 32 % 8, kk = w % 32 / 8;
+    hdr = (const u32x4 *)(g + i * 16);
+    qb = g + 64 + ((c * 2 + (l >> 2)) * 4 + i) * 16 + (l & 3) * 4 + kk;
+}
+__device__ __forceinline__ void q4K_row_addr(const char * base, int64_t row, int64_t nb1, bool repacked, int64_t k, const u32x4 *& hdr,
+                                             const uint8_t *& qb) {
+    const uint8_t * b = (const uint8_t *)base + row * nb1 + (k / QK_K) * (int64_t)sizeof(block_q4_K);
+    const int e = (int)(k % QK_K);
+    const int j64 = e / 64, l = e % 32;
+    hdr = (const u32x4 *)b;
+    qb = b + 16 + (repacked ? ((l & 7) * 16 + j64 * 4 + (l >> 3)) : (32 * j64 + l));
+}
+__device__ __forceinline__ float q4K_value(u32x4 hdr, uint8_t qb, int64_t k) {
+    const int e = (int)(k % QK_K);
+    const int c = e / 64, hi = e % 64 >= 32;
+    const int sb = 2 * c + hi, sh = 8 * (sb & 3);
+    const int q0 = (hdr.y >> sh) & 0xFF, q4 = (hdr.z >> sh) & 0xFF, q8 = (hdr.w >> sh) & 0xFF;
     int sc, mn;
     if (sb < 4) {
-        sc = q[sb] & 63;
-        mn = q[sb + 4] & 63;
+        sc = q0 & 63;
+        mn = q4 & 63;
     } else {
-        sc = (q[sb + 4] & 0xF) | ((q[sb - 4] >> 6) << 4);
-        mn = (q[sb + 4] >> 4) | ((q[sb] >> 6) << 4);
-    }
-    const float d = __half2float(__ushort_as_half(*(const uint16_t *)hdr));
-    const float dm = __half2float(__ushort_as_half(*(const uint16_t *)(hdr + 2)));
-    const uint8_t qb = g[64 + ((c * 2 + (l >> 2)) * 4 + i) * 16 + (l & 3) * 4 + kk];
+        sc = (q8 & 0xF) | ((q0 >> 6) << 4);
+        mn = (q8 >> 4) | ((q4 >> 6) << 4);
+    }
+    const float d = __half2float(__ushort_as_half((uint16_t)(hdr.x & 0xFFFF)));
+    const float dm = __half2float(__ushort_as_half((uint16_t)(hdr.x >> 16)));
     const int qv = hi ? (qb >> 4) : (qb & 0xF);
     return __fsub_rn(__fmul_rn(__fmul_rn(d, (float)sc), (float)qv), __fmul_rn(dm, (float)mn));
+}
+__device__ __forceinline__ float table_elem_q4K_tiled(const char * base, int64_t row, int64_t nb, int64_t k) {
+    const u32x4 * hdr;
+    const uint8_t * qb;
+    q4K_tiled_addr(base, row, nb, k, hdr, qb);
+    return q4K_value(*hdr, *qb, k);
 }
 
 __global__ void k_get_rows(TD dst, TD s0, TD s1) {
@@ -360,12 +379,13 @@
 struct EmbedArgs {
     EmbedTerm t[EMBED_MAX_TERMS];
     int n;
+    uint32_t moff_mask;
     float * out;
     int64_t H, M;
     int64_t ocs;
 };
 
-__global__ void k_embed_sum(EmbedArgs a) {
+__global__ void k_embed_sum_any(EmbedArgs a) {
     const int64_t m = blockIdx.y;
     const int64_t h = (int64_t)blockIdx.x * blockDim.x + threadIdx.x;
     if (h >= a.H) return;
@@ -379,6 +399,56 @@
         acc = t == 0 ? v : __fadd_rn(acc, v);
     }
     a.out[m * a.ocs + h] = acc;
+}
+
+template <int NT, bool MOFF>
+__global__ __launch_bounds__(256) void k_embed_sum(EmbedArgs a) {
+    const int64_t m = blockIdx.y;
+    const int64_t h = (int64_t)blockIdx.x * blockDim.x + threadIdx.x;
+    if (h >= a.H) return;
+    int64_t io[NT];
+#pragma unroll
+    for (int t = 0; t < NT; ++t) io[t] = MOFF ? *gptr(a.t[t].moff + m) : 0;
+    TTS_PIN_LOADS();
+    int32_t r[NT];
+#pragma unroll
+    for (int t = 0; t < NT; ++t) {
+        const EmbedTerm & T = a.t[t];
+        const int64_t o = (MOFF && ((a.moff_mask >> t) & 1)) ? io[t] : (T.rows == 1 ? 0 : m) * T.idx_stride;
+        r[t] = *gptr(T.idx + o);
+    }
+    TTS_PIN_LOADS();
+    u32x4 hdr[NT];
+    uint32_t w[NT];
+    int sh[NT];
+#pragma unroll
+    for (int t = 0; t < NT; ++t) {
+        const EmbedTerm & T = a.t[t];
+        const u32x4 *ph, *ph2;
+        const uint8_t *pq, *pq2;
+        q4K_tiled_addr(T.table.data, r[t], T.table.ne[0] / QK_K, h, ph, pq);
+        q4K_row_addr(T.table.data, r[t], T.table.nb[1], (T.table.pad & TTS_FLAG_REPACKED) != 0, h, ph2, pq2);
+        if (!(T.table.pad & TTS_FLAG_TILED)) ph = ph2, pq = pq2;
+        const char * pf = T.table.data + r[t] * T.table.nb[1] + h * 4;
+        const bool q = T.table.type == TTS_TYPE_Q4_K;
+        sh[t] = 8 * (int)((uintptr_t)pq & 3);
+        hdr[t] = *gptr(q ? ph : (const u32x4 *)((uintptr_t)pf & ~(uintptr_t)15));
+        w[t] = *gptr(q ? (const uint32_t *)((uintptr_t)pq & ~(uintptr_t)3) : (const uint32_t *)pf);
+    }
+    TTS_PIN_LOADS();
+    float acc = 0.f;
+#pragma unroll
+    for (int t = 0; t < NT; ++t) {
+        const float x = a.t[t].table.type == TTS_TYPE_Q4_K ? q4K_value(hdr[t], (uint8_t)(w[t] >> sh[t]), h) : __uint_as_float(w[t]);
+        if (t < a.n) acc = t == 0 ? x : __fadd_rn(acc, x);
+    }
+    a.out[m * a.ocs + h] = acc;
+}
+
+static bool embed_batched_ok(const tts_tensor * tb) {
+    const uintptr_t p = (uintptr_t)tb->data;
+    if (tb->type == TTS_TYPE_Q4_K) return p % 16 == 0 && ((tb->flags & TTS_FLAG_TILED) || tb->nb[1] % 16 == 0);
+    return tb->type == TTS_TYPE_F32 && tb->nb[0] == 4 && p % 16 == 0 && tb->nb[1] % 4 == 0 && (tb->nb[1] * tb->ne[1]) % 16 == 0;
 }
 
 void launch_embed_sum(tts_hip_backend * be, const tts_tensor * out, const tts_tensor * const * gr, int n, const BatchCtx * bat,
@@ -411,7 +481,35 @@
             a.t[i].idx = bat->win(a.t[i].idx);
         }
     }
-    hipLaunchKernelGGL(k_embed_sum, dim3((unsigned)((a.H + 255) / 256), (unsigned)a.M), dim3(256), 0, be->stream, a);
+    const dim3 grid((unsigned)((a.H + 255) / 256), (unsigned)a.M), block(256);
+    bool batched = true;
+    const int64_t * moff = nullptr;
+    for (int i = 0; i < n; ++i) {
+        batched &= embed_batched_ok(gr[i]->src[0]);
+        if (a.t[i].moff) {
+            a.moff_mask |= 1u << i;
+            moff = a.t[i].moff;
+        }
+    }
+    if (!batched) {
+        hipLaunchKernelGGL(k_embed_sum_any, grid, block, 0, be->stream, a);
+        TTS_HIP_CHECK(hipGetLastError());
+        return;
+    }
+    const int nt = (n + 3) / 4 * 4;
+    for (int i = n; i < nt; ++i) {
+        a.t[i] = a.t[n - 1];
+        a.moff_mask |= ((a.moff_mask >> (n - 1)) & 1u) << i;
+    }
+    for (int i = 0; i < nt; ++i)
+        if (!a.t[i].moff) a.t[i].moff = moff;
+#define TTS_EMBED(NT)                                                                                \
+    if (nt == NT) {                                                                                  \
+        if (moff) hipLaunchKernelGGL((k_embed_sum<NT, true>), grid, block, 0, be->stream, a);        \
+        else hipLaunchKernelGGL((k_embed_sum<NT, false>), grid, block, 0, be->stream, a);            \
+    }
+    TTS_EMBED(4) TTS_EMBED(8) TTS_EMBED(12) TTS_EMBED(16)
+#undef TTS_EMBED
     TTS_HIP_CHECK(hipGetLastError());
 }
 
diff --git a/tts.cpp_amd/csrc/k_sample.hip b/tts.cpp_amd/csrc/k_sample.hip
--- a/tts.cpp_amd/csrc/k_sample.hip
+++ b/tts.cpp_amd/csrc/k_sample.hip
@@ -19,6 +19,7 @@
     int32_t *eos_seen, *hist, *next;
     unsigned long long * cand;
     int nseg;
+    tts_step_feed feed;
 };
 
 __device__ __forceinline__ uint32_t ord_f32(float f) {
@@ -92,7 +93,9 @@
     a.hist[row] = tok;
     const int seen = a.eos_seen[row] | (tok == a.eos);
     a.eos_seen[row] = seen;
-    a.next[h * a.B + b] = a.step + 1 > h ? (seen ? a.eos : tok) : a.bos;
+    const int nx = a.step + 1 > h ? (seen ? a.eos : tok) : a.bos;
+    a.next[h * a.B + b] = nx;
+    if (a.feed.tokens) a.feed.tokens[h * a.B + b] = nx;
 }
 
 __device__ int draw_pick(const SampleArgs & a, int row, const float * p, const int * pick, int n, float mhp, bool topp) {
@@ -126,6 +129,7 @@
     const int row = blockIdx.x;
     const int V = a.V;
     const float * l = a.logits + (int64_t)row * V;
+    step_feed_write(a.feed, (int64_t)blockIdx.x * 256 + threadIdx.x, (int64_t)gridDim.x * 256);
     RowState r;
     load_state(a, row, r);
     int n2 = 1;
@@ -243,6 +247,7 @@
     __shared__ float s_cum;
     const int row = blockIdx.x;
     const float * l = a.logits + (int64_t)row * a.V;
+    step_feed_write(a.feed, (int64_t)blockIdx.x * 256 + threadIdx.x, (int64_t)gridDim.x * 256);
     RowState r;
     load_state(a, row, r);
     const int nc = a.nseg * KC;
@@ -275,8 +280,10 @@
 }
 
 int launch_sample_step(tts_hip_backend * be, const float * logits, int B, int NH, int V, const tts_sampling * c, int64_t call,
-                       int32_t * rep_state, int step, int bos, int eos, int32_t * eos_seen, int32_t * hist, int32_t * next) {
+                       int32_t * rep_state, int step, int bos, int eos, int32_t * eos_seen, int32_t * hist, int32_t * next,
+                       const tts_step_feed * feed) {
     SampleArgs a;
+    a.feed = feed ? *feed : tts_step_feed{};
     a.logits = logits;
     a.B = B, a.NH = NH, a.V = V;
     a.temperature = c->temperature, a.top_p = c->top_p, a.rep = c->repetition_penalty;
diff --git a/tts.cpp_amd/csrc/parler.cpp b/tts.cpp_amd/csrc/parler.cpp
--- a/tts.cpp_amd/csrc/parler.cpp
+++ b/tts.cpp_amd/csrc/parler.cpp
@@ -31,6 +31,7 @@
     std::vector<tts_tensor *> k_l, v_l;
     char * arena = nullptr;
     size_t arena_size = 0;
+    float * cross_buf = nullptr;
     tg::context gctx;
     tts_tensor * res = nullptr;
     tts_tensor *in_tokens = nullptr, *in_positions = nullptr, *in_mask = nullptr, *in_mask_cross = nullptr;
@@ -220,6 +221,11 @@
         tts_parler_free(p);
         return nullptr;
     }
+    p->cross_buf = (float *)p->be.alloc(p->be.ctx, sizeof(float) * (cf.n_encode > 0 ? cf.n_encode : 1));
+    if (!p->cross_buf) {
+        tts_parler_free(p);
+        return nullptr;
+    }
     if (cf.use_cross_attn && !prep_cross_key_values(p)) {
         fprintf(stderr, "parler: cross K/V precompute failed\n");
         tts_parler_free(p);
@@ -234,6 +240,7 @@
 extern "C" void tts_parler_free(tts_parler * p) {
     if (!p) return;
     if (p->arena) p->be.free(p->be.ctx, p->arena);
+    if (p->cross_buf) p->be.free(p->be.ctx, p->cross_buf);
     if (p->kvbuf) p->be.free(p->be.ctx, p->kvbuf);
     p->w.release(p->be);
     delete p;
@@ -320,6 +327,7 @@
     tg::set_input(p->in_mask);
     p->in_mask_cross = tg::new_tensor_2d(c, TTS_TYPE_F32, cf.n_encode, n);
     tg::set_input(p->in_mask_cross);
+    if (audio && n == 1) p->in_mask_cross->data = p->cross_buf;
 
     const float kq_scale = 1.0f / sqrtf((float)hd);
     tts_tensor * cur = nullptr;
@@ -486,10 +494,10 @@
     return 0;
 }
 
-static int launch_step(tts_parler * p, const int32_t * tokens, bool async = false) {
+static int launch_step(tts_parler * p, const int32_t * tokens, bool async = false, bool fed = false) {
     if (!p->prepared) return TTS_STATUS_FAILED;
     auto t0 = std::chrono::steady_clock::now();
-    if (set_inputs(p, tokens, p->prep_audio, p->prep_n, async) != 0) return TTS_STATUS_FAILED;
+    if (!fed && set_inputs(p, tokens, p->prep_audio, p->prep_n, async) != 0) return TTS_STATUS_FAILED;
     auto t1 = std::chrono::steady_clock::now();
     const int st = p->be.launch ? p->be.launch(p->be.ctx, p->prep_slot)
                                 : p->be.compute(p->be.ctx, p->gctx.nodes.data(), (int)p->gctx.nodes.size());
@@ -573,13 +581,19 @@
     int32_t * d_next = (int32_t *)be.alloc(be.ctx, rowi);
     int32_t * d_hist = (int32_t *)be.alloc(be.ctx, rowi * (size_t)n_steps);
     int32_t * d_rep = p->sampling ? (int32_t *)be.alloc(be.ctx, 2 * rowi) : nullptr;
+    const bool feed_len = be.step_feed && p->ragged && B > 1;
+    int32_t * d_len = feed_len ? (int32_t *)be.alloc(be.ctx, sizeof(int32_t) * B) : nullptr;
     auto release = [&] {
-        for (int32_t * q : {d_rep, d_seen, d_next, d_hist})
+        for (int32_t * q : {d_len, d_rep, d_seen, d_next, d_hist})
             if (q) be.free(be.ctx, q);
     };
-    if (!d_seen || !d_next || !d_hist || (p->sampling && !d_rep)) {
+    if (!d_seen || !d_next || !d_hist || (p->sampling && !d_rep) || (feed_len && !d_len)) {
         release();
         return TTS_STATUS_ALLOC_FAILED;
+    }
+    if (d_len && be.set(be.ctx, d_len, p->seq_len.data(), sizeof(int32_t) * B) != 0) {
+        release();
+        return TTS_STATUS_FAILED;
     }
     std::vector<int32_t> rep(2 * (size_t)B * NH);
     if (p->sampling) {
@@ -602,15 +616,33 @@
     for (int s = 0; st == 0 && s < n_steps; ++s) {
         const float * logits = (const float *)p->launched_out;
         if (s + 1 < n_steps) st = prepare_step(p, true, 1);
-        if (st == 0 && p->sampling)
+        bool fed = false;
+        if (st == 0 && s + 1 < n_steps && be.step_feed) {
+            const bool rg = p->ragged && B > 1;
+            tts_step_feed f{};
+            f.tokens = (int32_t *)p->in_tokens->data;
+            f.positions = (int32_t *)p->in_positions->data;
+            f.mask = (float *)p->in_mask->data;
+            f.mask_cross = (float *)p->in_mask_cross->data;
+            f.seq_len = rg ? d_len : nullptr;
+            f.position = p->position;
+            f.rows = rg ? B : 1;
+            f.n_cross = cf.n_encode;
+            f.hole_end = p->hole_end;
+            st = be.step_feed(be.ctx, logits, B, NH, V, p->sampling ? &p->samp : nullptr, p->sample_calls + s, d_rep, p->current_step + s,
+                              cf.bos_token, cf.eos_token, d_seen, d_hist + (size_t)s * B * NH, d_next, &f);
+            fed = st == 0;
+            if (st == TTS_STATUS_UNSUPPORTED) st = 0;
+        }
+        if (st == 0 && !fed && p->sampling)
             st = be.sample_step(be.ctx, logits, B, NH, V, &p->samp, p->sample_calls + s, d_rep, p->current_step + s, cf.bos_token, cf.eos_token,
                                 d_seen, d_hist + (size_t)s * B * NH, d_next);
-        else if (st == 0)
+        else if (st == 0 && !fed)
             st = be.greedy_step(be.ctx, logits, B, NH, V, p->current_step + s, cf.bos_token, cf.eos_token, d_seen,
                                 d_hist + (size_t)s * B * NH, d_next);
         if (st == 0 && s + 1 < n_steps) {
-            st = be.copy(be.ctx, p->in_tokens->data, d_next, rowi);
-            if (st == 0) st = launch_step(p, nullptr, true);
+            if (!fed) st = be.copy(be.ctx, p->in_tokens->data, d_next, rowi);
+            if (st == 0) st = launch_step(p, nullptr, true, fed);
         }
     }
     std::vector<int32_t> hist((size_t)n_steps * B * NH);
diff --git a/tts.cpp_amd/ttship/__init__.py b/tts.cpp_amd/ttship/__init__.py
--- a/tts.cpp_amd/ttship/__init__.py
+++ b/tts.cpp_amd/ttship/__init__.py
@@ -20,7 +20,7 @@
 FUSE_ALL = sum(FUSE.values())
 UNARY = {"ABS": 0, "NEG": 1, "TANH": 2, "RELU": 3, "SIGMOID": 4, "GELU": 5, "SILU": 6, "EXP": 7}
 
-OPT = {"FUSION": 0, "PROFILE_GEMV": 1, "GRAPHS": 2, "CONV_F32ACC": 3, "CONVT_LDS": 4, "ATTN_SPLIT": 5, "KV_PREFETCH": 6, "KV_PREFETCH_BLOCKS": 7, "Q4K_TILE_BYTES": 8, "GEMV_DEBUG": 10, "GEMV_UNIQUE": 11, "CONV_SPLIT": 12, "GEMV_KS": 13, "ATTN_FUSED": 14, "ATTN_PV16": 15, "Q4K_DUAL_BYTES": 16, "GEMV_RSPLIT": 17, "GEMM_Q8": 18, "BGEMM_F32": 19, "CU_PARTITION": 20, "GEMV_PREQUANT": 21, "GEMV_KRELAY": 22, "ATTN_KS": 23, "ATTN_PV8": 24, "GEMV_NW_MIN": 25, "GEMV_KRELAY_LOOP": 26, "GEMV_Q80_PRO": 27, "GEMV_Q80_SLAB": 28, "GEMV_Q80_RW": 29, "GEMM_Q8_STAGED": 30, "GEMV_KR_INKERNEL": 31, "GEMV_F32_WIDE": 32, "ATTN_PV_MP": 33, "GEMM_KR_NW": 34, "GEMM_KR_INKERNEL": 35, "GEMM_KR_CT2": 36, "COALESCE": 37, "GEMM_KR_XCD": 38, "GEMM_KR_CP": 39, "GEMM_KR_WALK": 40, "GEMM_PF": 41, "GEMM_PF_NW": 42, "ATTN_ONE": 43, "GEMV_KR_TAIL": 44, "GEMV_Q50_SLAB": 45, "GEMV_Q50_RW": 46, "GEMM_Q5": 47, "GEMM_Q5_STAGED": 48, "GEMV_Q40_SLAB": 49, "GEMV_Q40_RW": 50, "GEMM_Q4_0": 51, "GEMM_Q4_0_STAGED": 52, "CONV_VFMA": 53, "CONV_TILE96": 54, "CONV_PACK": 55, "CONVT_PACK": 56, "CONV_XREG": 57}
+OPT = {"FUSION": 0, "PROFILE_GEMV": 1, "GRAPHS": 2, "CONV_F32ACC": 3, "CONVT_LDS": 4, "ATTN_SPLIT": 5, "KV_PREFETCH": 6, "KV_PREFETCH_BLOCKS": 7, "Q4K_TILE_BYTES": 8, "GEMV_DEBUG": 10, "GEMV_UNIQUE": 11, "CONV_SPLIT": 12, "GEMV_KS": 13, "ATTN_FUSED": 14, "ATTN_PV16": 15, "Q4K_DUAL_BYTES": 16, "GEMV_RSPLIT": 17, "GEMM_Q8": 18, "BGEMM_F32": 19, "CU_PARTITION": 20, "GEMV_PREQUANT": 21, "GEMV_KRELAY": 22, "ATTN_KS": 23, "ATTN_PV8": 24, "GEMV_NW_MIN": 25, "GEMV_KRELAY_LOOP": 26, "GEMV_Q80_PRO": 27, "GEMV_Q80_SLAB": 28, "GEMV_Q80_RW": 29, "GEMM_Q8_STAGED": 30, "GEMV_KR_INKERNEL": 31, "GEMV_F32_WIDE": 32, "ATTN_PV_MP": 33, "GEMM_KR_NW": 34, "GEMM_KR_INKERNEL": 35, "GEMM_KR_CT2": 36, "COALESCE": 37, "GEMM_KR_XCD": 38, "GEMM_KR_CP": 39, "GEMM_KR_WALK": 40, "GEMM_PF": 41, "GEMM_PF_NW": 42, "ATTN_ONE": 43, "GEMV_KR_TAIL": 44, "GEMV_Q50_SLAB": 45, "GEMV_Q50_RW": 46, "GEMM_Q5": 47, "GEMM_Q5_STAGED": 48, "GEMV_Q40_SLAB": 49, "GEMV_Q40_RW": 50, "GEMM_Q4_0": 51, "GEMM_Q4_0_STAGED": 52, "CONV_VFMA": 53, "CONV_TILE96": 54, "CONV_PACK": 55, "CONVT_PACK": 56, "CONV_XREG": 57, "STEP_FEED": 58}
 ATTN_SPLIT_DEFAULT = 128
 ATTN_ONE_DEFAULT = 1
 GEMV_KR_TAIL_DEFAULT = 1
@@ -68,6 +68,7 @@
         ("copy", ctypes.c_void_p),
         ("greedy_step", ctypes.c_void_p),
         ("sample_step", ctypes.c_void_p),
+        ("step_feed", ctypes.c_void_p),
     ]
 
 
@@ -80,6 +81,20 @@
         ("do_sample", ctypes.c_int32),
         ("pad_", ctypes.c_int32),
         ("seed", ctypes.c_uint64),
+    ]
+
+
+class StepFeed(ctypes.Structure):
+    _fields_ = [
+        ("tokens", ctypes.c_void_p),
+        ("positions", ctypes.c_void_p),
+        ("mask", ctypes.c_void_p),
+        ("mask_cross", ctypes.c_void_p),
+        ("seq_len", ctypes.c_void_p),
+        ("position", ctypes.c_int32),
+        ("rows", ctypes.c_int32),
+        ("n_cross", ctypes.c_int32),
+        ("hole_end", ctypes.c_int32),
     ]
 
 
@@ -363,6 +378,8 @@
         "tts_sampler_sample": (ctypes.c_int, [ctypes.POINTER(Sampling), vp, i32, i32, ctypes.c_uint32, vp, vp, vp]),
         "tts_hip_sample_step": (ctypes.c_int, [vp, vp, i32, i32, i32, ctypes.POINTER(Sampling), i64, vp, i32, i32, i32, vp, vp, vp]),
         "tts_hip_greedy_step": (ctypes.c_int, [vp, vp, i32, i32, i32, i32, i32, i32, vp, vp, vp]),
+        "tts_hip_step_feed": (ctypes.c_int, [vp, vp, i32, i32, i32, ctypes.POINTER(Sampling), i64, vp, i32, i32, i32, vp, vp, vp,
+                                             ctypes.POINTER(StepFeed)]),
         "tts_hip_backend_iface": (ctypes.c_int, [vp, ctypes.POINTER(BackendIface)]),
         "tts_hip_weight_set": (ctypes.c_int, [vp, ctypes.POINTER(TtsTensor), vp]),
         "tts_hip_quantize": (ctypes.c_int, [vp, ctypes.c_int, vp, vp, i64, i64]),
@@ -556,7 +573,7 @@
         if self.L.tts_hip_backend_iface(self.ptr, ctypes.byref(it)) != 0:
             raise RuntimeError("tts_hip_backend_iface failed")
         if reference_flow:
-            for f in ("prepare", "launch", "set_async", "copy", "greedy_step", "sample_step"):
+            for f in ("prepare", "launch", "set_async", "copy", "greedy_step", "sample_step", "step_feed"):
                 setattr(it, f, None)
         return it
 
@@ -637,10 +654,10 @@
         return ms.value, n.value, b.value
 
     def counters(self):
-        out = (ctypes.c_int64 * 10)()
-        n = self.L.tts_hip_counters(self.ptr, out, 10)
+        out = (ctypes.c_int64 * 11)()
+        n = self.L.tts_hip_counters(self.ptr, out, 11)
         keys = ("graph_updates", "graph_instantiations", "lstm_chains", "lstm_steps", "plan_wait_ns",
-                "cap_plan_ns", "cap_launch_ns", "cap_update_ns", "conv_pack_images", "conv_pack_bytes")
+                "cap_plan_ns", "cap_launch_ns", "cap_update_ns", "conv_pack_images", "conv_pack_bytes", "step_feeds")
         return {keys[i]: int(out[i]) for i in range(n)}
 
     def close(self):
```

After: 125.5, median of 6. No clear change (+0.3%).
